# yanqinJiang/Animate3D

Measured on AMD Instinct MI355X. Metric: UNet denoise-steps/sec, 4view×16frame×512² MV-VDM @1/2/4/8 GPU, higher is better.
Workload: dtype bf16; 1 GPU; BASELINE config 2: 4 views x 16 frames x 512^2 px (64x64 latent), CFG-doubled batch V=8 videos, one MVUNetMotionModel.forward per step, SD1.5 MV-VDM UNet 1.53 B params, seeded synthetic weights; parallelism=single GPU

## Files before the change

### animate3d_amd/csrc/flash_attn.hip

```cpp
#include <type_traits>
#include <utility>

#include "common.h"
#include "flash_common.h"


namespace {

template <int D, int BKV, int QT, int OFS, bool ALIGNED, int VAR, int NM = 0, bool TWO = false>
__global__ __launch_bounds__(256, 2) void flash_attn_kernel(const AttnParams p) {
  constexpr int NU = BKV / 32;
  constexpr int VROW = BKV + 8;
  constexpr int DK = (D + 15) / 16 * 16;
  constexpr int KS = DK / 16;
  constexpr int MT = (D + 31) / 32;
  constexpr int KROW = DK + 8;
  constexpr int DCH = D / 8;
  constexpr int KCHUNKS = BKV * DCH;
  constexpr int KPT = (KCHUNKS + 255) / 256;
  constexpr int VITEMS = (BKV / 4) * DCH;
  constexpr int VPT = (VITEMS + 255) / 256;
  constexpr bool ONES = MT * 32 > D;
  constexpr int KS_ELEMS = BKV * KROW, VT_ELEMS = MT * 32 * VROW;
  constexpr int BQW = 32 * QT, BQ = 4 * BQW;
  constexpr int KS_PAD = D / 16, G_PAD = (D % 16) / 8;
  static_assert((KROW / 8) % 2 == 1 && (VROW / 8) % 2 == 1, "LDS row strides must be an odd number of 16-B slots");
  static_assert(OFS != OFS_PAD || (DK > D && D % 8 == 0), "OFS_PAD needs a spare contraction slot");

  __shared__ __attribute__((aligned(16))) uint16_t smem[2 * (KS_ELEMS + VT_ELEMS)];
  uint16_t* const Ks0 = smem;
  uint16_t* const Vt0 = smem + 2 * KS_ELEMS;

  const int tid = threadIdx.x, lane = tid & 63, wid = tid >> 6;
  const int l31 = lane & 31, g = lane >> 5;
  const int head = blockIdx.x % p.heads;
  const int qt = blockIdx.x / p.heads;
  const int64_t grp = blockIdx.y;
  const int64_t hoff = (int64_t)head * D;

  if constexpr (DK > D) {
    for (int i = tid; i < 2 * BKV * (DK - D); i += 256) {
      const int b = i / (BKV * (DK - D)), rem = i % (BKV * (DK - D));
      const int c = rem % (DK - D);
      Ks0[b * KS_ELEMS + (rem / (DK - D)) * KROW + D + c] = (OFS == OFS_PAD && c == 0) ? ONE16 : 0;
    }
  }
  if constexpr (ONES) {
    for (int i = tid; i < 2 * BKV; i += 256) Vt0[(i / BKV) * VT_ELEMS + D * VROW + (i % BKV)] = ONE16;
  }

  int q_idx[QT];
  bool q_ok[QT];
  u32x4_t qf[QT][KS];
#pragma unroll
  for (int qs = 0; qs < QT; ++qs) {
    q_idx[qs] = qt * BQ + wid * BQW + qs * 32 + l31;
    q_ok[qs] = q_idx[qs] < p.q_len;
    const int64_t q_row = map_row(p.qm, grp, q_ok[qs] ? q_idx[qs] : p.q_len - 1);
#pragma unroll
    for (int ks = 0; ks < KS; ++ks) {
      const int d0 = 16 * ks + 8 * g;
      if (d0 < D) {
        u32x4_t w = *reinterpret_cast<const u32x4_t*>(p.Q + q_row * p.qm.ld + hoff + d0);
        if constexpr (OFS != OFS_FMA) {
#pragma unroll
          for (int j = 0; j < 4; ++j) w[j] = pack16(lo16(w[j]) * p.scale_log2, hi16(w[j]) * p.scale_log2);
        }
        qf[qs][ks] = w;
      } else {
        qf[qs][ks] = u32x4_t{0u, 0u, 0u, 0u};
      }
    }
  }

#ifdef A3D_STORAGE_F16
  constexpr bool TRY_NOMAX = false;
#else
  constexpr bool TRY_NOMAX = NM != 0;
#endif
  static_assert(NM == 0 || (OFS != OFS_FMA && ALIGNED && ONES), "the max-free pass needs the offset inside the matrix pipe and MFMA row sums");
  f32x16_t osave[TWO ? QT : 1][TWO ? MT : 1];
  auto pass = [&](auto nm_c, auto set_c) __attribute__((always_inline)) -> bool {
  constexpr bool NOMAX = decltype(nm_c)::value;
  constexpr bool SET1 = decltype(set_c)::value;
  const uint16_t* const Kp = SET1 ? p.K2 : p.K;
  const uint16_t* const Vp = SET1 ? p.V2 : p.V;
  const a3d_rowmap& kmp = SET1 ? p.km2 : p.km;
  const int kvl = SET1 ? p.kv_len2 : p.kv_len;
  const float oscale = SET1 ? p.out_scale2 : p.out_scale;
  if constexpr (OFS == OFS_PAD) {
#pragma unroll
    for (int qs = 0; qs < QT; ++qs)
      if (g == G_PAD) qf[qs][KS_PAD][0] = 0u;
  }
  const int64_t ld = kmp.ld;
  const int64_t kgbase = map_group_base(kmp, grp);
  const uint16_t* const Kh = Kp + hoff;
  const uint16_t* const Vh = Vp + hoff;
  const uint32_t seg_len = (uint32_t)kmp.seg_len;
  const int64_t tile_step = (int64_t)BKV * ld;
  const int64_t wrap_step = (kmp.seg_stride - kmp.seg_len) * ld;
  int kr[KPT], kc[KPT], vq[VPT], vc[VPT];
  const uint16_t* kptr[KPT];
  const uint16_t* vptr[VPT];
#pragma unroll
  for (int i = 0; i < KPT; ++i) {
    const int c = tid + 256 * i;
    kr[i] = c / DCH; kc[i] = c % DCH;
    kptr[i] = Kh + (kgbase + kr[i]) * ld + kc[i] * 8;
  }
#pragma unroll
  for (int i = 0; i < VPT; ++i) {
    const int it = tid + 256 * i;
    vq[i] = it / DCH; vc[i] = it % DCH;
    vptr[i] = Vh + (kgbase + vq[i] * 4) * ld + vc[i] * 8;
  }
  uint32_t seg_off = 0;
  int next_kv0 = 0;

  auto row_generic = [&](int s) -> int64_t {
    if (s >= kvl) s = kvl - 1;
    const uint32_t seg = (uint32_t)s / seg_len;
    return kgbase + (int64_t)seg * kmp.seg_stride + ((uint32_t)s - seg * seg_len);
  };

  u32x4_t kreg[KPT];
  u32x4_t vreg[VPT][4];
  auto load_kv = [&](auto tail_c) {
    constexpr bool TAIL = decltype(tail_c)::value;
    if constexpr (ALIGNED && !TAIL) {
#pragma unroll
      for (int i = 0; i < KPT; ++i)
        if (tid + 256 * i < KCHUNKS) kreg[i] = *reinterpret_cast<const u32x4_t*>(kptr[i]);
#pragma unroll
      for (int i = 0; i < VPT; ++i)
        if (tid + 256 * i < VITEMS) {
#pragma unroll
          for (int r = 0; r < 4; ++r) vreg[i][r] = *reinterpret_cast<const u32x4_t*>(vptr[i] + r * ld);
        }
      seg_off += BKV;
      int64_t step = tile_step;
      if (seg_off >= seg_len) { step += wrap_step; seg_off = 0; }
#pragma unroll
      for (int i = 0; i < KPT; ++i) kptr[i] += step;
#pragma unroll
      for (int i = 0; i < VPT; ++i) vptr[i] += step;
    } else {
#pragma unroll
      for (int i = 0; i < KPT; ++i)
        if (tid + 256 * i < KCHUNKS)
          kreg[i] = *reinterpret_cast<const u32x4_t*>(Kh + row_generic(next_kv0 + kr[i]) * ld + kc[i] * 8);
#pragma unroll
      for (int i = 0; i < VPT; ++i)
        if (tid + 256 * i < VITEMS) {
#pragma unroll
          for (int r = 0; r < 4; ++r)
            vreg[i][r] = *reinterpret_cast<const u32x4_t*>(Vh + row_generic(next_kv0 + vq[i] * 4 + r) * ld + vc[i] * 8);
        }
    }
    next_kv0 += BKV;
  };
  auto store_kv = [&](int buf) {
    uint16_t* const Ks = Ks0 + buf * KS_ELEMS;
    uint16_t* const Vt = Vt0 + buf * VT_ELEMS;
#pragma unroll
    for (int i = 0; i < KPT; ++i)
      if (tid + 256 * i < KCHUNKS) *reinterpret_cast<u32x4_t*>(Ks + kr[i] * KROW + kc[i] * 8) = kreg[i];
#pragma unroll
    for (int i = 0; i < VPT; ++i)
      if (tid + 256 * i < VITEMS) {
#pragma unroll
        for (int j = 0; j < 4; ++j) {
          const uint32_t w0 = vreg[i][0][j], w1 = vreg[i][1][j], w2 = vreg[i][2][j], w3 = vreg[i][3][j];
          u32x2_t even, odd;
          even[0] = __builtin_amdgcn_perm(w1, w0, 0x05040100u);
          even[1] = __builtin_amdgcn_perm(w3, w2, 0x05040100u);
          odd[0] = __builtin_amdgcn_perm(w1, w0, 0x07060302u);
          odd[1] = __builtin_amdgcn_perm(w3, w2, 0x07060302u);
          *reinterpret_cast<u32x2_t*>(Vt + (vc[i] * 8 + 2 * j) * VROW + vq[i] * 4) = even;
          *reinterpret_cast<u32x2_t*>(Vt + (vc[i] * 8 + 2 * j + 1) * VROW + vq[i] * 4) = odd;
        }
      }
  };

  f32x16_t oacc[QT][MT];
#pragma unroll
  for (int qs = 0; qs < QT; ++qs)
#pragma unroll
    for (int mt = 0; mt < MT; ++mt)
#pragma unroll
      for (int r = 0; r < 16; ++r) oacc[qs][mt][r] = 0.f;
  float m_off[QT];
  float l_run = 0.f;
  f32x16_t minit[OFS == OFS_ACC ? QT : 1];
#pragma unroll
  for (int qs = 0; qs < QT; ++qs) m_off[qs] = (OFS == OFS_FMA) ? -INFINITY : 0.f;
  if constexpr (OFS == OFS_ACC) {
#pragma unroll
    for (int qs = 0; qs < QT; ++qs)
#pragma unroll
      for (int r = 0; r < 16; ++r) minit[qs][r] = 0.f;
  }
  bool first = true;
  const int krow_off = kperm(l31) * KROW + 8 * g;
  const int vrow_off = l31 * VROW + 8 * g;

  auto compute = [&](int buf, int kv0, auto tail_c, auto first_c) {
    constexpr bool TAIL = decltype(tail_c)::value;
    constexpr int FM = decltype(first_c)::value;
    const uint16_t* const Ks = Ks0 + buf * KS_ELEMS + krow_off;
    const uint16_t* const Vt = Vt0 + buf * VT_ELEMS + vrow_off;
    f32x16_t sacc[QT][NU];
#pragma unroll
    for (int u = 0; u < NU; ++u) {
#pragma unroll
      for (int qs = 0; qs < QT; ++qs) {
        if constexpr (OFS == OFS_ACC) sacc[qs][u] = minit[qs];
        else {
#pragma unroll
          for (int r = 0; r < 16; ++r) sacc[qs][u][r] = 0.f;
        }
      }
#pragma unroll
      for (int ks = 0; ks < KS; ++ks) {
        const u32x4_t kf = *reinterpret_cast<const u32x4_t*>(Ks + 32 * u * KROW + 16 * ks);
        if constexpr ((VAR & 1) != 0) __builtin_amdgcn_s_setprio(1);
#pragma unroll
        for (int qs = 0; qs < QT; ++qs) sacc[qs][u] = mfma32(kf, qf[qs][ks], sacc[qs][u]);
        if constexpr ((VAR & 1) != 0) __builtin_amdgcn_s_setprio(0);
      }
    }
    if constexpr (TAIL) {
#pragma unroll
      for (int u = 0; u < NU; ++u)
#pragma unroll
        for (int r = 0; r < 16; ++r)
          if (kv0 + 32 * u + 16 * (r >> 3) + 8 * g + (r & 7) >= kvl) {
#pragma unroll
            for (int qs = 0; qs < QT; ++qs) sacc[qs][u][r] = -INFINITY;
          }
    }
    if (p.causal) {
#pragma unroll
      for (int qs = 0; qs < QT; ++qs)
#pragma unroll
        for (int u = 0; u < NU; ++u)
#pragma unroll
          for (int r = 0; r < 16; ++r)
            if (kv0 + 32 * u + 16 * (r >> 3) + 8 * g + (r & 7) > q_idx[qs]) sacc[qs][u][r] = -INFINITY;
    }

    if constexpr (OFS == OFS_FMA && QT > 1) {
#pragma unroll
      for (int qs = 0; qs < QT; ++qs) {
        float mx = sacc[qs][0][0];
#pragma unroll
        for (int u = 0; u < NU; ++u)
#pragma unroll
          for (int r = 0; r < 16; ++r) mx = fmaxf(mx, sacc[qs][u][r]);
        if (__any(mx > m_off[qs] + LAZY_THR / p.scale_log2)) {
          mx = fmaxf(mx, __shfl_xor(mx, 32));
          const float m_new = fmaxf(m_off[qs], mx);
          const float alpha = __builtin_amdgcn_exp2f((m_off[qs] - m_new) * p.scale_log2);
          m_off[qs] = m_new;
          if constexpr (!ONES) l_run *= alpha;
#pragma unroll
          for (int mt = 0; mt < MT; ++mt)
#pragma unroll
            for (int r = 0; r < 16; ++r) oacc[qs][mt][r] *= alpha;
        }
        const float mneg = -m_off[qs] * p.scale_log2;
#pragma unroll
        for (int u = 0; u < NU; ++u)
#pragma unroll
          for (int r = 0; r < 16; ++r) sacc[qs][u][r] = fmaf(sacc[qs][u][r], p.scale_log2, mneg);
      }
    } else if constexpr (OFS == OFS_FMA) {
      float mx = sacc[0][0][0];
#pragma unroll
      for (int u = 0; u < NU; ++u)
#pragma unroll
        for (int r = 0; r < 16; ++r) mx = fmaxf(mx, sacc[0][u][r]);
      if (__any(mx > m_off[0] + LAZY_THR / p.scale_log2)) {
        mx = fmaxf(mx, __shfl_xor(mx, 32));
        const float m_new = fmaxf(m_off[0], mx);
        const float alpha = __builtin_amdgcn_exp2f((m_off[0] - m_new) * p.scale_log2);
        m_off[0] = m_new;
        l_run *= alpha;
#pragma unroll
        for (int mt = 0; mt < MT; ++mt)
#pragma unroll
          for (int r = 0; r < 16; ++r) oacc[0][mt][r] *= alpha;
      }
      const float mneg = -m_off[0] * p.scale_log2;
#pragma unroll
      for (int u = 0; u < NU; ++u)
#pragma unroll
        for (int r = 0; r < 16; ++r) sacc[0][u][r] = fmaf(sacc[0][u][r], p.scale_log2, mneg);
    } else {
      if constexpr (FM != 0) {
      const bool isfirst = (FM == 1) ? true : first;
#pragma unroll
      for (int qs = 0; qs < QT; ++qs) {
        float mx = sacc[qs][0][0];
#pragma unroll
        for (int u = 0; u < NU; ++u)
#pragma unroll
          for (int r = 0; r < 16; ++r) mx = fmaxf(mx, sacc[qs][u][r]);
        if (__any(isfirst || mx > LAZY_THR)) {
          const float mxp = fmaxf(mx, __shfl_xor(mx, 32));
          float delta = isfirst ? mxp + (NOMAX ? 40.f : 0.f) : fmaxf(mxp, 0.f);
          float new_off = m_off[qs] + delta;
          if constexpr (OFS == OFS_PAD) { new_off = round16(new_off); delta = new_off - m_off[qs]; }
          m_off[qs] = new_off;
#pragma unroll
          for (int u = 0; u < NU; ++u)
#pragma unroll
            for (int r = 0; r < 16; ++r) sacc[qs][u][r] -= delta;
          if (!isfirst) {
            const float alpha = __builtin_amdgcn_exp2f(-delta);
            if constexpr (!ONES) l_run *= alpha;
#pragma unroll
            for (int mt = 0; mt < MT; ++mt)
#pragma unroll
              for (int r = 0; r < 16; ++r) oacc[qs][mt][r] *= alpha;
          }
          if constexpr (OFS == OFS_PAD) {
            if (g == G_PAD) qf[qs][KS_PAD][0] = pack16(-new_off, 0.f);
          } else {
#pragma unroll
            for (int r = 0; r < 16; ++r) minit[qs][r] = -new_off;
          }
        }
      }
      }
      first = false;
    }

#pragma unroll
    for (int u = 0; u < NU; ++u) {
      u32x4_t vfr[(VAR & 2) ? MT : 1][2];
      if constexpr ((VAR & 2) != 0) {
#pragma unroll
        for (int mt = 0; mt < MT; ++mt)
#pragma unroll
          for (int h = 0; h < 2; ++h) vfr[mt][h] = *reinterpret_cast<const u32x4_t*>(Vt + 32 * mt * VROW + 32 * u + 16 * h);
      }
      u32x4_t pf[QT][2];
#pragma unroll
      for (int qs = 0; qs < QT; ++qs) {
        float pv[16];
#pragma unroll
        for (int r = 0; r < 16; ++r) {
          pv[r] = __builtin_amdgcn_exp2f(sacc[qs][u][r]);
          if constexpr (!ONES) l_run += pv[r];
        }
#pragma unroll
        for (int h = 0; h < 2; ++h)
#pragma unroll
          for (int j = 0; j < 4; ++j) pf[qs][h][j] = pack16(pv[8 * h + 2 * j], pv[8 * h + 2 * j + 1]);
      }
      if constexpr ((VAR & 1) != 0) __builtin_amdgcn_s_setprio(1);
#pragma unroll
      for (int mt = 0; mt < MT; ++mt)
#pragma unroll
        for (int h = 0; h < 2; ++h) {
          u32x4_t vf;
          if constexpr ((VAR & 2) != 0) vf = vfr[mt][h];
          else vf = *reinterpret_cast<const u32x4_t*>(Vt + 32 * mt * VROW + 32 * u + 16 * h);
#pragma unroll
          for (int qs = 0; qs < QT; ++qs) oacc[qs][mt] = mfma32(vf, pf[qs][h], oacc[qs][mt]);
        }
      if constexpr ((VAR & 1) != 0) __builtin_amdgcn_s_setprio(0);
    }
    if constexpr ((VAR & 4) != 0) {
#pragma unroll
      for (int i = 0; i < NU * MT * 2 * QT; ++i) {
        __builtin_amdgcn_sched_group_barrier(0x008, 1, 0);
        __builtin_amdgcn_sched_group_barrier(0x400, 4, 0);
        __builtin_amdgcn_sched_group_barrier(0x002, 2, 0);
      }
    }
  };

  const int ntiles = (kvl + BKV - 1) / BKV;
  const bool has_tail = (kvl % BKV) != 0;
  auto load_tile = [&](int t) {
    if (has_tail && t == ntiles - 1) load_kv(std::true_type{}); else load_kv(std::false_type{});
  };

  load_tile(0);
  store_kv(0);
  if (ntiles > 1) load_tile(1);
  __syncthreads();
  const int nfast = has_tail ? ntiles - 1 : ntiles;
  constexpr std::integral_constant<int, NOMAX ? 0 : 2> FM_LOOP{};
  int t = 0;
  if constexpr (ALIGNED) {
    if constexpr (NOMAX) {
      store_kv(1);
      load_kv(std::false_type{});
      compute(0, 0, std::false_type{}, std::integral_constant<int, 1>{});
      __syncthreads();
      t = 1;
    }
    for (; t + 2 < nfast; ++t) {
      store_kv((t + 1) & 1);
      load_kv(std::false_type{});
      compute(t & 1, t * BKV, std::false_type{}, FM_LOOP);
      __syncthreads();
    }
  }
  for (; t < ntiles - 1; ++t) {
    store_kv((t + 1) & 1);
    if (t + 2 < ntiles) load_tile(t + 2);
    compute(t & 1, t * BKV, std::false_type{}, FM_LOOP);
    __syncthreads();
  }
  if (has_tail) compute((ntiles - 1) & 1, (ntiles - 1) * BKV, std::true_type{}, FM_LOOP);
  else compute((ntiles - 1) & 1, (ntiles - 1) * BKV, std::false_type{}, FM_LOOP);

  float inv[QT], l_fin[QT];
  bool bad = false;
#pragma unroll
  for (int qs = 0; qs < QT; ++qs) {
    float l_tot;
    if constexpr (ONES) {
      constexpr int LM = D / 32, LR = ((D % 32) / 8) * 4;
      static_assert((D % 32) % 8 == 0, "row D must map to half 0");
      l_tot = __shfl(oacc[qs][LM][LR], l31);
    } else {
      l_tot = l_run + __shfl_xor(l_run, 32);
    }
    bad = bad || !(l_tot < 1.2676506e30f) || !(l_tot > 0.f);
    inv[qs] = oscale / l_tot;
    l_fin[qs] = l_tot;
  }
  if constexpr (NOMAX) {
    if (__syncthreads_or(bad ? 1 : 0)) return false;
  }
  if constexpr (!TWO) {
    if (p.lse != nullptr) {
#pragma unroll
      for (int qs = 0; qs < QT; ++qs)
        if (q_ok[qs] && g == 0)
          p.lse[((int64_t)grp * p.heads + head) * p.q_len + q_idx[qs]] =
              __builtin_amdgcn_logf(l_fin[qs]) + (OFS == OFS_FMA ? m_off[qs] * p.scale_log2 : m_off[qs]);
    }
  }
  if constexpr (TWO && !SET1) {
    if (p.K2 != nullptr) {
#pragma unroll
      for (int qs = 0; qs < QT; ++qs)
#pragma unroll
        for (int mt = 0; mt < MT; ++mt)
#pragma unroll
          for (int r = 0; r < 16; ++r) osave[qs][mt][r] = oacc[qs][mt][r] * inv[qs];
      return true;
    }
  }
#pragma unroll
  for (int qs = 0; qs < QT; ++qs) {
    if (q_ok[qs]) {
      uint16_t* orow = p.O + map_row(p.om, grp, q_idx[qs]) * p.om.ld + hoff;
#pragma unroll
      for (int mt = 0; mt < MT; ++mt)
#pragma unroll
        for (int qd = 0; qd < 4; ++qd) {
          const int d = 32 * mt + 8 * qd + 4 * g;
          if (d < D) {
            float v[4];
#pragma unroll
            for (int j = 0; j < 4; ++j) {
              v[j] = oacc[qs][mt][4 * qd + j] * inv[qs];
              if constexpr (TWO && SET1) v[j] += osave[qs][mt][4 * qd + j];
            }
            if (p.accumulate) {
              const u32x2_t prev = *reinterpret_cast<const u32x2_t*>(orow + d);
              v[0] += lo16(prev[0]); v[1] += hi16(prev[0]); v[2] += lo16(prev[1]); v[3] += hi16(prev[1]);
            }
            u32x2_t o;
            o[0] = pack16(v[0], v[1]);
            o[1] = pack16(v[2], v[3]);
            *reinterpret_cast<u32x2_t*>(orow + d) = o;
          }
        }
    }
  }
  return true;
  };

  if constexpr (TRY_NOMAX) {
    if (!pass(std::true_type{}, std::false_type{})) pass(std::false_type{}, std::false_type{});
  } else {
    pass(std::false_type{}, std::false_type{});
  }
  if constexpr (TWO) {
    if (p.K2 != nullptr) {
      __syncthreads();
      pass(std::false_type{}, std::true_type{});
    }
  }
}

bool map_ok(const a3d_rowmap* m, int head_dim) {
  return m && m->gdiv > 0 && m->seg_len > 0 && m->ld > 0 && m->ld % 8 == 0 && head_dim % 8 == 0;
}


template <int D, int BKV, int QT, int OFS, int VAR = 0, int NM = 0>
void launch(bool aligned, int groups, hipStream_t s, const AttnParams& p) {
  const int q_tiles = (p.q_len + 128 * QT - 1) / (128 * QT);
  const dim3 grid((unsigned)(p.heads * q_tiles), (unsigned)groups);
  if (aligned) flash_attn_kernel<D, BKV, QT, OFS, true, VAR, NM><<<grid, dim3(256), 0, s>>>(p);
  else flash_attn_kernel<D, BKV, QT, OFS, false, 0><<<grid, dim3(256), 0, s>>>(p);
}

template <int D, int BKV, int OFS>
void launch_two(bool aligned, int groups, hipStream_t s, const AttnParams& p) {
  const int q_tiles = (p.q_len + 127) / 128;
  const dim3 grid((unsigned)(p.heads * q_tiles), (unsigned)groups);
  if (aligned) flash_attn_kernel<D, BKV, 1, OFS, true, 0, 0, true><<<grid, dim3(256), 0, s>>>(p);
  else flash_attn_kernel<D, BKV, 1, OFS, false, 0, 0, true><<<grid, dim3(256), 0, s>>>(p);
}

}

static int flash_attn_impl(a3d_stream_t stream, const void* Q, const void* K, const void* V, void* O,
                           const a3d_rowmap* qmap, const a3d_rowmap* kmap, const a3d_rowmap* omap,
                           int groups, int heads, int head_dim, int64_t q_len, int64_t kv_len,
                           float scale, float out_scale, int accumulate, float* lse, unsigned int* counters = nullptr) {
  if (!Q || !K || !V || !O || groups <= 0 || heads <= 0 || q_len <= 0 || kv_len <= 0) return A3D_EINVAL;
  if (!map_ok(qmap, head_dim) || !map_ok(kmap, head_dim) || !map_ok(omap, head_dim)) return A3D_EINVAL;
  if ((reinterpret_cast<uintptr_t>(Q) | reinterpret_cast<uintptr_t>(K) | reinterpret_cast<uintptr_t>(V)) & 15u) return A3D_EINVAL;
  if (reinterpret_cast<uintptr_t>(O) & 7u) return A3D_EINVAL;
  if (groups > 65535 || q_len > 0x3fffffffLL || kv_len > 0x3fffffffLL || kmap->seg_len > 0x3fffffffLL) return A3D_EINVAL;
  AttnParams p{};
  p.Q = (const uint16_t*)Q; p.K = (const uint16_t*)K; p.V = (const uint16_t*)V; p.O = (uint16_t*)O;
  p.qm = *qmap; p.km = *kmap; p.om = *omap;
  p.heads = heads; p.q_len = (int)q_len; p.kv_len = (int)kv_len;
  if (accumulate & ~(A3D_ATTN_ACCUMULATE | A3D_ATTN_CAUSAL | A3D_ATTN_EXACT | A3D_ATTN_PLAIN)) return A3D_EINVAL;
  p.scale_log2 = scale * 1.4426950408889634f; p.out_scale = out_scale; p.accumulate = accumulate & 1; p.causal = (accumulate >> 1) & 1;
  const bool exact = (accumulate & A3D_ATTN_EXACT) != 0, plain = (accumulate & A3D_ATTN_PLAIN) != 0;
  p.lse = lse;
  p.counters = counters;
  if (p.causal && head_dim != 64 && head_dim != 160) return A3D_EUNSUPPORTED;
  const int bkv = head_dim == 160 ? 32 : 64;
  const bool aligned = (kmap->seg_len % bkv == 0) || (kv_len <= kmap->seg_len);
  hipStream_t s = (hipStream_t)stream;
  switch (head_dim) {
    case 40:
      if (q_len <= 128) { launch<40, 64, 1, OFS_PAD>(aligned, groups, s, p); break; }
      if (!plain && aligned && kv_len % 64 == 0 && kv_len >= 256 && q_len >= 256) {
        if (int rc = A3D_FN(a3d_launch_flash_dm)(exact ? 4 : 5, groups, s, p)) return rc;
        break;
      }
      launch<40, 64, 2, OFS_PAD, 0>(aligned, groups, s, p);
      break;
    case 80:
      if (!plain && aligned && kv_len % 64 == 0 && kv_len >= 512 && q_len >= 256) {
        if (int rc = A3D_FN(a3d_launch_flash_dm80)(exact ? 0 : 1, groups, s, p)) return rc;
        break;
      }
      if (q_len >= 2048 && kv_len >= 2048) { launch<80, 32, 2, OFS_FMA>(aligned, groups, s, p); break; }
      launch<80, 64, 1, OFS_ACC>(aligned, groups, s, p);
      break;
    case 64: launch<64, 64, 1, OFS_FMA>(aligned, groups, s, p); break;
    case 160:
#ifndef A3D_EXP_R5_PATHS
      if (!plain && !p.causal && kv_len % 64 == 0 && kv_len >= 256 && ((kmap->seg_len % 64 == 0) || (kv_len <= kmap->seg_len)) &&
          (reinterpret_cast<uintptr_t>(O) & 15u) == 0 && omap->ld % 8 == 0) {
        if (int rc = A3D_FN(a3d_launch_flash_dm160)(exact ? 0 : 1, groups, s, p)) return rc;
        break;
      }
#endif
      launch<160, 32, 1, OFS_FMA>(aligned, groups, s, p);
      break;
    default: return A3D_EUNSUPPORTED;
  }
  return a3d_launch_status();
}

extern "C" int A3D_FN(a3d_flash_attn)(a3d_stream_t stream, const void* Q, const void* K, const void* V, void* O,
                                   const a3d_rowmap* qmap, const a3d_rowmap* kmap, const a3d_rowmap* omap,
                                   int groups, int heads, int head_dim, int64_t q_len, int64_t kv_len,
                                   float scale, float out_scale, int accumulate) {
  return flash_attn_impl(stream, Q, K, V, O, qmap, kmap, omap, groups, heads, head_dim, q_len, kv_len, scale, out_scale, accumulate, nullptr);
}

extern "C" int A3D_FN(a3d_flash_attn_lse)(a3d_stream_t stream, const void* Q, const void* K, const void* V, void* O,
                                       const a3d_rowmap* qmap, const a3d_rowmap* kmap, const a3d_rowmap* omap,
                                       int groups, int heads, int head_dim, int64_t q_len, int64_t kv_len,
                                       float scale, float out_scale, int accumulate, float* lse2) {
  if (!lse2) return A3D_EINVAL;
  return flash_attn_impl(stream, Q, K, V, O, qmap, kmap, omap, groups, heads, head_dim, q_len, kv_len, scale, out_scale, accumulate, lse2);
}

extern "C" int A3D_FN(a3d_flash_attn_counted)(a3d_stream_t stream, const void* Q, const void* K, const void* V, void* O,
                                           const a3d_rowmap* qmap, const a3d_rowmap* kmap, const a3d_rowmap* omap,
                                           int groups, int heads, int head_dim, int64_t q_len, int64_t kv_len,
                                           float scale, float out_scale, int accumulate, unsigned int* counters) {
  if (!counters || (reinterpret_cast<uintptr_t>(counters) & 3u)) return A3D_EINVAL;
  return flash_attn_impl(stream, Q, K, V, O, qmap, kmap, omap, groups, heads, head_dim, q_len, kv_len, scale, out_scale, accumulate, nullptr, counters);
}

extern "C" int A3D_FN(a3d_flash_attn2)(a3d_stream_t stream, const void* Q, const void* K, const void* V, const void* K2, const void* V2, void* O,
                                    const a3d_rowmap* qmap, const a3d_rowmap* kmap, const a3d_rowmap* kmap2, const a3d_rowmap* omap,
                                    int groups, int heads, int head_dim, int64_t q_len, int64_t kv_len, int64_t kv_len2,
                                    float scale, float out_scale, float out_scale2, int accumulate) {
  if (!Q || !K || !V || !K2 || !V2 || !O || groups <= 0 || heads <= 0 || q_len <= 0 || kv_len <= 0 || kv_len2 <= 0) return A3D_EINVAL;
  if (!map_ok(qmap, head_dim) || !map_ok(kmap, head_dim) || !map_ok(kmap2, head_dim) || !map_ok(omap, head_dim)) return A3D_EINVAL;
  if ((reinterpret_cast<uintptr_t>(Q) | reinterpret_cast<uintptr_t>(K) | reinterpret_cast<uintptr_t>(V) | reinterpret_cast<uintptr_t>(K2) |
       reinterpret_cast<uintptr_t>(V2)) & 15u) return A3D_EINVAL;
  if (reinterpret_cast<uintptr_t>(O) & 7u) return A3D_EINVAL;
  if (groups > 65535 || q_len > 0x3fffffffLL || kv_len > 0x3fffffffLL || kv_len2 > 0x3fffffffLL || kmap->seg_len > 0x3fffffffLL ||
      kmap2->seg_len > 0x3fffffffLL) return A3D_EINVAL;
  if (head_dim != 40 && head_dim != 80) return A3D_EUNSUPPORTED;
  AttnParams p{};
  p.Q = (const uint16_t*)Q; p.K = (const uint16_t*)K; p.V = (const uint16_t*)V; p.O = (uint16_t*)O;
  p.K2 = (const uint16_t*)K2; p.V2 = (const uint16_t*)V2;
  p.qm = *qmap; p.km = *kmap; p.km2 = *kmap2; p.om = *omap;
  p.heads = heads; p.q_len = (int)q_len; p.kv_len = (int)kv_len; p.kv_len2 = (int)kv_len2;
  if (accumulate & ~(A3D_ATTN_ACCUMULATE | A3D_ATTN_PLAIN)) return A3D_EINVAL;
  p.scale_log2 = scale * 1.4426950408889634f; p.out_scale = out_scale; p.out_scale2 = out_scale2; p.accumulate = accumulate & 1; p.causal = 0;
  const bool aligned = ((kmap->seg_len % 64 == 0) || (kv_len <= kmap->seg_len)) && ((kmap2->seg_len % 64 == 0) || (kv_len2 <= kmap2->seg_len));
  hipStream_t s = (hipStream_t)stream;
  if (head_dim == 40 && !(accumulate & A3D_ATTN_PLAIN)) {
    const int rc = A3D_FN(a3d_launch_cross_attn40)(groups, s, p);
    if (rc != A3D_EUNSUPPORTED) return rc;
  }
  if (head_dim == 40) launch_two<40, 64, OFS_PAD>(aligned, groups, s, p);
  else launch_two<80, 64, OFS_ACC>(aligned, groups, s, p);
  return a3d_launch_status();
}
```

### animate3d_amd/csrc/flash_attn_dm80.hip

```cpp
#include "flash_common.h"

namespace {

constexpr int E_ROWB = 160;
constexpr int E_UNITB = 32 * E_ROWB;
constexpr int E_KB = 2 * E_UNITB;
constexpr int E_TILEB = 2 * E_KB;
constexpr int E_RING = 5;
constexpr int E_CV = E_RING * E_TILEB + 32;
constexpr int E_CV_BYTES = 2752;
constexpr int E_SAMPLE = E_CV + E_CV_BYTES;
constexpr int E_SMEM_BYTES = E_SAMPLE + E_UNITB;
constexpr float E_L_BAD = 1.2676506e30f;
#ifdef A3D_STORAGE_F16
constexpr float E_BIAS = F16_BIAS;
constexpr bool E_SAMPLED = true;
#else
constexpr float E_BIAS = 40.f;
constexpr bool E_SAMPLED = false;
#endif

#ifdef A3D_EXP_R5_PATHS
constexpr bool E_EARLY_DMA = false;
#else
constexpr bool E_EARLY_DMA = true;
#endif

extern __shared__ __attribute__((aligned(16))) uint8_t e_smem[];
A3D_DEV u32x4_t e_lds128(uint32_t off) { return *reinterpret_cast<const u32x4_t*>(e_smem + off); }
A3D_DEV u32x2_t e_ldstr(uint32_t off) { return lds_tr16_b64(reinterpret_cast<const uint16_t*>(e_smem + off)); }

template <int FLAGS>
__global__ __launch_bounds__(512, 2) void flash_attn_dm80_kernel(const AttnParams p) {
  constexpr int D = 80, KS = 5, MT = 3, NT = 512, BQ = 256;
  constexpr int NEXP = 16, NCVT = 8, NDMA = 3;
  constexpr bool TRY_NOMAX = (FLAGS & 1) != 0;

  const int tid = threadIdx.x, lane = tid & 63, wid = tid >> 6;
  const int w = __builtin_amdgcn_readfirstlane(wid);
  const int l31 = lane & 31, g = lane >> 5, i16 = lane & 15, q4 = lane >> 4;
  const int head = blockIdx.x % p.heads;
  const int qt = blockIdx.x / p.heads;
  const int64_t grp = blockIdx.y;
  const int64_t hoff = (int64_t)head * D;
  const uint32_t lds0 = fa_lds_addr(e_smem);

  for (int i = tid; i < E_CV_BYTES / 2; i += NT) {
    const int vb = 2 * i;
    reinterpret_cast<uint16_t*>(e_smem + E_CV)[i] = (vb == 0 || vb == 160 || vb == 2560 || vb == 2720) ? ONE16 : (uint16_t)0;
  }

  const int64_t ld = p.km.ld;
  const int64_t kgbase = map_group_base(p.km, grp);
  const uint32_t seg_len = (uint32_t)p.km.seg_len;
  const int64_t tile_step = (int64_t)64 * ld;
  const int64_t wrap_step = (p.km.seg_stride - p.km.seg_len) * ld;
  auto slot_src = [&](int slot) -> uint32_t {
    const bool isk = slot < 640;
    const int s2 = isk ? slot : slot - 640;
    const int prow = s2 / 10, cpos = s2 % 10;
    const int c = isk ? (cpos ^ ((prow >> 3) & 1)) : cpos;
    const int key = isk ? prow : ((prow & ~7) | (((prow & 7) >> 1) + 4 * (prow & 1)));
    return (uint32_t)(((int64_t)key * ld + c * 8) * 2);
  };
  const uint32_t voffA = slot_src(64 * w + lane);
  const uint32_t voffB = slot_src(512 + 64 * w + lane);
  const uint32_t voffC = slot_src(1024 + 32 * w + l31);
  uint32_t voffS = 0;
  if constexpr (E_SAMPLED) {
    const int ss = (64 * w + lane) % 320, prow = ss / 10;
    const int64_t key = (int64_t)prow * (p.kv_len / 32);
    voffS = (uint32_t)((map_seq(p.km, key) * ld + ((ss % 10) ^ ((prow >> 3) & 1)) * 8) * 2);
  }
  const uint64_t maskS = w < 5 ? ~0ull : 0ull;

  const int krow = kperm(l31);
  const uint32_t klane = (uint32_t)(krow * E_ROWB + 16 * (g ^ ((krow >> 3) & 1)));
  const int c4 = i16 & 3;
  const uint32_t vrow = (uint32_t)((8 * (q4 >> 1) + 2 * (i16 >> 2)) * E_ROWB);
  const uint32_t vlane01 = vrow + (uint32_t)(2 * (16 * (q4 & 1) + 4 * c4));
  const bool v2_data = (q4 & 1) == 0;
  const uint32_t vlane2 = v2_data ? vrow + (uint32_t)(2 * (64 + 4 * c4)) : (c4 == 0 ? (uint32_t)E_CV : (uint32_t)(E_CV + 8));
  uint32_t vmul = v2_data ? 1u : 0u;
  asm volatile("" : "+v"(vmul));

  const uint16_t* gA = nullptr;
  const uint16_t* gB = nullptr;
  const uint16_t* gC = nullptr;
  uint32_t seg_off = 0;
  auto dma_reset = [&]() __attribute__((always_inline)) {
    gA = dm_scalar(p.K + hoff + kgbase * ld);
    gB = dm_scalar((w < 2 ? p.K : p.V) + hoff + kgbase * ld);
    gC = dm_scalar(p.V + hoff + kgbase * ld);
    seg_off = 0;
  };
  auto tile_base = [&](int tile) __attribute__((always_inline)) -> uint32_t { return (uint32_t)((tile % E_RING) * E_TILEB); };
  auto dma_a = [&](int tile) __attribute__((always_inline)) { dm_glds16(voffA, gA, lds0 + tile_base(tile) + 1024 * w); };
  auto dma_b = [&](int tile) __attribute__((always_inline)) { dm_glds16(voffB, gB, lds0 + tile_base(tile) + 8192 + 1024 * w); };
  auto dma_c = [&](int tile) __attribute__((always_inline)) {
    dm_glds16_m(voffC, gC, lds0 + tile_base(tile) + 16384 + 512 * w, 0xffffffffull);
    seg_off += 64;
    int64_t stp = tile_step;
    if (seg_off >= seg_len) { stp += wrap_step; seg_off = 0; }
    gA += stp; gB += stp; gC += stp;
  };
  auto prologue_issue = [&]() __attribute__((always_inline)) {
    dma_reset();
    if constexpr (E_SAMPLED && TRY_NOMAX)
      dm_glds16_m(voffS, dm_scalar(p.K + hoff + kgbase * ld), lds0 + (uint32_t)(E_SAMPLE + 1024 * (w < 5 ? w : 0)), maskS);
    dma_a(0); dma_b(0); dma_c(0);
    dma_a(1); dma_b(1); dma_c(1);
    dma_a(2); dma_b(2); dma_c(2);
  };
  auto prologue_wait = [&]() __attribute__((always_inline)) { asm volatile("s_waitcnt vmcnt(%0)\n\ts_barrier" :: "i"(NDMA) : "memory"); };
  if constexpr (E_EARLY_DMA) prologue_issue();

  const int q_idx = qt * BQ + wid * 32 + l31;
  u32x4_t qf[KS];
  {
    const int64_t q_row = map_row(p.qm, grp, q_idx < p.q_len ? q_idx : p.q_len - 1);
#pragma unroll
    for (int ks = 0; ks < KS; ++ks) {
      u32x4_t wq = *reinterpret_cast<const u32x4_t*>(p.Q + q_row * p.qm.ld + hoff + 16 * ks + 8 * g);
#pragma unroll
      for (int j = 0; j < 4; ++j) wq[j] = pack16(lo16(wq[j]) * p.scale_log2, hi16(wq[j]) * p.scale_log2);
      qf[ks] = wq;
    }
  }


  f32x16_t oacc[MT];
  f32x16_t minit;
  u32x4_t kf[KS];
  u32x4_t vf[MT][2];
  auto read_k = [&](uint32_t koff) __attribute__((always_inline)) {
    const uint32_t a = klane + koff;
#pragma unroll
    for (int ks = 0; ks < KS; ++ks) kf[ks] = e_lds128(a + 32 * ks);
  };
  auto read_vhalf = [&](auto i_c, uint32_t a01, uint32_t a2) __attribute__((always_inline)) {
    constexpr int i = decltype(i_c)::value, h = i / 6, mt = (i / 2) % 3, rr = i % 2;
    const u32x2_t t = e_ldstr((mt == 2 ? a2 : a01 + 64 * mt) + (16 * h + rr) * E_ROWB);
    vf[mt][h][2 * rr] = t[0];
    vf[mt][h][2 * rr + 1] = t[1];
  };
  auto read_v = [&](uint32_t voff) __attribute__((always_inline)) {
    const uint32_t a01 = vlane01 + voff, a2 = __umul24(vmul, voff) + vlane2;
    static_for<12>([&](auto i_c) __attribute__((always_inline)) { read_vhalf(i_c, a01, a2); });
  };
  auto pv_mfma = [&](auto i_c, u32x4_t (&P)[2]) __attribute__((always_inline)) {
    constexpr int i = decltype(i_c)::value, h = i / 3, mt = i % 3;
    oacc[mt] = mfma32(vf[mt][h], P[h], oacc[mt]);
  };
  auto clear_o = [&]() __attribute__((always_inline)) {
#pragma unroll
    for (int mt = 0; mt < MT; ++mt)
#pragma unroll
      for (int r = 0; r < 16; ++r) oacc[mt][r] = 0.f;
#pragma unroll
    for (int r = 0; r < 16; ++r) minit[r] = 0.f;
  };
  const int nt = p.kv_len / 64;
  auto first_scores = [&](f32x16_t& s, float& m_off, float bias, uint32_t koff = 0u) __attribute__((always_inline)) -> bool {
    read_k(koff);
#pragma unroll
    for (int r = 0; r < 16; ++r) s[r] = 0.f;
#pragma unroll
    for (int ks = 0; ks < KS; ++ks) s = mfma32(kf[ks], qf[ks], s);
    float mx = s[0];
#pragma unroll
    for (int r = 1; r < 16; ++r) mx = fmaxf(mx, s[r]);
    mx = fmaxf(mx, __shfl_xor(mx, 32));
    bool wide = false;
    if constexpr (E_SAMPLED) {
      if (bias != 0.f) {
        float sm = 0.f, sq = 0.f;
#pragma unroll
        for (int r = 0; r < 16; ++r) { sm += s[r]; sq = fmaf(s[r], s[r], sq); }
        sm += __shfl_xor(sm, 32); sq += __shfl_xor(sq, 32);
        const float mean = sm * (1.f / 32.f);
        bias = f16_sampled_bias(mx, mean, sq * (1.f / 32.f) - mean * mean, f16_expected_max_sds(p.kv_len), wide);
      }
    }
    m_off = mx + bias;
#pragma unroll
    for (int r = 0; r < 16; ++r) { s[r] -= m_off; minit[r] = -m_off; }
    return wide;
  };
  auto finish = [&](bool check) __attribute__((always_inline)) -> bool {
    const float l_tot = __shfl(oacc[2][8], l31);
    const bool bad = !(l_tot < E_L_BAD) || !(l_tot > 0.f);
    if (check) {
      if (__syncthreads_or(bad ? 1 : 0)) { dm_count(p, 1); return false; }
    }
    const float inv = p.out_scale / l_tot;
    if (p.lse != nullptr && q_idx < p.q_len && g == 0)
      p.lse[((int64_t)grp * p.heads + head) * p.q_len + q_idx] = __builtin_amdgcn_logf(l_tot) - minit[0];
    if (q_idx < p.q_len) {
      uint16_t* orow = p.O + map_row(p.om, grp, q_idx) * p.om.ld + hoff;
      const bool wide_rows = E_EARLY_DMA && !p.accumulate && ((reinterpret_cast<uintptr_t>(p.O) | (uintptr_t)(p.om.ld * 2)) & 15u) == 0;
      if (wide_rows) {
#pragma unroll
        for (int mt = 0; mt < MT; ++mt)
#pragma unroll
          for (int pr = 0; pr < 2; ++pr) {
            if (32 * mt + 16 * pr >= D) continue;
            u32x4_t v;
#pragma unroll
            for (int c = 0; c < 2; ++c) {
              const uint32_t w0 = pack16(oacc[mt][8 * pr + 2 * c] * inv, oacc[mt][8 * pr + 2 * c + 1] * inv);
              const uint32_t w1 = pack16(oacc[mt][8 * pr + 4 + 2 * c] * inv, oacc[mt][8 * pr + 4 + 2 * c + 1] * inv);
              const auto r = __builtin_amdgcn_permlane32_swap(w0, w1, false, false);
              v[c] = r[0];
              v[2 + c] = r[1];
            }
            *reinterpret_cast<u32x4_t*>(orow + 32 * mt + 16 * pr + 8 * g) = v;
          }
      } else {
#pragma unroll
        for (int mt = 0; mt < MT; ++mt)
#pragma unroll
          for (int qd = 0; qd < 4; ++qd) {
            const int d = 32 * mt + 8 * qd + 4 * g;
            if (d < D) {
              float v[4];
#pragma unroll
              for (int j = 0; j < 4; ++j) v[j] = oacc[mt][4 * qd + j] * inv;
              if (p.accumulate) {
                const u32x2_t prev = *reinterpret_cast<const u32x2_t*>(orow + d);
                v[0] += lo16(prev[0]); v[1] += hi16(prev[0]); v[2] += lo16(prev[1]); v[3] += hi16(prev[1]);
              }
              u32x2_t o;
              o[0] = pack16(v[0], v[1]);
              o[1] = pack16(v[2], v[3]);
              *reinterpret_cast<u32x2_t*>(orow + d) = o;
            }
          }
      }
    }
    return true;
  };

  auto run_fast = [&]() __attribute__((always_inline)) -> bool {
    clear_o();
    f32x16_t sA, sB;
    u32x4_t pA[2], pB[2];
#pragma unroll
    for (int h = 0; h < 2; ++h) { pA[h] = u32x4_t{0u, 0u, 0u, 0u}; pB[h] = u32x4_t{0u, 0u, 0u, 0u}; }

    auto step = [&](auto do_qk_c, auto do_pv_c, f32x16_t& sCur, f32x16_t& sNext, u32x4_t (&pCur)[2], u32x4_t (&pPrev)[2],
                    uint32_t kOff, uint32_t vOff, auto&& hook) __attribute__((always_inline)) {
      constexpr bool DO_QK = decltype(do_qk_c)::value, DO_PV = decltype(do_pv_c)::value;
      constexpr int NPV = DO_PV ? 2 * MT : 0, NQK = DO_QK ? KS : 0, NS = NPV + NQK;
      constexpr int KSLOT = 2, VS0 = NPV + 1, VPS = 3;
      const uint32_t va01 = vlane01 + vOff, va2 = __umul24(vmul, vOff) + vlane2;
      float e[NEXP];
      auto do_cvt = [&](auto c_c) __attribute__((always_inline)) {
        constexpr int c = decltype(c_c)::value, h = c / 4, jj = c % 4;
        pCur[h][jj] = pack16(e[2 * c], e[2 * c + 1]);
      };
      auto cdone = [](int s) constexpr { return s < 0 ? 0 : (NEXP * s / NS) / 2; };
      __builtin_amdgcn_sched_barrier(0);
      static_for<NS>([&](auto s_c) __attribute__((always_inline)) {
        constexpr int s = decltype(s_c)::value;
        if constexpr (s < NPV) {
          pv_mfma(s_c, pPrev);
        } else {
          constexpr int ks = s - NPV;
          if constexpr (ks == 0) sNext = mfma32(kf[0], qf[0], minit);
          else sNext = mfma32(kf[ks], qf[ks], sNext);
        }
        if constexpr (DO_QK && DO_PV && s == KSLOT) read_k(kOff);
        if constexpr (DO_QK && s >= VS0 && VPS * (s - VS0) < 12) {
          static_for<VPS>([&](auto i_c) __attribute__((always_inline)) {
            constexpr int i = VPS * (s - VS0) + decltype(i_c)::value;
            if constexpr (i < 12) read_vhalf(std::integral_constant<int, i>{}, va01, va2);
          });
        }
        hook(s_c);
        constexpr int E0 = NEXP * s / NS, E1 = NEXP * (s + 1) / NS;
        static_for<E1 - E0>([&](auto x_c) __attribute__((always_inline)) {
          constexpr int x = E0 + decltype(x_c)::value;
          e[x] = __builtin_amdgcn_exp2f(sCur[x]);
        });
        constexpr int C0 = cdone(s - 1), C1 = cdone(s);
        static_for<C1 - C0>([&](auto c_c) __attribute__((always_inline)) { do_cvt(std::integral_constant<int, C0 + decltype(c_c)::value>{}); });
        __builtin_amdgcn_sched_barrier(0);
      });
      {
        constexpr int C0 = cdone(NS - 1);
        static_for<NCVT - C0>([&](auto c_c) __attribute__((always_inline)) { do_cvt(std::integral_constant<int, C0 + decltype(c_c)::value>{}); });
      }
    };

    if constexpr (!E_EARLY_DMA) prologue_issue();
    prologue_wait();
    {
      float m_off;
      if constexpr (E_SAMPLED) {
        const bool wide = first_scores(sA, m_off, E_BIAS, (uint32_t)E_SAMPLE);
        if (__syncthreads_count(wide ? 1 : 0) * 4 > NT) { dm_count(p, 0); return false; }
        read_k(0u);
        sA = minit;
#pragma unroll
        for (int ks = 0; ks < KS; ++ks) sA = mfma32(kf[ks], qf[ks], sA);
      } else {
        first_scores(sA, m_off, E_BIAS);
      }
      read_k((uint32_t)E_UNITB);
    }

    auto iteration = [&](int t, auto first_c, auto last_c, auto dma_c_) __attribute__((always_inline)) {
      constexpr bool FIRST = decltype(first_c)::value, LAST = decltype(last_c)::value, DMA = decltype(dma_c_)::value;
      auto even_hook = [&](auto s_c) __attribute__((always_inline)) {
        if constexpr (DMA && decltype(s_c)::value == 1) dma_a(t + 3);
      };
      auto odd_hook = [&](auto s_c) __attribute__((always_inline)) {
        if constexpr (DMA && decltype(s_c)::value == 1) dma_b(t + 3);
        if constexpr (DMA && decltype(s_c)::value == 4) dma_c(t + 3);
      };
      const uint32_t tb = tile_base(t), tn = tile_base(t + 1);
      step(std::true_type{}, std::integral_constant<bool, !FIRST>{}, sA, sB, pA, pB, tb + E_UNITB, tb + E_KB, even_hook);
      step(std::integral_constant<bool, !LAST>{}, std::true_type{}, sB, sA, pB, pA, tn, tb + E_KB + E_UNITB, odd_hook);
      if constexpr (!LAST) {
        if constexpr (DMA) asm volatile("s_waitcnt vmcnt(%0)\n\ts_barrier" :: "i"(NDMA) : "memory");
        else asm volatile("s_waitcnt vmcnt(0)\n\ts_barrier" ::: "memory");
      }
    };
    constexpr std::true_type Y{};
    constexpr std::false_type N{};
    iteration(0, Y, N, Y);
    for (int t = 1; t < nt - 3; ++t) iteration(t, N, N, Y);
    iteration(nt - 3, N, N, N);
    iteration(nt - 2, N, N, N);
    iteration(nt - 1, N, Y, N);
    {
      read_v(tile_base(nt - 1) + E_KB + E_UNITB);
      static_for<2 * MT>([&](auto i_c) __attribute__((always_inline)) { pv_mfma(i_c, pB); });
    }
    return finish(true);
  };

  auto run_exact = [&](auto rerun_c) __attribute__((always_inline)) {
    clear_o();
    float m_off;
    f32x16_t sc;
    if constexpr (decltype(rerun_c)::value || !E_EARLY_DMA) prologue_issue();
    prologue_wait();
    first_scores(sc, m_off, 0.f);
    for (int t = 0; t < nt; ++t) {
      const bool more = t + 3 < nt;
      if (more) { dma_a(t + 3); dma_b(t + 3); dma_c(t + 3); }
      const uint32_t tb = tile_base(t);
#pragma unroll
      for (int sub = 0; sub < 2; ++sub) {
        if (t > 0 || sub > 0) {
          read_k(tb + sub * E_UNITB);
          sc = minit;
#pragma unroll
          for (int ks = 0; ks < KS; ++ks) sc = mfma32(kf[ks], qf[ks], sc);
          float mx = sc[0];
#pragma unroll
          for (int r = 1; r < 16; ++r) mx = fmaxf(mx, sc[r]);
          if (__any(mx > LAZY_THR)) {
            const float delta = fmaxf(fmaxf(mx, __shfl_xor(mx, 32)), 0.f);
            m_off += delta;
            const float alpha = __builtin_amdgcn_exp2f(-delta);
#pragma unroll
            for (int r = 0; r < 16; ++r) { sc[r] -= delta; minit[r] = -m_off; }
#pragma unroll
            for (int mt = 0; mt < MT; ++mt)
#pragma unroll
              for (int r = 0; r < 16; ++r) oacc[mt][r] *= alpha;
          }
        }
        u32x4_t pf[2];
#pragma unroll
        for (int h = 0; h < 2; ++h)
#pragma unroll
          for (int jj = 0; jj < 4; ++jj)
            pf[h][jj] = pack16(__builtin_amdgcn_exp2f(sc[8 * h + 2 * jj]), __builtin_amdgcn_exp2f(sc[8 * h + 2 * jj + 1]));
        read_v(tb + E_KB + sub * E_UNITB);
        static_for<2 * MT>([&](auto i_c) __attribute__((always_inline)) { pv_mfma(i_c, pf); });
      }
      if (t + 1 < nt) {
        if (more) asm volatile("s_waitcnt vmcnt(%0)\n\ts_barrier" :: "i"(NDMA) : "memory");
        else asm volatile("s_waitcnt vmcnt(0)\n\ts_barrier" ::: "memory");
      }
    }
    finish(false);
  };

  __syncthreads();
  dm_count(p, 2);
  if constexpr (TRY_NOMAX) {
    if (!run_fast()) run_exact(std::true_type{});
  } else {
    run_exact(std::false_type{});
  }
}

template <int FLAGS>
int launch_dm80(int groups, hipStream_t s, const AttnParams& p) {
  static uint64_t attr_done = 0;
  if (int rc = a3d_once_per_device(attr_done, [] {
        return (int)hipFuncSetAttribute(reinterpret_cast<const void*>(&flash_attn_dm80_kernel<FLAGS>),
                                        hipFuncAttributeMaxDynamicSharedMemorySize, E_SMEM_BYTES); })) return rc;
  const int q_tiles = (p.q_len + 255) / 256;
  flash_attn_dm80_kernel<FLAGS><<<dim3((unsigned)(p.heads * q_tiles), (unsigned)groups), dim3(512), E_SMEM_BYTES, s>>>(p);
  return a3d_launch_status();
}

}

int A3D_FN(a3d_launch_flash_dm80)(int flags, int groups, hipStream_t s, const AttnParams& p) {
  switch (flags) {
    case 0: return launch_dm80<0>(groups, s, p);
    case 1: return launch_dm80<1>(groups, s, p);
    default: return A3D_EINVAL;
  }
}
```

### animate3d_amd/csrc/flash_common.h

```cpp
#pragma once
#include <type_traits>
#include <utility>

#include "common.h"

struct AttnParams {
  const uint16_t* Q; const uint16_t* K; const uint16_t* V; uint16_t* O;
  a3d_rowmap qm, km, om;
  int heads; int q_len, kv_len;
  float scale_log2, out_scale; int accumulate;
  int causal;
  const uint16_t* K2; const uint16_t* V2; a3d_rowmap km2; int kv_len2; float out_scale2;
  float* lse;
  unsigned int* counters;
};

namespace {

constexpr int OFS_FMA = 0, OFS_PAD = 1, OFS_ACC = 2;
constexpr float LAZY_THR = 6.0f;


A3D_DEV uint32_t map_clamp32(int64_t d) { return d > 0x7fffffffLL ? 0x7fffffffu : (uint32_t)d; }
A3D_DEV int64_t map_group_base(const a3d_rowmap& m, int64_t g) {
  const uint32_t g32 = (uint32_t)g, gd = map_clamp32(m.gdiv), gq = g32 / gd, gr = g32 - gq * gd;
  return (int64_t)gq * m.ga + (int64_t)gr * m.gb;
}
A3D_DEV int64_t map_seq(const a3d_rowmap& m, int64_t s) {
  const uint32_t s32 = (uint32_t)s, sl = map_clamp32(m.seg_len), sq = s32 / sl, sr = s32 - sq * sl;
  return (int64_t)sq * m.seg_stride + (int64_t)sr;
}
A3D_DEV int64_t map_row(const a3d_rowmap& m, int64_t g, int64_t s) { return map_group_base(m, g) + map_seq(m, s); }

A3D_DEV int kperm(int i) {
  const int j = i & 3, g = (i >> 2) & 1, b = i >> 3;
  return 16 * (b >> 1) + 8 * g + 4 * (b & 1) + j;
}

A3D_DEV float round16(float x) { return lo16(pack16(x, 0.f)); }

constexpr float F16_BIAS = 4.f, F16_LIFT_MAX = 8.f, F16_TOP = 16.f;
A3D_DEV float f16_expected_max_sds(int kv_len) {
  return 2.85f + 0.175f * (float)(31 - __builtin_clz((unsigned)(kv_len < 256 ? 256 : kv_len)) - 8);
}
A3D_DEV float f16_sampled_bias(float mx, float mean, float var, float cmax, bool& wide) {
  const float sd = __builtin_amdgcn_sqrtf(fmaxf(var, 0.f));
  const float lift = fminf(fmaxf(fmaf(cmax, sd, mean) - mx, 0.f), F16_LIFT_MAX);
  wide = !(fmaf(cmax + 2.2f, sd, mean) <= mx + F16_BIAS + lift + F16_TOP);
  return F16_BIAS + lift;
}


A3D_DEV void dm_glds16(uint32_t voff, const void* sbase, uint32_t lds_dst) {
  unsigned keep;
  asm volatile("s_mov_b32 %0, m0\n\ts_mov_b32 m0, %3\n\ts_nop 0\n\tglobal_load_lds_dwordx4 %1, %2\n\ts_mov_b32 m0, %0"
               : "=&s"(keep) : "v"(voff), "s"(sbase), "s"(__builtin_amdgcn_readfirstlane(lds_dst)) : "memory");
}
A3D_DEV void dm_glds16_q(uint32_t voff, const void* sbase, uint32_t lds_dst) {
  unsigned keep;
  uint64_t ex;
  asm volatile("s_mov_b32 %0, m0\n\ts_mov_b32 m0, %4\n\ts_mov_b64 %1, exec\n\ts_mov_b64 exec, 0xffff\n\ts_nop 0\n\t"
               "global_load_lds_dwordx4 %2, %3\n\ts_mov_b64 exec, %1\n\ts_mov_b32 m0, %0"
               : "=&s"(keep), "=&s"(ex) : "v"(voff), "s"(sbase), "s"(__builtin_amdgcn_readfirstlane(lds_dst)) : "memory");
}
A3D_DEV void dm_glds16_m(uint32_t voff, const void* sbase, uint32_t lds_dst, uint64_t mask) {
  unsigned keep;
  uint64_t ex;
  mask = ((uint64_t)(uint32_t)__builtin_amdgcn_readfirstlane((int)(mask >> 32)) << 32) | (uint32_t)__builtin_amdgcn_readfirstlane((int)(uint32_t)mask);
  asm volatile("s_mov_b32 %0, m0\n\ts_mov_b32 m0, %4\n\ts_mov_b64 %1, exec\n\ts_mov_b64 exec, %5\n\ts_nop 0\n\t"
               "global_load_lds_dwordx4 %2, %3\n\ts_mov_b64 exec, %1\n\ts_mov_b32 m0, %0"
               : "=&s"(keep), "=&s"(ex) : "v"(voff), "s"(sbase), "s"(__builtin_amdgcn_readfirstlane(lds_dst)), "s"(mask) : "memory");
}
A3D_DEV const uint16_t* dm_scalar(const uint16_t* ptr) {
  const uint64_t a = (uint64_t)(uintptr_t)ptr;
  return (const uint16_t*)(uintptr_t)(((uint64_t)(uint32_t)__builtin_amdgcn_readfirstlane((int)(a >> 32)) << 32) |
                                      (uint32_t)__builtin_amdgcn_readfirstlane((int)(uint32_t)a));
}

A3D_DEV void dm_count(const AttnParams& p, int which) {
#ifndef A3D_EXP_R5_PATHS
  if (p.counters != nullptr && threadIdx.x == 0) atomicAdd(p.counters + which, 1u);
#endif
}

A3D_DEV uint32_t fa_lds_addr(const void* p) {
  return (uint32_t)(uintptr_t)(__attribute__((address_space(3))) const void*)p;
}

}

__attribute__((visibility("hidden"))) int A3D_FN(a3d_launch_flash_dm)(int flags, int groups, hipStream_t s, const AttnParams& p);
__attribute__((visibility("hidden"))) int A3D_FN(a3d_launch_flash_dm80)(int flags, int groups, hipStream_t s, const AttnParams& p);
__attribute__((visibility("hidden"))) int A3D_FN(a3d_launch_flash_dm160)(int flags, int groups, hipStream_t s, const AttnParams& p);
__attribute__((visibility("hidden"))) int A3D_FN(a3d_launch_cross_attn40)(int groups, hipStream_t s, const AttnParams& p);
```

### animate3d_amd/hip_ops.py

```python
from __future__ import annotations

import ctypes
import os
from dataclasses import dataclass
from typing import Optional

import torch

_LIB_PATH = os.path.join(os.path.dirname(os.path.abspath(__file__)), "lib", "libanimate3d_hip.so")
_lib = None

c_i64, c_int, c_f32, c_vp = ctypes.c_int64, ctypes.c_int, ctypes.c_float, ctypes.c_void_p


class _RowMapC(ctypes.Structure):
    _fields_ = [("gdiv", c_i64), ("ga", c_i64), ("gb", c_i64), ("seg_len", c_i64), ("seg_stride", c_i64), ("ld", c_i64)]


@dataclass(frozen=True)
class RowMap:
    gdiv: int
    ga: int
    gb: int
    seg_len: int
    seg_stride: int

    def c(self, ld: int) -> _RowMapC:
        return _RowMapC(self.gdiv, self.ga, self.gb, self.seg_len, self.seg_stride, ld)


def rowmap_rows(m: RowMap, groups: int, step: int, length: int, device="cpu") -> torch.Tensor:
    g = torch.arange(0, groups, step, device=device).view(-1, 1)
    s = torch.arange(length, device=device).view(1, -1)
    return ((g // m.gdiv) * m.ga + (g % m.gdiv) * m.gb + (s // m.seg_len) * m.seg_stride + s % m.seg_len).reshape(-1)


def rowmap_covers(m: RowMap, groups: int, step: int, length: int, rows: int, device="cpu") -> bool:
    if (groups + step - 1) // step * length != rows:
        return False
    idx = rowmap_rows(m, groups, step, length, device)
    return bool(int(idx.min()) >= 0 and int(idx.max()) < rows and torch.unique(idx).numel() == rows)


_SIGNATURES = {
    "a3d_version": (ctypes.c_char_p, []),
    "a3d_gemm_bf16": (c_int, [c_vp, c_vp, c_i64, c_vp, c_i64, c_vp, c_vp, c_i64, c_vp, c_i64, c_vp, c_i64, c_i64, c_i64, c_i64, c_f32, c_f32, c_int]),
    "a3d_gemm_ws_bf16": (c_int, [c_vp, c_vp, c_i64, c_vp, c_i64, c_vp, c_vp, c_i64, c_vp, c_i64, c_vp, c_i64, c_i64, c_i64, c_i64, c_f32, c_f32, c_int,
                                 c_vp, c_i64, ctypes.POINTER(c_i64)]),
    "a3d_gemm2_bf16": (c_int, [c_vp, c_vp, c_i64, c_vp, c_i64, c_i64, c_vp, c_i64, c_vp, c_vp, c_i64, c_i64, c_i64, c_i64, c_int]),
    "a3d_gemm_geglu_bf16": (c_int, [c_vp, c_vp, c_i64, c_vp, c_i64, c_vp, c_vp, c_i64, c_i64, c_i64, c_i64, c_int]),
    "a3d_conv3x3_bf16": (c_int, [c_vp, c_vp, c_vp, c_vp, c_vp, c_i64, c_vp, c_vp, c_int, c_int, c_int, c_int, c_int, c_int, c_int, c_int]),
    "a3d_conv3x3_ws_bf16": (c_int, [c_vp, c_vp, c_vp, c_vp, c_vp, c_i64, c_vp, c_vp, c_int, c_int, c_int, c_int, c_int, c_int, c_int, c_int,
                                    c_vp, c_i64, ctypes.POINTER(c_i64)]),
    "a3d_flash_attn_bf16": (c_int, [c_vp, c_vp, c_vp, c_vp, c_vp, ctypes.POINTER(_RowMapC), ctypes.POINTER(_RowMapC), ctypes.POINTER(_RowMapC),
                                    c_int, c_int, c_int, c_i64, c_i64, c_f32, c_f32, c_int]),
    "a3d_flash_attn_counted_bf16": (c_int, [c_vp, c_vp, c_vp, c_vp, c_vp, ctypes.POINTER(_RowMapC), ctypes.POINTER(_RowMapC), ctypes.POINTER(_RowMapC),
                                            c_int, c_int, c_int, c_i64, c_i64, c_f32, c_f32, c_int, c_vp]),
    "a3d_flash_attn2_bf16": (c_int, [c_vp, c_vp, c_vp, c_vp, c_vp, c_vp, c_vp, ctypes.POINTER(_RowMapC), ctypes.POINTER(_RowMapC), ctypes.POINTER(_RowMapC),
                                     ctypes.POINTER(_RowMapC), c_int, c_int, c_int, c_i64, c_i64, c_i64, c_f32, c_f32, c_f32, c_int]),
    "a3d_temporal_attn_bf16": (c_int, [c_vp, c_vp, c_vp, c_vp, c_i64, c_vp, c_i64, c_int, c_int, c_i64, c_int, c_int, c_f32]),
    "a3d_temporal_attn_sharded_bf16": (c_int, [c_vp, c_vp, c_i64, c_vp, c_vp, c_i64, c_vp, c_i64, c_int, c_int, c_i64, c_int, c_int, c_f32,
                                               c_int, c_int, c_int, c_i64]),
    "a3d_group_norm_ws_floats": (c_i64, [c_int, c_i64, c_int]),
    "a3d_group_norm_bf16": (c_int, [c_vp, c_vp, c_vp, c_vp, c_vp, c_vp, c_int, c_i64, c_int, c_int, c_f32, c_int]),
    "a3d_group_norm2_bf16": (c_int, [c_vp, c_vp, c_int, c_vp, c_int, c_vp, c_vp, c_vp, c_vp, c_int, c_i64, c_int, c_f32, c_int]),
    "a3d_group_norm_sums_bf16": (c_int, [c_vp, c_vp, c_vp, c_vp, c_int, c_i64, c_int, c_int]),
    "a3d_group_norm_apply_bf16": (c_int, [c_vp, c_vp, c_vp, c_vp, c_vp, c_vp, c_int, c_i64, c_int, c_int, c_int]),
    "a3d_layer_norm_bf16": (c_int, [c_vp, c_vp, c_vp, c_vp, c_vp, c_vp, c_i64, c_int, c_f32, c_vp, c_i64, c_i64, c_vp, c_i64, c_i64]),
    "a3d_geglu_bf16": (c_int, [c_vp, c_vp, c_i64, c_vp, c_i64, c_i64, c_i64]),
    "a3d_silu_bf16": (c_int, [c_vp, c_vp, c_vp, c_i64]),
    "a3d_activation_bf16": (c_int, [c_vp, c_vp, c_vp, c_i64, c_int]),
    "a3d_concat_bf16": (c_int, [c_vp, c_vp, c_i64, c_vp, c_i64, c_vp, c_i64]),
    "a3d_timestep_embed_bf16": (c_int, [c_vp, c_vp, c_vp, c_int, c_int]),
    "a3d_im2col_in": (c_int, [c_vp, c_vp, c_int, c_vp, c_int, c_int, c_int, c_int, c_int]),
    "a3d_unpack_out": (c_int, [c_vp, c_vp, c_vp, c_int, c_int, c_int, c_int, c_int, c_int]),
    "a3d_gemm_f32out_bf16": (c_int, [c_vp, c_vp, c_i64, c_vp, c_i64, c_vp, c_vp, c_i64, c_i64, c_i64, c_i64, c_f32]),
    "a3d_softmax_rows_f32_bf16": (c_int, [c_vp, c_vp, c_i64, c_vp, c_i64, c_i64, c_i64]),
    "a3d_softmax_rows_bwd_bf16": (c_int, [c_vp, c_vp, c_i64, c_vp, c_i64, c_vp, c_i64, c_i64, c_i64, c_f32]),
    "a3d_im2col_in_bwd": (c_int, [c_vp, c_vp, c_vp, c_int, c_int, c_int, c_int, c_int, c_f32]),
    "a3d_channel_mix_f32": (c_int, [c_vp, c_vp, c_vp, c_vp, c_vp, c_int, c_int, c_int, c_i64, c_f32]),
    "a3d_cfg_ddim_step_f32": (c_int, [c_vp, c_vp, c_vp, c_vp, c_vp, c_i64, c_int, c_int, c_i64, c_f32, c_f32, c_f32]),
    "a3d_flash_attn_bwd_bf16": (c_int, [c_vp, c_vp, c_vp, c_vp, c_vp, c_vp, c_vp, c_vp, c_vp, c_vp,
                                        ctypes.POINTER(_RowMapC), ctypes.POINTER(_RowMapC), ctypes.POINTER(_RowMapC), ctypes.POINTER(_RowMapC),
                                        ctypes.POINTER(_RowMapC), c_int, c_int, c_int, c_i64, c_i64, c_int, c_f32, c_f32, c_int]),
    "a3d_flash_attn_lse_bf16": (c_int, [c_vp, c_vp, c_vp, c_vp, c_vp, ctypes.POINTER(_RowMapC), ctypes.POINTER(_RowMapC), ctypes.POINTER(_RowMapC),
                                        c_int, c_int, c_int, c_i64, c_i64, c_f32, c_f32, c_int, c_vp]),
    "a3d_attn_delta_bf16": (c_int, [c_vp, c_vp, c_vp, ctypes.POINTER(_RowMapC), ctypes.POINTER(_RowMapC), c_vp, c_int, c_int, c_int, c_i64]),
    "a3d_temporal_attn_bwd_bf16": (c_int, [c_vp, c_vp, c_vp, c_vp, c_i64, c_vp, c_i64, c_vp, c_vp, c_vp, c_i64, c_int, c_int, c_i64, c_int, c_int, c_f32]),
    "a3d_layer_norm_bwd_bf16": (c_int, [c_vp, c_vp, c_vp, c_vp, c_vp, c_vp, c_vp, c_i64, c_int, c_f32, c_int]),
    "a3d_group_norm_bwd_bf16": (c_int, [c_vp, c_vp, c_vp, c_vp, c_vp, c_vp, c_vp, c_vp, c_vp, c_vp, c_int, c_i64, c_int, c_int, c_int]),
    "a3d_geglu_bwd_bf16": (c_int, [c_vp, c_vp, c_i64, c_vp, c_i64, c_vp, c_i64, c_i64, c_i64]),
    "a3d_transpose_bf16": (c_int, [c_vp, c_vp, c_i64, c_vp, c_i64, c_i64, c_i64, c_i64]),
    "a3d_wgrad_ws_floats": (c_i64, [c_i64, c_i64, c_i64]),
    "a3d_wgrad_bf16": (c_int, [c_vp, c_vp, c_i64, c_vp, c_i64, c_vp, c_i64, c_vp, c_i64, c_i64, c_i64, c_f32, c_int]),
    "a3d_colsum_bf16": (c_int, [c_vp, c_vp, c_i64, c_i64, c_i64, c_vp, c_f32, c_int]),
    "a3d_axpby_bf16": (c_int, [c_vp, c_vp, c_vp, c_i64, c_f32, c_f32]),
    "a3d_zero_insert2x_bf16": (c_int, [c_vp, c_vp, c_vp, c_int, c_int, c_int, c_int]),
    "a3d_upsample2x_bwd_bf16": (c_int, [c_vp, c_vp, c_vp, c_int, c_int, c_int, c_int, c_int, c_int]),
    "a3d_sqnorm_f32": (c_int, [c_vp, c_vp, c_i64, c_vp, c_int]),
    "a3d_clip_ctrl_f32": (c_int, [c_vp, c_vp, c_f32, c_f32, c_vp]),
    "a3d_adamw_f32": (c_int, [c_vp, c_vp, c_vp, c_vp, c_vp, c_i64, c_f32, c_f32, c_f32, c_f32, c_f32, c_f32, c_f32, c_vp]),
    "a3d_gs_preprocess_f32": (c_int, [c_vp, c_int, c_int, c_vp, c_i64, c_vp, c_i64, c_vp, c_i64, c_vp, c_i64, c_vp, c_i64, c_int, c_int, c_vp, c_i64, c_vp, c_vp, c_vp, c_vp, c_vp, c_int, c_int, c_f32, c_vp, c_vp, c_vp, c_vp, c_vp, c_vp, c_vp]),
    "a3d_gs_duplicate_f32": (c_int, [c_vp, c_int, c_int, c_int, c_int, c_vp, c_vp, c_vp, c_vp, c_vp, c_vp]),
    "a3d_gs_tile_ranges_f32": (c_int, [c_vp, c_vp, c_i64, c_vp, c_i64]),
    "a3d_gs_render_f32": (c_int, [c_vp, c_int, c_int, c_int, c_int, c_vp, c_vp, c_vp, c_vp, c_vp, c_vp, c_vp, c_vp, c_vp, c_vp, c_vp, c_vp, c_vp]),
    "a3d_gs_render_bwd_f32": (c_int, [c_vp, c_int, c_int, c_int, c_int, c_vp, c_vp, c_vp, c_vp, c_vp, c_vp, c_vp, c_vp, c_vp, c_vp, c_vp,
                                      c_vp, c_vp, c_vp]),
    "a3d_gs_preprocess_bwd_f32": (c_int, [c_vp, c_int, c_int, c_vp, c_i64, c_vp, c_i64, c_vp, c_i64, c_vp, c_i64, c_vp, c_i64, c_int, c_int, c_vp, c_i64, c_vp, c_vp, c_vp, c_vp, c_vp, c_int, c_int, c_f32, c_vp, c_vp, c_vp, c_vp, c_vp, c_vp, c_vp, c_vp, c_vp, c_vp, c_vp, c_vp]),
    "a3d_gs_sum_batch_f32": (c_int, [c_vp, c_vp, c_vp, c_int, c_i64]),
    "a3d_dg_cells_f32": (c_int, [c_vp, c_int, c_vp, c_vp, c_vp]),
    "a3d_dg_mean_partials": (c_i64, [c_int]),
    "a3d_dg_forward_f32": (c_int, [c_vp, c_int, c_int, c_int, c_vp, c_vp, c_vp, c_vp, c_vp, c_vp, c_vp, c_int, c_vp, c_vp, c_vp, c_vp, c_vp, c_vp,
                                   c_vp, c_vp, c_vp]),
    "a3d_dg_backward_ws_floats": (c_i64, [c_int, c_int, c_vp]),
    "a3d_dg_backward_f32": (c_int, [c_vp, c_int, c_int, c_int, c_vp, c_vp, c_vp, c_vp, c_vp, c_vp, c_vp, c_int, c_vp, c_vp, c_vp, c_vp, c_vp,
                                    c_vp, c_vp, c_vp, c_vp, c_vp, c_vp, c_vp, c_vp, c_vp, c_vp]),
    "a3d_knn_f32": (c_int, [c_vp, c_int, c_vp, c_int, c_int, c_f32, c_vp, c_vp]),
    "a3d_arap_energy_f32": (c_int, [c_vp, c_int, c_int, c_int, c_int, c_vp, c_vp, c_i64, c_vp, c_vp, c_vp, c_vp, c_vp, c_vp, c_vp]),
    "a3d_arap_backward_f32": (c_int, [c_vp, c_int, c_int, c_int, c_int, c_vp, c_vp, c_i64, c_vp, c_vp, c_vp, c_vp, c_vp, c_vp, c_vp, c_vp, c_vp]),
}
_UNSUFFIXED_TWINS = ("a3d_im2col_in", "a3d_unpack_out", "a3d_im2col_in_bwd")
for _name in list(_SIGNATURES):
    if _name.endswith("_bf16"):
        _SIGNATURES[_name[:-5] + "_f16"] = _SIGNATURES[_name]
    elif _name in _UNSUFFIXED_TWINS:
        _SIGNATURES[_name + "_f16"] = _SIGNATURES[_name]
EXPORTED_SYMBOLS = tuple(_SIGNATURES)

_DTYPE_CODE = {torch.float32: 0, torch.bfloat16: 1, torch.float16: 2}
A3D_EUNSUPPORTED = -2


def lib_path() -> str:
    return _LIB_PATH


def load_library():
    global _lib
    if _lib is None:
        if not os.path.exists(_LIB_PATH):
            raise RuntimeError(f"{_LIB_PATH} is missing: run `python -m animate3d_amd.build` (or __graft_entry__.build()). "
                               "There is no CPU fallback for the MI355X kernels.")
        lib = ctypes.CDLL(_LIB_PATH)
        for name, (res, args) in _SIGNATURES.items():
            fn = getattr(lib, name)
            fn.restype, fn.argtypes = res, args
        _lib = lib
    return _lib


def _check(rc: int, what: str):
    if rc != 0:
        kind = {-1: "A3D_EINVAL (shape/alignment precondition)", -2: "A3D_EUNSUPPORTED"}.get(rc, f"hipError {rc}")
        raise RuntimeError(f"{what} failed: {kind}")


def _p(t: Optional[torch.Tensor]):
    return None if t is None else t.data_ptr()


def on_model_device(method):
    import functools

    @functools.wraps(method)
    def wrapper(self, *args, **kwargs):
        dev = self.device
        if dev.type == "cuda" and torch.cuda.current_device() != (dev.index if dev.index is not None else torch.cuda.current_device()):
            with torch.cuda.device(dev):
                return method(self, *args, **kwargs)
        return method(self, *args, **kwargs)
    return wrapper


class _Entry:

    def __init__(self, lib, f16: bool):
        self._lib, self._f16 = lib, f16

    def __getattr__(self, name):
        if self._f16:
            if name.endswith("_bf16"):
                name = name[:-5] + "_f16"
            elif name in _UNSUFFIXED_TWINS:
                name = name + "_f16"
        return getattr(self._lib, name)


class HipOps:

    has_attn_lse = True

    def __init__(self, device: Optional[torch.device] = None, act_dtype: torch.dtype = torch.bfloat16, split_k: bool = True):
        if not torch.cuda.is_available():
            raise RuntimeError("HipOps needs a visible MI355X (torch.cuda.is_available() is False); no CPU fallback exists")
        if act_dtype not in (torch.bfloat16, torch.float16):
            raise ValueError(f"storage type {act_dtype} is not supported (bfloat16 or float16)")
        self.raw_lib = load_library()
        self._kv_row_cache = {}
        self._kv_cover_cache = {}
        self.act_dtype = act_dtype
        self.lib = _Entry(self.raw_lib, act_dtype == torch.float16)
        self.device = torch.device(device) if device is not None else torch.device("cuda", torch.cuda.current_device())
        self.reserved_cus = 0
        self.split_k = bool(split_k)
        self.split_k_gemm = False
        self.attn_counters = None
        self._ws_plan = {}
        self._ws_bufs = {}

    def _workspace(self, need: int) -> torch.Tensor:
        if torch.cuda.is_current_stream_capturing():
            return torch.empty(max(need, 1 << 20), dtype=torch.uint8, device=self.device)
        stream = self._stream()
        buf = self._ws_bufs.get(stream)
        if buf is None or buf.numel() < need:
            buf = self._ws_bufs[stream] = torch.empty(max(need, 1 << 20), dtype=torch.uint8, device=self.device)
        return buf

    def _gemm_flags(self, tile128: bool, ring: bool = False, direct: bool = False) -> int:
        r = int(self.reserved_cus)
        if not 0 <= r <= 0xFF:
            raise ValueError(f"reserved_cus = {self.reserved_cus}: the flags word of a3d_gemm / a3d_conv3x3 carries 0..255 reserved compute units")
        return r | (0x100 if tile128 else (0x200 if ring else (0x300 if direct else 0)))

    def _stream(self):
        return torch.cuda.current_stream(self.device).cuda_stream

    def _act(self, t: torch.Tensor, name: str):
        if t.dtype != self.act_dtype or not t.is_cuda or t.dim() != 2 or t.stride(1) != 1:
            raise RuntimeError(f"{name}: expected a 2-D {self.act_dtype} CUDA tensor with contiguous rows, got {t.dtype} {tuple(t.shape)} {t.device} strides {t.stride()}")
        return t

    def split_cols(self, x, *bounds):
        return tuple(x[:, a:b] for a, b in zip(bounds[:-1], bounds[1:]))

    def empty(self, rows: int, cols: int) -> torch.Tensor:
        return torch.empty((rows, cols), dtype=self.act_dtype, device=self.device)

    def gemm(self, x, w, bias=None, *, residual=None, alpha: float = 1.0, beta: float = 1.0, rowbias=None, rb_div: int = 1, out=None,
             tile128: bool = False, ring: bool = False, direct: bool = False):
        x, w = self._act(x, "gemm.x"), self._act(w, "gemm.w")
        M, K = x.shape
        N = w.shape[0]
        assert w.shape[1] == K, (x.shape, w.shape)
        y = out if out is not None else self.empty(M, N)
        self._act(y, "gemm.out")
        if residual is not None:
            self._act(residual, "gemm.residual")
            assert residual.shape == (M, N)
        if rowbias is not None:
            self._act(rowbias, "gemm.rowbias")
            assert rowbias.is_contiguous() and rowbias.shape[1] == N
        if bias is not None:
            assert bias.dtype == torch.float32 and bias.numel() == N
        flags = self._gemm_flags(tile128, ring, direct)
        args = (self._stream(), _p(x), x.stride(0), _p(w), w.stride(0), _p(bias), _p(rowbias), rb_div,
                _p(residual), residual.stride(0) if residual is not None else 0, _p(y), y.stride(0), M, N, K, alpha, beta, flags)
        if self.split_k and self.split_k_gemm and not tile128 and M <= 32768 and K >= 1152:
            key = ("gemm", M, N, K, x.stride(0), w.stride(0), y.stride(0), rb_div if rowbias is not None else 0, flags)
            need = self._ws_plan.get(key)
            if need is None:
                q = c_i64(0)
                _check(self.lib.a3d_gemm_ws_bf16(*args, None, 0, ctypes.byref(q)), f"a3d_gemm_ws_bf16 (query) M={M} N={N} K={K}")
                need = self._ws_plan[key] = int(q.value)
            if need > 0:
                ws = self._workspace(need)
                _check(self.lib.a3d_gemm_ws_bf16(*args, _p(ws), need, None), f"a3d_gemm_ws_bf16 M={M} N={N} K={K}")
                return y
        rc = self.lib.a3d_gemm_bf16(*args)
        _check(rc, f"a3d_gemm_bf16 M={M} N={N} K={K}")
        return y

    def gemm2(self, xa, xb, w, bias=None):
        xa, xb, w = self._act(xa, "gemm2.xa"), self._act(xb, "gemm2.xb"), self._act(w, "gemm2.w")
        M, K1 = xa.shape
        K = K1 + xb.shape[1]
        N = w.shape[0]
        assert xb.shape[0] == M and w.shape[1] == K
        if K1 % 64 or K % 64 or N % 8:
            return None
        y = self.empty(M, N)
        rc = self.lib.a3d_gemm2_bf16(self._stream(), _p(xa), xa.stride(0), _p(xb), xb.stride(0), K1, _p(w), w.stride(0), _p(bias), _p(y), y.stride(0),
                                     M, N, K, self._gemm_flags(False))
        if rc == A3D_EUNSUPPORTED:
            return None
        _check(rc, f"a3d_gemm2_bf16 M={M} N={N} K={K1}+{K - K1}")
        return y

    @staticmethod
    def interleave_geglu(w: torch.Tensor) -> torch.Tensor:
        n = w.shape[0] // 2
        assert n % 32 == 0
        h, g = w[:n].reshape(n // 32, 32, *w.shape[1:]), w[n:].reshape(n // 32, 32, *w.shape[1:])
        return torch.stack([h, g], dim=1).reshape(w.shape).contiguous()

    def gemm_geglu(self, x, w_il, bias_il, *, tile128: bool = False):
        x, w_il = self._act(x, "geglu.x"), self._act(w_il, "geglu.w")
        M, K = x.shape
        N2 = w_il.shape[0]
        y = self.empty(M, N2 // 2)
        rc = self.lib.a3d_gemm_geglu_bf16(self._stream(), _p(x), x.stride(0), _p(w_il), w_il.stride(0), _p(bias_il), _p(y), y.stride(0), M, N2, K,
                                          self._gemm_flags(tile128))
        _check(rc, f"a3d_gemm_geglu_bf16 M={M} N2={N2} K={K}")
        return y

    def conv3x3(self, x, B: int, H: int, W: int, w, bias, *, stride: int = 1, up2x: bool = False, rowbias=None, rb_div: int = 1, residual=None,
                up_size=None, tile128: bool = False):
        x, w = self._act(x, "conv.x"), self._act(w, "conv.w")
        Cin = x.shape[1]
        Cout = w.shape[0]
        assert x.is_contiguous() and w.is_contiguous() and x.shape[0] == B * H * W and w.shape[1] == 9 * Cin
        He, We = (2 * H, 2 * W) if up2x else (H, W)
        up_code = 1 if up2x else 0
        if up_size is not None:
            if not up2x or up_size[0] not in (2 * H, 2 * H - 1) or up_size[1] not in (2 * W, 2 * W - 1):
                raise ValueError(f"forced upsample size {tuple(up_size)} is not reachable from {(H, W)} (2x or 2x - 1 per axis)")
            He, We = int(up_size[0]), int(up_size[1])
            up_code |= (2 if He == 2 * H - 1 else 0) | (4 if We == 2 * W - 1 else 0)
        Ho, Wo = (He - 1) // stride + 1, (We - 1) // stride + 1
        y = self.empty(B * Ho * Wo, Cout)
        if residual is not None:
            assert residual.is_contiguous() and residual.shape == y.shape
        if rowbias is not None:
            assert rowbias.is_contiguous() and rowbias.shape[1] == Cout
        flags = self._gemm_flags(tile128)
        args = (self._stream(), _p(x), _p(w), _p(bias), _p(rowbias), rb_div, _p(residual), _p(y), B, H, W, Cin, Cout, stride, up_code, flags)
        if self.split_k and not tile128 and B * Ho * Wo <= 32768:
            key = ("conv", B, H, W, Cin, Cout, stride, up_code, rb_div if rowbias is not None else 0, flags)
            need = self._ws_plan.get(key)
            if need is None:
                q = c_i64(0)
                _check(self.lib.a3d_conv3x3_ws_bf16(*args, None, 0, ctypes.byref(q)), f"a3d_conv3x3_ws_bf16 (query) B={B} H={H} W={W} Cin={Cin} Cout={Cout}")
                need = self._ws_plan[key] = int(q.value)
            if need > 0:
                ws = self._workspace(need)
                _check(self.lib.a3d_conv3x3_ws_bf16(*args, _p(ws), need, None), f"a3d_conv3x3_ws_bf16 B={B} H={H} W={W} Cin={Cin} Cout={Cout}")
                return y, Ho, Wo
        rc = self.lib.a3d_conv3x3_bf16(*args)
        _check(rc, f"a3d_conv3x3_bf16 B={B} H={H} W={W} Cin={Cin} Cout={Cout} stride={stride} up={up2x}")
        return y, Ho, Wo

    def flash_attn(self, q, k, v, qmap: RowMap, kmap: RowMap, groups: int, heads: int, q_len: int, kv_len: int, *,
                   out=None, out_scale: float = 1.0, accumulate: bool = False, causal: bool = False, with_lse: bool = False,
                   accumulation_target: bool = False, exact: bool = False, plain: bool = False):
        q, k, v = self._act(q, "attn.q"), self._act(k, "attn.k"), self._act(v, "attn.v")
        C = q.shape[1]
        D = C // heads
        assert k.stride(0) == v.stride(0)
        o = out if out is not None else self.empty(q.shape[0], C)
        qm, km, om = qmap.c(q.stride(0)), kmap.c(k.stride(0)), qmap.c(o.stride(0))
        flags = (1 if accumulate else 0) | (2 if causal else 0) | (4 if exact else 0) | (8 if plain else 0)
        if with_lse:
            lse = torch.empty((groups, heads, q_len), dtype=torch.float32, device=self.device)
            rc = self.lib.a3d_flash_attn_lse_bf16(self._stream(), _p(q), _p(k), _p(v), _p(o), ctypes.byref(qm), ctypes.byref(km), ctypes.byref(om),
                                                  groups, heads, D, q_len, kv_len, float(D) ** -0.5, out_scale,
                                                  flags, _p(lse))
            _check(rc, f"a3d_flash_attn_lse_bf16 groups={groups} heads={heads} D={D} q_len={q_len} kv_len={kv_len}")
            return o, lse
        if self.attn_counters is not None:
            cnt = self.attn_counters
            assert cnt.dtype == torch.int32 and cnt.is_cuda and cnt.numel() >= 3 and cnt.is_contiguous()
            rc = self.lib.a3d_flash_attn_counted_bf16(self._stream(), _p(q), _p(k), _p(v), _p(o), ctypes.byref(qm), ctypes.byref(km), ctypes.byref(om),
                                                      groups, heads, D, q_len, kv_len, float(D) ** -0.5, out_scale, flags, _p(cnt))
            _check(rc, f"a3d_flash_attn_counted_bf16 groups={groups} heads={heads} D={D} q_len={q_len} kv_len={kv_len}")
            return o
        rc = self.lib.a3d_flash_attn_bf16(self._stream(), _p(q), _p(k), _p(v), _p(o), ctypes.byref(qm), ctypes.byref(km), ctypes.byref(om),
                                          groups, heads, D, q_len, kv_len, float(D) ** -0.5, out_scale, flags)
        _check(rc, f"a3d_flash_attn_bf16 groups={groups} heads={heads} D={D} q_len={q_len} kv_len={kv_len}")
        return o

    def flash_attn2(self, q, k, v, k2, v2, qmap: RowMap, kmap: RowMap, kmap2: RowMap, groups: int, heads: int, q_len: int, kv_len: int,
                    kv_len2: int, *, out_scale2: float = 1.0):
        D = q.shape[1] // heads
        if D not in (40, 80):
            return None
        q, k, v, k2, v2 = self._act(q, "attn.q"), self._act(k, "attn.k"), self._act(v, "attn.v"), self._act(k2, "attn.k2"), self._act(v2, "attn.v2")
        assert k.stride(0) == v.stride(0) and k2.stride(0) == v2.stride(0)
        o = self.empty(q.shape[0], q.shape[1])
        qm, km, km2, om = qmap.c(q.stride(0)), kmap.c(k.stride(0)), kmap2.c(k2.stride(0)), qmap.c(o.stride(0))
        rc = self.lib.a3d_flash_attn2_bf16(self._stream(), _p(q), _p(k), _p(v), _p(k2), _p(v2), _p(o), ctypes.byref(qm), ctypes.byref(km),
                                           ctypes.byref(km2), ctypes.byref(om), groups, heads, D, q_len, kv_len, kv_len2, float(D) ** -0.5,
                                           1.0, out_scale2, 0)
        _check(rc, f"a3d_flash_attn2_bf16 groups={groups} heads={heads} D={D} q_len={q_len} kv_len={kv_len} kv_len2={kv_len2}")
        return o

    def temporal_attn(self, q, k, v, videos: int, frames: int, L: int, heads: int, *, q_f0: int = 0, q_frames: Optional[int] = None,
                      out=None):
        q, k, v = self._act(q, "tattn.q"), self._act(k, "tattn.k"), self._act(v, "tattn.v")
        C = q.shape[1]
        D = C // heads
        assert k.stride(0) == v.stride(0)
        o = self._act(out, "tattn.out") if out is not None else self.empty(q.shape[0], C)
        assert o.shape == (q.shape[0], C)
        if q_frames is None or q_frames == frames:
            assert q.stride(0) == k.stride(0)
            rc = self.lib.a3d_temporal_attn_bf16(self._stream(), _p(q), _p(k), _p(v), q.stride(0), _p(o), o.stride(0),
                                                 videos, frames, L, heads, D, float(D) ** -0.5)
        else:
            assert q.shape[0] == videos * q_frames * L and k.shape[0] == videos * frames * L
            rc = self.lib.a3d_temporal_attn_sharded_bf16(self._stream(), _p(q), q.stride(0), _p(k), _p(v), k.stride(0), _p(o), o.stride(0),
                                                         videos, frames, L, heads, D, float(D) ** -0.5, q_f0, q_frames, q_frames,
                                                         videos * q_frames * L)
        _check(rc, f"a3d_temporal_attn_bf16 videos={videos} frames={frames} L={L} D={D} q_f0={q_f0} q_frames={q_frames}")
        return o

    def group_norm(self, x, B: int, rows: int, gamma, beta, groups: int, eps: float, silu: bool):
        x = self._act(x, "gn.x")
        assert x.is_contiguous() and x.shape[0] == B * rows
        C = x.shape[1]
        y = self.empty(x.shape[0], C)
        ws = torch.empty(int(self.lib.a3d_group_norm_ws_floats(B, rows, groups)), dtype=torch.float32, device=self.device)
        rc = self.lib.a3d_group_norm_bf16(self._stream(), _p(x), _p(y), _p(gamma), _p(beta), _p(ws), B, rows, C, groups, eps, 1 if silu else 0)
        _check(rc, f"a3d_group_norm_bf16 B={B} rows={rows} C={C}")
        return y

    def group_norm2(self, xa, xb, B: int, rows: int, gamma, beta, groups: int, eps: float, silu: bool):
        xa, xb = self._act(xa, "gn2.xa"), self._act(xb, "gn2.xb")
        assert xa.is_contiguous() and xb.is_contiguous() and xa.shape[0] == B * rows == xb.shape[0]
        Ca, Cb = xa.shape[1], xb.shape[1]
        y = self.empty(xa.shape[0], Ca + Cb)
        ws = torch.empty(int(self.lib.a3d_group_norm_ws_floats(B, rows, groups)), dtype=torch.float32, device=self.device)
        rc = self.lib.a3d_group_norm2_bf16(self._stream(), _p(xa), Ca, _p(xb), Cb, _p(y), _p(gamma), _p(beta), _p(ws), B, rows, groups, eps, 1 if silu else 0)
        _check(rc, f"a3d_group_norm2_bf16 B={B} rows={rows} C={Ca}+{Cb}")
        return y

    def group_norm_sums(self, x, B: int, rows: int, groups: int) -> torch.Tensor:
        x = self._act(x, "gn.x")
        assert x.is_contiguous() and x.shape[0] == B * rows
        ws = torch.empty(int(self.lib.a3d_group_norm_ws_floats(B, rows, groups)), dtype=torch.float32, device=self.device)
        sums = torch.empty((B, groups, 2), dtype=torch.float64, device=self.device)
        _check(self.lib.a3d_group_norm_sums_bf16(self._stream(), _p(x), _p(ws), _p(sums), B, rows, x.shape[1], groups),
               f"a3d_group_norm_sums_bf16 B={B} rows={rows} C={x.shape[1]}")
        return sums

    def group_norm_apply(self, x, B: int, rows: int, gamma, beta, groups: int, stats: torch.Tensor, silu: bool):
        x = self._act(x, "gn.x")
        assert x.is_contiguous() and x.shape[0] == B * rows
        assert stats.dtype == torch.float32 and stats.is_contiguous() and stats.shape == (B, groups, 2)
        y = self.empty(x.shape[0], x.shape[1])
        _check(self.lib.a3d_group_norm_apply_bf16(self._stream(), _p(x), _p(y), _p(gamma), _p(beta), _p(stats), B, rows, x.shape[1], groups,
                                                  1 if silu else 0), f"a3d_group_norm_apply_bf16 B={B} rows={rows} C={x.shape[1]}")
        return y

    def layer_norm(self, x, gamma, beta, eps: float, pe1=None, pe1_div: int = 1, pe2=None, pe2_div: int = 1, two: bool = False):
        x = self._act(x, "ln.x")
        assert x.is_contiguous()
        M, C = x.shape
        y1 = self.empty(M, C)
        y2 = self.empty(M, C) if two else None
        for pe in (pe1, pe2):
            if pe is not None:
                self._act(pe, "ln.pe")
                assert pe.is_contiguous() and pe.shape[1] == C
        rc = self.lib.a3d_layer_norm_bf16(self._stream(), _p(x), _p(y1), _p(y2), _p(gamma), _p(beta), M, C, eps,
                                          _p(pe1), pe1_div, pe1.shape[0] if pe1 is not None else 1,
                                          _p(pe2), pe2_div, pe2.shape[0] if pe2 is not None else 1)
        _check(rc, f"a3d_layer_norm_bf16 M={M} C={C}")
        return (y1, y2) if two else y1

    def geglu(self, x):
        x = self._act(x, "geglu.x")
        M, N2 = x.shape
        y = self.empty(M, N2 // 2)
        _check(self.lib.a3d_geglu_bf16(self._stream(), _p(x), x.stride(0), _p(y), y.stride(0), M, N2 // 2), "a3d_geglu_bf16")
        return y

    def silu(self, x):
        x = self._act(x, "silu.x")
        assert x.is_contiguous()
        y = torch.empty_like(x)
        _check(self.lib.a3d_silu_bf16(self._stream(), _p(x), _p(y), x.numel()), "a3d_silu_bf16")
        return y

    def activation(self, x, kind: str):
        x = self._act(x, "act.x")
        assert x.is_contiguous()
        y = torch.empty_like(x)
        _check(self.lib.a3d_activation_bf16(self._stream(), _p(x), _p(y), x.numel(), {"silu": 0, "quick_gelu": 1, "gelu": 2}[kind]), f"a3d_activation {kind}")
        return y

    def concat(self, a, b):
        a, b = self._act(a, "concat.a"), self._act(b, "concat.b")
        assert a.is_contiguous() and b.is_contiguous() and a.shape[0] == b.shape[0]
        y = self.empty(a.shape[0], a.shape[1] + b.shape[1])
        _check(self.lib.a3d_concat_bf16(self._stream(), _p(a), a.shape[1], _p(b), b.shape[1], _p(y), a.shape[0]), "a3d_concat_bf16")
        return y

    def timestep_embed(self, t: torch.Tensor, dim: int):
        assert t.dtype == torch.float32 and t.is_cuda and t.dim() == 1
        y = self.empty(t.shape[0], dim)
        _check(self.lib.a3d_timestep_embed_bf16(self._stream(), _p(t), _p(y), t.shape[0], dim), "a3d_timestep_embed_bf16")
        return y

    def im2col_in(self, sample: torch.Tensor):
        assert sample.is_cuda and sample.dim() == 5 and sample.dtype in _DTYPE_CODE
        sample = sample.contiguous()
        V, C, F, H, W = sample.shape
        y = self.empty(V * F * H * W, 64)
        _check(self.lib.a3d_im2col_in(self._stream(), _p(sample), _DTYPE_CODE[sample.dtype], _p(y), V, C, F, H, W), "a3d_im2col_in")
        return y

    def unpack_out(self, x, V: int, C: int, F: int, H: int, W: int, dtype: torch.dtype):
        x = self._act(x, "unpack.x")
        assert x.is_contiguous() and x.shape == (V * F * H * W, C)
        y = torch.empty((V, C, F, H, W), dtype=dtype, device=self.device)
        _check(self.lib.a3d_unpack_out(self._stream(), _p(x), _p(y), _DTYPE_CODE[dtype], V, C, F, H, W), "a3d_unpack_out")
        return y

    def gemm_f32out(self, x, w, bias=None, alpha: float = 1.0):
        x, w = self._act(x, "gemm_f32out.x"), self._act(w, "gemm_f32out.w")
        M, K = x.shape
        N = w.shape[0]
        assert x.stride(1) == 1 and w.stride(1) == 1 and w.shape[1] == K
        y = torch.empty((M, N), dtype=torch.float32, device=x.device)
        _check(self.lib.a3d_gemm_f32out_bf16(self._stream(), _p(x), x.stride(0), _p(w), w.stride(0), _p(bias), _p(y), N, M, N, K, alpha),
               f"a3d_gemm_f32out M={M} N={N} K={K}")
        return y

    def softmax_rows(self, x, out=None):
        assert x.dtype == torch.float32 and x.is_contiguous() and x.is_cuda
        M, N = x.shape
        y = self._act(out, "softmax_rows.out") if out is not None else self.empty(M, N)
        assert y.shape == (M, N)
        _check(self.lib.a3d_softmax_rows_f32_bf16(self._stream(), _p(x), N, _p(y), y.stride(0), M, N), f"a3d_softmax_rows_f32_bf16 M={M} N={N}")
        return y

    def channel_mix(self, x, w, bias, scale: float = 1.0):
        assert x.dtype == torch.float32 and x.is_contiguous() and x.is_cuda
        B, Cin, H, W = x.shape
        Cout = w.shape[0]
        w = w.to(device=x.device, dtype=torch.float32).contiguous()
        b = None if bias is None else bias.to(device=x.device, dtype=torch.float32).contiguous()
        y = torch.empty((B, Cout, H, W), dtype=torch.float32, device=x.device)
        _check(self.lib.a3d_channel_mix_f32(self._stream(), _p(x), _p(w), _p(b), _p(y), B, Cin, Cout, H * W, scale), "a3d_channel_mix_f32")
        return y

    def im2col_in_bwd(self, dcol, V: int, C: int, F: int, H: int, W: int, scale: float = 1.0):
        dcol = self._act(dcol, "im2col_in_bwd.dcol")
        assert dcol.is_contiguous() and dcol.shape == (V * F * H * W, 64)
        dx = torch.empty((V, C, F, H, W), dtype=torch.float32, device=self.device)
        _check(self.lib.a3d_im2col_in_bwd(self._stream(), _p(dcol), _p(dx), V, C, F, H, W, scale), f"a3d_im2col_in_bwd V={V} C={C} F={F} H={H} W={W}")
        return dx

    def softmax_rows_bwd(self, p, dp, alpha: float = 1.0, out=None):
        p = self._act(p, "softmax_rows_bwd.p")
        assert dp.dtype == torch.float32 and dp.is_cuda and dp.stride(1) == 1 and dp.shape == p.shape
        M, N = p.shape
        y = self._act(out, "softmax_rows_bwd.out") if out is not None else self.empty(M, N)
        assert y.shape == (M, N)
        _check(self.lib.a3d_softmax_rows_bwd_bf16(self._stream(), _p(p), p.stride(0), _p(dp), dp.stride(0), _p(y), y.stride(0), M, N, alpha),
               f"a3d_softmax_rows_bwd M={M} N={N}")
        return y

    def flash_attn_bwd(self, q, k, v, do, qmap: RowMap, kmap: RowMap, groups: int, heads: int, q_len: int, kv_len: int, *,
                       q_per_kv: int = 1, do_scale: float = 1.0, need_dq: bool = True, need_dkv: bool = True, o=None, lse=None,
                       dq_out=None, dk_out=None, dv_out=None, accumulate: bool = False):
        q, k, v, do = self._act(q, "attn_bwd.q"), self._act(k, "attn_bwd.k"), self._act(v, "attn_bwd.v"), self._act(do, "attn_bwd.do")
        C = q.shape[1]
        D = C // heads
        assert k.stride(0) == v.stride(0) and do.shape == q.shape
        def grad_buf(out, rows, covered):
            if out is not None:
                assert out.shape == (rows, C) and out.stride(1) == 1 and out.dtype == self.act_dtype and out.stride(0) % 8 == 0 and out.data_ptr() % 16 == 0
                if not covered and not accumulate:
                    out.zero_()
                return out
            return self.empty(rows, C) if covered else torch.zeros((rows, C), dtype=self.act_dtype, device=self.device)
        assert (dk_out is None) == (dv_out is None)
        if accumulate:
            assert (dq_out is not None or not need_dq) and (dk_out is not None or not need_dkv), "accumulate adds into dq_out / dk_out / dv_out"
        flags = 1 if accumulate else 0
        dq = grad_buf(dq_out, q.shape[0], q.shape[0] == groups * q_len) if need_dq else None
        kv_covered = need_dkv and self._kv_map_covers(kmap, groups, q_per_kv, kv_len, k.shape[0])
        dk = grad_buf(dk_out, k.shape[0], kv_covered) if need_dkv else None
        dv = grad_buf(dv_out, k.shape[0], kv_covered) if need_dkv else None
        assert dk is None or dk.stride(0) == dv.stride(0)
        qm, km, dom = qmap.c(q.stride(0)), kmap.c(k.stride(0)), qmap.c(do.stride(0))
        dqm, dkm = qmap.c(dq.stride(0) if dq is not None else C), kmap.c(dk.stride(0) if dk is not None else C)
        if lse is not None:
            assert o is not None and lse.dtype == torch.float32 and lse.is_contiguous() and lse.numel() == groups * heads * q_len
            o = self._act(o, "attn_bwd.o")
            lse2, delta = lse, torch.empty(groups * heads * q_len, dtype=torch.float32, device=self.device)
            om = qmap.c(o.stride(0))
            rc = self.lib.a3d_attn_delta_bf16(self._stream(), _p(do), _p(o), ctypes.byref(dom), ctypes.byref(om), _p(delta), groups, heads, D, q_len)
            _check(rc, f"a3d_attn_delta_bf16 groups={groups} heads={heads} D={D} q_len={q_len}")
            flags |= 2
        else:
            stats = torch.empty((2, groups * heads * q_len), dtype=torch.float32, device=self.device)
            lse2, delta = stats[0], stats[1]
        def run(dq_, dk_, dv_, dkm_, share, fl):
            rc = self.lib.a3d_flash_attn_bwd_bf16(self._stream(), _p(q), _p(k), _p(v), _p(do), _p(dq_), _p(dk_), _p(dv_), _p(lse2), _p(delta),
                                                  ctypes.byref(qm), ctypes.byref(km), ctypes.byref(dom), ctypes.byref(dqm), ctypes.byref(dkm_),
                                                  groups, heads, D, q_len, kv_len, share, float(D) ** -0.5, do_scale, fl)
            _check(rc, f"a3d_flash_attn_bwd_bf16 groups={groups} heads={heads} D={D} q_len={q_len} kv_len={kv_len} q_per_kv={share}")

        wgs_shared = (groups // q_per_kv) * heads * ((kv_len + 127) // 128)
        if need_dkv and q_per_kv > 1 and wgs_shared < 512:
            if need_dq:
                run(dq, None, None, dkm, q_per_kv, flags)
            pk = self.empty(groups * kv_len, C)
            pv = self.empty(groups * kv_len, C)
            run(None, pk, pv, RowMap(1, kv_len, 0, kv_len, 0).c(C), 1, (flags & 2) | (2 if need_dq else 0))
            idx = self._shared_kv_rows(kmap, groups, q_per_kv, kv_len)
            put = dk.index_add_ if accumulate else dk.index_copy_
            put(0, idx, pk.view(groups // q_per_kv, q_per_kv, kv_len, C).sum(dim=1).view(-1, C))
            put = dv.index_add_ if accumulate else dv.index_copy_
            put(0, idx, pv.view(groups // q_per_kv, q_per_kv, kv_len, C).sum(dim=1).view(-1, C))
            return dq, dk, dv
        run(dq, dk, dv, dkm, q_per_kv, flags)
        return dq, dk, dv

    def _kv_map_covers(self, kmap: RowMap, groups: int, q_per_kv: int, kv_len: int, rows: int) -> bool:
        key = (kmap.gdiv, kmap.ga, kmap.gb, kmap.seg_len, kmap.seg_stride, groups, q_per_kv, kv_len, rows)
        hit = self._kv_cover_cache.get(key)
        if hit is None:
            hit = self._kv_cover_cache[key] = rowmap_covers(kmap, groups, q_per_kv, kv_len, rows, "cpu")
        return hit

    def _shared_kv_rows(self, kmap: RowMap, groups: int, q_per_kv: int, kv_len: int) -> torch.Tensor:
        key = (kmap.gdiv, kmap.ga, kmap.gb, kmap.seg_len, kmap.seg_stride, groups, q_per_kv, kv_len)
        cache = self._kv_row_cache
        if key not in cache:
            cache[key] = rowmap_rows(kmap, groups, q_per_kv, kv_len, self.device)
        return cache[key]

    def temporal_attn_bwd(self, q, k, v, do, videos: int, frames: int, L: int, heads: int):
        q, k, v, do = self._act(q, "tattn_bwd.q"), self._act(k, "tattn_bwd.k"), self._act(v, "tattn_bwd.v"), self._act(do, "tattn_bwd.do")
        C = q.shape[1]
        assert q.stride(0) == k.stride(0) == v.stride(0)
        d = self.empty(q.shape[0], 3 * C)
        rc = self.lib.a3d_temporal_attn_bwd_bf16(self._stream(), _p(q), _p(k), _p(v), q.stride(0), _p(do), do.stride(0),
                                                 _p(d), d.data_ptr() + 2 * C, d.data_ptr() + 4 * C, 3 * C,
                                                 videos, frames, L, heads, C // heads, float(C // heads) ** -0.5)
        _check(rc, f"a3d_temporal_attn_bwd_bf16 videos={videos} frames={frames} L={L} C={C}")
        return d

    def layer_norm_bwd(self, x, dy, gamma, eps: float, need_param: bool = True):
        x, dy = self._act(x, "ln_bwd.x"), self._act(dy, "ln_bwd.dy")
        assert x.is_contiguous() and dy.is_contiguous() and x.shape == dy.shape
        M, C = x.shape
        dx = self.empty(M, C)
        dg = torch.empty(C, dtype=torch.float32, device=self.device) if need_param else None
        db = torch.empty(C, dtype=torch.float32, device=self.device) if need_param else None
        _check(self.lib.a3d_layer_norm_bwd_bf16(self._stream(), _p(x), _p(dy), _p(gamma), _p(dx), _p(dg), _p(db), M, C, eps, 0),
               f"a3d_layer_norm_bwd_bf16 M={M} C={C}")
        return dx, dg, db

    def group_norm_stats(self, x, B: int, rows: int, groups: int, eps: float) -> torch.Tensor:
        sums = self.group_norm_sums(x, B, rows, groups)
        m = sums / float(rows * (x.shape[1] // groups))
        mean = m[..., 0]
        rstd = torch.addcmul(m[..., 1], mean, mean, value=-1.0).clamp_min_(0.0).add_(eps).rsqrt_()
        return torch.stack([mean, rstd], dim=-1).to(torch.float32)

    def group_norm_bwd(self, x, dy, B: int, rows: int, gamma, beta, groups: int, stats, silu: bool, need_param: bool = False):
        x, dy = self._act(x, "gn_bwd.x"), self._act(dy, "gn_bwd.dy")
        assert x.is_contiguous() and dy.is_contiguous() and x.shape == dy.shape and x.shape[0] == B * rows
        C = x.shape[1]
        dx = self.empty(x.shape[0], C)
        ws = torch.empty(B * C * 2, dtype=torch.float32, device=self.device)
        dg = torch.zeros(C, dtype=torch.float32, device=self.device) if need_param else None
        db = torch.zeros(C, dtype=torch.float32, device=self.device) if need_param else None
        _check(self.lib.a3d_group_norm_bwd_bf16(self._stream(), _p(x), _p(dy), _p(gamma), _p(beta), _p(stats), _p(dx), _p(ws), _p(dg), _p(db),
                                                B, rows, C, groups, 1 if silu else 0), f"a3d_group_norm_bwd_bf16 B={B} rows={rows} C={C}")
        return dx, dg, db

    def geglu_bwd(self, proj_il, dy):
        proj_il, dy = self._act(proj_il, "geglu_bwd.p"), self._act(dy, "geglu_bwd.dy")
        M, N2 = proj_il.shape
        dp = self.empty(M, N2)
        _check(self.lib.a3d_geglu_bwd_bf16(self._stream(), _p(proj_il), proj_il.stride(0), _p(dy), dy.stride(0), _p(dp), N2, M, N2 // 2),
               f"a3d_geglu_bwd_bf16 M={M} N={N2 // 2}")
        return dp

    def transpose(self, x, pad: int = 64):
        x = self._act(x, "transpose.x")
        rows, cols = x.shape
        rp = (rows + pad - 1) // pad * pad
        y = self.empty(cols, rp)
        _check(self.lib.a3d_transpose_bf16(self._stream(), _p(x), x.stride(0), _p(y), rp, rows, cols, rp), f"a3d_transpose_bf16 {rows}x{cols}")
        return y

    def wgrad(self, dy, x, alpha: float = 1.0):
        dy, x = self._act(dy, "wgrad.dy"), self._act(x, "wgrad.x")
        assert dy.shape[0] == x.shape[0]
        M, N, K = dy.shape[0], dy.shape[1], x.shape[1]
        dw = torch.empty((N, K), dtype=torch.float32, device=self.device)
        ws = torch.empty(int(self.raw_lib.a3d_wgrad_ws_floats(M, N, K)), dtype=torch.float32, device=self.device)
        _check(self.lib.a3d_wgrad_bf16(self._stream(), _p(dy), dy.stride(0), _p(x), x.stride(0), _p(dw), K, _p(ws), M, N, K, alpha, 0),
               f"a3d_wgrad_bf16 M={M} N={N} K={K}")
        return dw

    def colsum(self, x, alpha: float = 1.0):
        x = self._act(x, "colsum.x")
        out = torch.empty(x.shape[1], dtype=torch.float32, device=self.device)
        _check(self.lib.a3d_colsum_bf16(self._stream(), _p(x), x.stride(0), x.shape[0], x.shape[1], _p(out), alpha, 0), "a3d_colsum_bf16")
        return out

    def axpby_(self, x, y, a: float = 1.0, b: float = 1.0):
        x, y = self._act(x, "axpby.x"), self._act(y, "axpby.y")
        assert x.is_contiguous() and y.is_contiguous() and x.shape == y.shape
        _check(self.lib.a3d_axpby_bf16(self._stream(), _p(x), _p(y), x.numel(), a, b), "a3d_axpby_bf16")
        return y

    def scaled(self, x, a: float):
        return self.axpby_(x, torch.empty_like(x), a, 0.0)

    def zero_insert2x(self, dy, B: int, H: int, W: int):
        dy = self._act(dy, "zero_insert.dy")
        assert dy.is_contiguous() and dy.shape[0] == B * ((H - 1) // 2 + 1) * ((W - 1) // 2 + 1)
        z = self.empty(B * H * W, dy.shape[1])
        _check(self.lib.a3d_zero_insert2x_bf16(self._stream(), _p(dy), _p(z), B, H, W, dy.shape[1]), "a3d_zero_insert2x_bf16")
        return z

    def upsample2x_bwd(self, du, B: int, H: int, W: int, He: int, We: int):
        du = self._act(du, "upsample_bwd.du")
        assert du.is_contiguous() and du.shape[0] == B * He * We
        dx = self.empty(B * H * W, du.shape[1])
        _check(self.lib.a3d_upsample2x_bwd_bf16(self._stream(), _p(du), _p(dx), B, H, W, He, We, du.shape[1]), "a3d_upsample2x_bwd_bf16")
        return dx

    def sqnorm(self, g: torch.Tensor, out: Optional[torch.Tensor] = None, accumulate: bool = False):
        assert g.dtype == torch.float32 and g.is_contiguous()
        out = out if out is not None else torch.empty(1, dtype=torch.float32, device=self.device)
        _check(self.raw_lib.a3d_sqnorm_f32(self._stream(), _p(g), g.numel(), _p(out), 1 if accumulate else 0), "a3d_sqnorm_f32")
        return out

    def clip_ctrl(self, sq: torch.Tensor, max_norm: float, inv_loss_scale: float = 1.0):
        ctrl = torch.empty(3, dtype=torch.float32, device=self.device)
        _check(self.raw_lib.a3d_clip_ctrl_f32(self._stream(), _p(sq), max_norm, inv_loss_scale, _p(ctrl)), "a3d_clip_ctrl_f32")
        return ctrl

    def adamw_(self, p, g, m, v, *, lr: float, betas=(0.9, 0.999), eps: float = 1e-8, weight_decay: float = 1e-2, step: int = 1, ctrl=None):
        for t in (p, g, m, v):
            assert t.dtype == torch.float32 and t.is_contiguous() and t.numel() == p.numel()
        b1, b2 = betas
        _check(self.raw_lib.a3d_adamw_f32(self._stream(), _p(p), _p(g), _p(m), _p(v), p.numel(), lr, b1, b2, eps, weight_decay,
                                          1.0 - b1 ** step, 1.0 - b2 ** step, _p(ctrl)), "a3d_adamw_f32")
        return p

    def cfg_ddim_step(self, eps_pair, x, first_frame, guidance: float, alpha_t: float, alpha_prev: float):
        for t in (eps_pair, x, first_frame):
            assert t.is_cuda and t.dtype == torch.float32 and t.is_contiguous()
        n, C, F, H, W = x.shape
        assert eps_pair.shape == (2 * n, C, F, H, W) and first_frame.numel() == n * C * H * W
        y = torch.empty_like(x)
        _check(self.lib.a3d_cfg_ddim_step_f32(self._stream(), _p(eps_pair), _p(x), _p(first_frame), _p(y), n, C, F, H * W,
                                              guidance, alpha_t, alpha_prev), "a3d_cfg_ddim_step_f32")
        return y
```

### include/animate3d_hip.h

```cpp
#ifndef ANIMATE3D_HIP_H
#define ANIMATE3D_HIP_H

#include <stdint.h>

#ifdef __cplusplus
extern "C" {
#endif

typedef void* a3d_stream_t;

enum {
  A3D_OK = 0,
  A3D_EINVAL = -1,
  A3D_EUNSUPPORTED = -2
};

enum { A3D_F32 = 0, A3D_BF16 = 1, A3D_F16 = 2 };

const char* a3d_version(void);

typedef struct a3d_rowmap {
  int64_t gdiv, ga, gb;
  int64_t seg_len, seg_stride;
  int64_t ld;
} a3d_rowmap;

#define A3D_GEMM_RESERVED_CUS_MASK 0xff
#define A3D_GEMM_KERNEL_MASK 0x300
#define A3D_GEMM_TILE128 0x100
#define A3D_GEMM_RING 0x200
#define A3D_GEMM_DIRECT 0x300
int a3d_gemm_bf16(a3d_stream_t stream, const void* X, int64_t ldx, const void* W, int64_t ldw,
                  const float* bias, const void* rowbias, int64_t rb_div, const void* R, int64_t ldr,
                  void* Y, int64_t ldy, int64_t M, int64_t N, int64_t K, float alpha, float beta, int flags);

int a3d_gemm_ws_bf16(a3d_stream_t stream, const void* X, int64_t ldx, const void* W, int64_t ldw,
                     const float* bias, const void* rowbias, int64_t rb_div, const void* R, int64_t ldr,
                     void* Y, int64_t ldy, int64_t M, int64_t N, int64_t K, float alpha, float beta, int flags,
                     void* ws, int64_t ws_bytes, int64_t* ws_needed);

int a3d_gemm2_bf16(a3d_stream_t stream, const void* X, int64_t ldx, const void* X2, int64_t ldx2, int64_t K1,
                   const void* W, int64_t ldw, const float* bias, void* Y, int64_t ldy, int64_t M, int64_t N, int64_t K, int flags);

int a3d_gemm_f32out_bf16(a3d_stream_t stream, const void* X, int64_t ldx, const void* W, int64_t ldw,
                         const float* bias, float* Y, int64_t ldy, int64_t M, int64_t N, int64_t K, float alpha);

int a3d_gemm_geglu_bf16(a3d_stream_t stream, const void* X, int64_t ldx, const void* W, int64_t ldw,
                        const float* bias, void* Y, int64_t ldy, int64_t M, int64_t N2, int64_t K, int flags);

int a3d_conv3x3_bf16(a3d_stream_t stream, const void* X, const void* Wp, const float* bias,
                     const void* rowbias, int64_t rb_div, const void* R, void* Y,
                     int B, int H, int W, int Cin, int Cout, int stride, int up2x, int flags);

int a3d_conv3x3_ws_bf16(a3d_stream_t stream, const void* X, const void* Wp, const float* bias,
                        const void* rowbias, int64_t rb_div, const void* R, void* Y,
                        int B, int H, int W, int Cin, int Cout, int stride, int up2x, int flags,
                        void* ws, int64_t ws_bytes, int64_t* ws_needed);

#define A3D_ATTN_ACCUMULATE 1
#define A3D_ATTN_CAUSAL 2
#define A3D_ATTN_EXACT 4
#define A3D_ATTN_PLAIN 8
int a3d_flash_attn_bf16(a3d_stream_t stream, const void* Q, const void* K, const void* V, void* O,
                        const a3d_rowmap* qmap, const a3d_rowmap* kmap, const a3d_rowmap* omap,
                        int groups, int heads, int head_dim, int64_t q_len, int64_t kv_len,
                        float scale, float out_scale, int accumulate);

int a3d_flash_attn_counted_bf16(a3d_stream_t stream, const void* Q, const void* K, const void* V, void* O,
                                const a3d_rowmap* qmap, const a3d_rowmap* kmap, const a3d_rowmap* omap,
                                int groups, int heads, int head_dim, int64_t q_len, int64_t kv_len,
                                float scale, float out_scale, int accumulate, unsigned int* counters);

int a3d_flash_attn2_bf16(a3d_stream_t stream, const void* Q, const void* K, const void* V, const void* K2, const void* V2, void* O,
                         const a3d_rowmap* qmap, const a3d_rowmap* kmap, const a3d_rowmap* kmap2, const a3d_rowmap* omap,
                         int groups, int heads, int head_dim, int64_t q_len, int64_t kv_len, int64_t kv_len2,
                         float scale, float out_scale, float out_scale2, int accumulate);

int a3d_temporal_attn_bf16(a3d_stream_t stream, const void* Q, const void* K, const void* V, int64_t ldqkv,
                           void* O, int64_t ldo, int videos, int frames, int64_t L, int heads,
                           int head_dim, float scale);

int a3d_temporal_attn_sharded_bf16(a3d_stream_t stream, const void* Q, int64_t ldq, const void* K, const void* V, int64_t ldkv,
                                   void* O, int64_t ldo, int videos, int frames, int64_t L, int heads,
                                   int head_dim, float scale, int q_f0, int q_frames, int kv_frames_per_block,
                                   int64_t kv_block_stride);

int64_t a3d_group_norm_ws_floats(int B, int64_t rows, int groups);
int a3d_group_norm_bf16(a3d_stream_t stream, const void* X, void* Y, const float* gamma, const float* beta,
                        float* ws, int B, int64_t rows, int C, int groups, float eps, int silu);

int a3d_group_norm2_bf16(a3d_stream_t stream, const void* Xa, int Ca, const void* Xb, int Cb, void* Y, const float* gamma,
                         const float* beta, float* ws, int B, int64_t rows, int groups, float eps, int silu);

int a3d_group_norm_sums_bf16(a3d_stream_t stream, const void* X, float* ws, double* sums, int B, int64_t rows, int C, int groups);
int a3d_group_norm_apply_bf16(a3d_stream_t stream, const void* X, void* Y, const float* gamma, const float* beta,
                              const float* stats, int B, int64_t rows, int C, int groups, int silu);

int a3d_layer_norm_bf16(a3d_stream_t stream, const void* X, void* Y1, void* Y2, const float* gamma,
                        const float* beta, int64_t M, int C, float eps,
                        const void* pe1, int64_t pe1_div, int64_t pe1_mod,
                        const void* pe2, int64_t pe2_div, int64_t pe2_mod);

int a3d_geglu_bf16(a3d_stream_t stream, const void* X, int64_t ldx, void* Y, int64_t ldy, int64_t M, int64_t N);

int a3d_silu_bf16(a3d_stream_t stream, const void* X, void* Y, int64_t n);

int a3d_activation_bf16(a3d_stream_t stream, const void* X, void* Y, int64_t n, int mode);

int a3d_concat_bf16(a3d_stream_t stream, const void* A, int64_t Ca, const void* Bsrc, int64_t Cb, void* Y, int64_t M);

int a3d_timestep_embed_bf16(a3d_stream_t stream, const float* t, void* Y, int V, int dim);

int a3d_im2col_in(a3d_stream_t stream, const void* sample, int dtype, void* Y, int V, int C, int F, int H, int W);

int a3d_im2col_in_bwd(a3d_stream_t stream, const void* dCol, float* dX, int V, int C, int F, int H, int W, float scale);

int a3d_unpack_out(a3d_stream_t stream, const void* X, void* Y, int dtype, int V, int C, int F, int H, int W);

int a3d_softmax_rows_f32_bf16(a3d_stream_t stream, const float* X, int64_t ldx, void* Y, int64_t ldy, int64_t M, int64_t N);

int a3d_softmax_rows_bwd_bf16(a3d_stream_t stream, const void* P, int64_t ldp, const float* dP, int64_t lddp, void* dS, int64_t ldds,
                              int64_t M, int64_t N, float alpha);

int a3d_channel_mix_f32(a3d_stream_t stream, const float* X, const float* W, const float* bias, float* Y,
                        int B, int Cin, int Cout, int64_t HW, float scale);

int a3d_cfg_ddim_step_f32(a3d_stream_t stream, const float* eps_pair, const float* x, const float* first_frame,
                          float* x_prev, int64_t n, int C, int F, int64_t HW, float guidance,
                          float alpha_t, float alpha_prev);



int a3d_flash_attn_bwd_bf16(a3d_stream_t stream, const void* Q, const void* K, const void* V, const void* dO,
                            void* dQ, void* dK, void* dV, float* lse2, float* delta,
                            const a3d_rowmap* qmap, const a3d_rowmap* kmap, const a3d_rowmap* domap,
                            const a3d_rowmap* dqmap, const a3d_rowmap* dkmap,
                            int groups, int heads, int head_dim, int64_t q_len, int64_t kv_len, int q_per_kv,
                            float scale, float do_scale, int accumulate);

int a3d_flash_attn_lse_bf16(a3d_stream_t stream, const void* Q, const void* K, const void* V, void* O,
                            const a3d_rowmap* qmap, const a3d_rowmap* kmap, const a3d_rowmap* omap,
                            int groups, int heads, int head_dim, int64_t q_len, int64_t kv_len,
                            float scale, float out_scale, int accumulate, float* lse2);
int a3d_attn_delta_bf16(a3d_stream_t stream, const void* dO, const void* O, const a3d_rowmap* domap, const a3d_rowmap* omap,
                        float* delta, int groups, int heads, int head_dim, int64_t q_len);

int a3d_temporal_attn_bwd_bf16(a3d_stream_t stream, const void* Q, const void* K, const void* V, int64_t ldqkv,
                               const void* dO, int64_t lddo, void* dQ, void* dK, void* dV, int64_t ldd,
                               int videos, int frames, int64_t L, int heads, int head_dim, float scale);

int a3d_layer_norm_bwd_bf16(a3d_stream_t stream, const void* X, const void* dY, const float* gamma, void* dX,
                            float* dgamma, float* dbeta, int64_t M, int C, float eps, int accumulate);

int a3d_group_norm_bwd_bf16(a3d_stream_t stream, const void* X, const void* dY, const float* gamma, const float* beta,
                            const float* stats, void* dX, float* ws, float* dgamma, float* dbeta,
                            int B, int64_t rows, int C, int groups, int silu);

int a3d_geglu_bwd_bf16(a3d_stream_t stream, const void* P, int64_t ldp, const void* dY, int64_t lddy, void* dP, int64_t lddp,
                       int64_t M, int64_t N);

int a3d_transpose_bf16(a3d_stream_t stream, const void* X, int64_t ldx, void* Y, int64_t ldy, int64_t rows, int64_t cols,
                       int64_t rows_pad);

int64_t a3d_wgrad_ws_floats(int64_t M, int64_t N, int64_t K);
int a3d_wgrad_bf16(a3d_stream_t stream, const void* dY, int64_t lddy, const void* X, int64_t ldx, float* dW, int64_t lddw,
                   float* ws, int64_t M, int64_t N, int64_t K, float alpha, int accumulate);

int a3d_colsum_bf16(a3d_stream_t stream, const void* X, int64_t ldx, int64_t rows, int64_t cols, float* out, float alpha, int accumulate);

int a3d_axpby_bf16(a3d_stream_t stream, const void* X, void* Y, int64_t n, float a, float b);

int a3d_zero_insert2x_bf16(a3d_stream_t stream, const void* dY, void* Z, int B, int H, int W, int C);

int a3d_upsample2x_bwd_bf16(a3d_stream_t stream, const void* dU, void* dX, int B, int H, int W, int He, int We, int C);

int a3d_sqnorm_f32(a3d_stream_t stream, const float* g, int64_t n, float* out, int accumulate);
int a3d_clip_ctrl_f32(a3d_stream_t stream, const float* sqnorm, float max_norm, float inv_loss_scale, float* ctrl);
int a3d_adamw_f32(a3d_stream_t stream, float* p, const float* g, float* m, float* v, int64_t n, float lr, float beta1, float beta2,
                  float eps, float weight_decay, float bias_corr1, float bias_corr2, const float* ctrl);

int a3d_gs_preprocess_f32(a3d_stream_t stream, int B, int N, const float* means, int64_t means_bs, const float* scales, int64_t scales_bs,
                          const float* rots, int64_t rots_bs, const float* opac, int64_t opac_bs, const float* shs, int64_t shs_bs, int M,
                          int deg, const float* colors, int64_t colors_bs, const float* view, const float* proj, const float* campos,
                          const float* tanfovx, const float* tanfovy, int H, int W, float scale_mod, int* radii, float* xy, float* depth,
                          float* conic_o, float* rgb, int* clamped, int* tiles_touched);
int a3d_gs_duplicate_f32(a3d_stream_t stream, int B, int N, int H, int W, const float* xy, const float* depth, const int* radii,
                         const int64_t* offsets, int64_t* keys, int* vals);
int a3d_gs_tile_ranges_f32(a3d_stream_t stream, const int64_t* keys, int64_t L, int* ranges, int64_t n_tiles);
int a3d_gs_render_f32(a3d_stream_t stream, int B, int N, int H, int W, const int* ranges, const int64_t* perm, const int* vals,
                      const float* xy, const float* conic_o, const float* rgb, const float* depth, const float* bg,
                      float* out_img, float* out_depth, float* out_alpha, float* T_final, int* n_contrib);
int a3d_gs_render_bwd_f32(a3d_stream_t stream, int B, int N, int H, int W, const int* ranges, const int64_t* perm, const int* vals,
                          const float* xy, const float* conic_o, const float* rgb, const float* depth, const float* bg,
                          const float* T_final, const int* n_contrib, const float* d_img, const float* d_depth,
                          const float* d_alpha, float* rows);
int a3d_gs_preprocess_bwd_f32(a3d_stream_t stream, int B, int N, const float* means, int64_t means_bs, const float* scales, int64_t scales_bs,
                              const float* rots, int64_t rots_bs, const float* opac, int64_t opac_bs, const float* shs, int64_t shs_bs, int M,
                              int deg, const float* colors, int64_t colors_bs, const float* view, const float* proj, const float* campos,
                              const float* tanfovx, const float* tanfovy, int H, int W, float scale_mod, const int* radii,
                              const int* clamped, const int64_t* offsets, const int* tiles_touched, const float* rows,
                              float* d_means2d, float* d_means, float* d_scales, float* d_rots, float* d_opac, float* d_shs,
                              float* d_colors);
int a3d_gs_sum_batch_f32(a3d_stream_t stream, const float* src, float* dst, int B, int64_t M);

int a3d_dg_cells_f32(a3d_stream_t stream, int N, const float* xyz, const int64_t* plane_desc, int* cells);
int64_t a3d_dg_mean_partials(int N);
int a3d_dg_forward_f32(a3d_stream_t stream, int T, int N, int B, const float* xyz, const float* scaling, const float* rotation,
                       const float* timestamps, const float* grid, const int64_t* plane_desc, const float* weights, int flags,
                       const int* img_start, const int* img_list, float* sp, float* mpart, float* gmean, float* glob, float* means,
                       float* scales, float* rots);
int64_t a3d_dg_backward_ws_floats(int T, int N, const int64_t* plane_desc);
int a3d_dg_backward_f32(a3d_stream_t stream, int T, int N, int B, const float* xyz, const float* scaling, const float* rotation,
                        const float* timestamps, const float* grid, const int64_t* plane_desc, const float* weights, int flags,
                        const int* img_start, const int* img_list, const float* sp, const float* gmean, const float* glob,
                        const int* order, const int* starts, const float* d_means, const float* d_scales, const float* d_rots,
                        float* ws, float* d_grid, float* d_weights, float* d_scaling, float* d_rotation);

int a3d_knn_f32(a3d_stream_t stream, int N, const float* points, int K, int least_edge_num, float radius2, int* nn_idx, float* nn_dist);
int a3d_arap_energy_f32(a3d_stream_t stream, int F, int Nv, int K, int S, const float* source, const float* targets, int64_t targets_bs,
                        const int* nn_idx, const float* weight, const int* sample_idx, double* rot, float* rot_f32, double* energy,
                        float* loss);
int a3d_arap_backward_f32(a3d_stream_t stream, int F, int Nv, int K, int S, const float* source, const float* targets, int64_t targets_bs,
                          const int* nn_idx, const float* weight, const int* sample_idx, const double* rot, const int* order,
                          const int* starts, const float* grad_out, float* d_targets, float* d_source);

int a3d_gemm_f16(a3d_stream_t stream, const void* X, int64_t ldx, const void* W, int64_t ldw,
                  const float* bias, const void* rowbias, int64_t rb_div, const void* R, int64_t ldr,
                  void* Y, int64_t ldy, int64_t M, int64_t N, int64_t K, float alpha, float beta, int flags);
int a3d_gemm_ws_f16(a3d_stream_t stream, const void* X, int64_t ldx, const void* W, int64_t ldw,
                    const float* bias, const void* rowbias, int64_t rb_div, const void* R, int64_t ldr,
                    void* Y, int64_t ldy, int64_t M, int64_t N, int64_t K, float alpha, float beta, int flags,
                    void* ws, int64_t ws_bytes, int64_t* ws_needed);
int a3d_gemm2_f16(a3d_stream_t stream, const void* X, int64_t ldx, const void* X2, int64_t ldx2, int64_t K1,
                  const void* W, int64_t ldw, const float* bias, void* Y, int64_t ldy, int64_t M, int64_t N, int64_t K, int flags);
int a3d_gemm_f32out_f16(a3d_stream_t stream, const void* X, int64_t ldx, const void* W, int64_t ldw,
                         const float* bias, float* Y, int64_t ldy, int64_t M, int64_t N, int64_t K, float alpha);
int a3d_gemm_geglu_f16(a3d_stream_t stream, const void* X, int64_t ldx, const void* W, int64_t ldw,
                        const float* bias, void* Y, int64_t ldy, int64_t M, int64_t N2, int64_t K, int flags);
int a3d_conv3x3_f16(a3d_stream_t stream, const void* X, const void* Wp, const float* bias,
                     const void* rowbias, int64_t rb_div, const void* R, void* Y,
                     int B, int H, int W, int Cin, int Cout, int stride, int up2x, int flags);
int a3d_conv3x3_ws_f16(a3d_stream_t stream, const void* X, const void* Wp, const float* bias,
                       const void* rowbias, int64_t rb_div, const void* R, void* Y,
                       int B, int H, int W, int Cin, int Cout, int stride, int up2x, int flags,
                       void* ws, int64_t ws_bytes, int64_t* ws_needed);
int a3d_flash_attn_f16(a3d_stream_t stream, const void* Q, const void* K, const void* V, void* O,
                        const a3d_rowmap* qmap, const a3d_rowmap* kmap, const a3d_rowmap* omap,
                        int groups, int heads, int head_dim, int64_t q_len, int64_t kv_len,
                        float scale, float out_scale, int accumulate);
int a3d_flash_attn_counted_f16(a3d_stream_t stream, const void* Q, const void* K, const void* V, void* O,
                               const a3d_rowmap* qmap, const a3d_rowmap* kmap, const a3d_rowmap* omap,
                               int groups, int heads, int head_dim, int64_t q_len, int64_t kv_len,
                               float scale, float out_scale, int accumulate, unsigned int* counters);
int a3d_flash_attn2_f16(a3d_stream_t stream, const void* Q, const void* K, const void* V, const void* K2, const void* V2, void* O,
                        const a3d_rowmap* qmap, const a3d_rowmap* kmap, const a3d_rowmap* kmap2, const a3d_rowmap* omap,
                        int groups, int heads, int head_dim, int64_t q_len, int64_t kv_len, int64_t kv_len2,
                        float scale, float out_scale, float out_scale2, int accumulate);
int a3d_temporal_attn_f16(a3d_stream_t stream, const void* Q, const void* K, const void* V, int64_t ldqkv,
                           void* O, int64_t ldo, int videos, int frames, int64_t L, int heads,
                           int head_dim, float scale);
int a3d_temporal_attn_sharded_f16(a3d_stream_t stream, const void* Q, int64_t ldq, const void* K, const void* V, int64_t ldkv,
                                   void* O, int64_t ldo, int videos, int frames, int64_t L, int heads,
                                   int head_dim, float scale, int q_f0, int q_frames, int kv_frames_per_block,
                                   int64_t kv_block_stride);
int a3d_group_norm_f16(a3d_stream_t stream, const void* X, void* Y, const float* gamma, const float* beta,
                        float* ws, int B, int64_t rows, int C, int groups, float eps, int silu);
int a3d_group_norm2_f16(a3d_stream_t stream, const void* Xa, int Ca, const void* Xb, int Cb, void* Y, const float* gamma,
                        const float* beta, float* ws, int B, int64_t rows, int groups, float eps, int silu);
int a3d_group_norm_sums_f16(a3d_stream_t stream, const void* X, float* ws, double* sums, int B, int64_t rows, int C, int groups);
int a3d_group_norm_apply_f16(a3d_stream_t stream, const void* X, void* Y, const float* gamma, const float* beta,
                              const float* stats, int B, int64_t rows, int C, int groups, int silu);
int a3d_layer_norm_f16(a3d_stream_t stream, const void* X, void* Y1, void* Y2, const float* gamma,
                        const float* beta, int64_t M, int C, float eps,
                        const void* pe1, int64_t pe1_div, int64_t pe1_mod,
                        const void* pe2, int64_t pe2_div, int64_t pe2_mod);
int a3d_geglu_f16(a3d_stream_t stream, const void* X, int64_t ldx, void* Y, int64_t ldy, int64_t M, int64_t N);
int a3d_silu_f16(a3d_stream_t stream, const void* X, void* Y, int64_t n);
int a3d_activation_f16(a3d_stream_t stream, const void* X, void* Y, int64_t n, int mode);
int a3d_concat_f16(a3d_stream_t stream, const void* A, int64_t Ca, const void* Bsrc, int64_t Cb, void* Y, int64_t M);
int a3d_timestep_embed_f16(a3d_stream_t stream, const float* t, void* Y, int V, int dim);
int a3d_im2col_in_f16(a3d_stream_t stream, const void* sample, int dtype, void* Y, int V, int C, int F, int H, int W);
int a3d_unpack_out_f16(a3d_stream_t stream, const void* X, void* Y, int dtype, int V, int C, int F, int H, int W);
int a3d_softmax_rows_f32_f16(a3d_stream_t stream, const float* X, int64_t ldx, void* Y, int64_t ldy, int64_t M, int64_t N);
int a3d_softmax_rows_bwd_f16(a3d_stream_t stream, const void* P, int64_t ldp, const float* dP, int64_t lddp, void* dS, int64_t ldds,
                             int64_t M, int64_t N, float alpha);
int a3d_im2col_in_bwd_f16(a3d_stream_t stream, const void* dCol, float* dX, int V, int C, int F, int H, int W, float scale);
int a3d_flash_attn_bwd_f16(a3d_stream_t stream, const void* Q, const void* K, const void* V, const void* dO,
                            void* dQ, void* dK, void* dV, float* lse2, float* delta,
                            const a3d_rowmap* qmap, const a3d_rowmap* kmap, const a3d_rowmap* domap,
                            const a3d_rowmap* dqmap, const a3d_rowmap* dkmap,
                            int groups, int heads, int head_dim, int64_t q_len, int64_t kv_len, int q_per_kv,
                            float scale, float do_scale, int accumulate);
int a3d_flash_attn_lse_f16(a3d_stream_t stream, const void* Q, const void* K, const void* V, void* O,
                           const a3d_rowmap* qmap, const a3d_rowmap* kmap, const a3d_rowmap* omap,
                           int groups, int heads, int head_dim, int64_t q_len, int64_t kv_len,
                           float scale, float out_scale, int accumulate, float* lse2);
int a3d_attn_delta_f16(a3d_stream_t stream, const void* dO, const void* O, const a3d_rowmap* domap, const a3d_rowmap* omap,
                       float* delta, int groups, int heads, int head_dim, int64_t q_len);
int a3d_temporal_attn_bwd_f16(a3d_stream_t stream, const void* Q, const void* K, const void* V, int64_t ldqkv,
                               const void* dO, int64_t lddo, void* dQ, void* dK, void* dV, int64_t ldd,
                               int videos, int frames, int64_t L, int heads, int head_dim, float scale);
int a3d_layer_norm_bwd_f16(a3d_stream_t stream, const void* X, const void* dY, const float* gamma, void* dX,
                            float* dgamma, float* dbeta, int64_t M, int C, float eps, int accumulate);
int a3d_group_norm_bwd_f16(a3d_stream_t stream, const void* X, const void* dY, const float* gamma, const float* beta,
                            const float* stats, void* dX, float* ws, float* dgamma, float* dbeta,
                            int B, int64_t rows, int C, int groups, int silu);
int a3d_geglu_bwd_f16(a3d_stream_t stream, const void* P, int64_t ldp, const void* dY, int64_t lddy, void* dP, int64_t lddp,
                       int64_t M, int64_t N);
int a3d_transpose_f16(a3d_stream_t stream, const void* X, int64_t ldx, void* Y, int64_t ldy, int64_t rows, int64_t cols,
                       int64_t rows_pad);
int a3d_colsum_f16(a3d_stream_t stream, const void* X, int64_t ldx, int64_t rows, int64_t cols, float* out, float alpha, int accumulate);
int a3d_axpby_f16(a3d_stream_t stream, const void* X, void* Y, int64_t n, float a, float b);
int a3d_zero_insert2x_f16(a3d_stream_t stream, const void* dY, void* Z, int B, int H, int W, int C);
int a3d_upsample2x_bwd_f16(a3d_stream_t stream, const void* dU, void* dX, int B, int H, int W, int He, int We, int C);
int a3d_wgrad_f16(a3d_stream_t stream, const void* dY, int64_t lddy, const void* X, int64_t ldx, float* dW, int64_t lddw,
                   float* ws, int64_t M, int64_t N, int64_t K, float alpha, int accumulate);

#ifdef __cplusplus
}
#endif
#endif
```

Measured before the change: 2.379 denoise-steps/s.

## Restructure head-dim-80 flash attention kernel with 16x16 MFMA and configurable wavefronts

Replaces the default head-dim-80 direct-to-LDS flash attention kernel with a template over wavefront count. Each wave now processes 64 query rows as two 32-row subtiles, and the PV product uses 16x16 MFMA with permlane16 swaps. The LDS ring shrinks from 5 to 3 tiles, and per-lane DMA source offsets move into an LDS table to cut register use. The previous kernel stays available behind a new 'narrow' flag, and a WG512 flag picks the wider variant. The aim is better occupancy and data reuse for the 4096-token self-attention, at the cost of shallower prefetch and a risk of new scheduling stalls.

```diff
diff --git a/animate3d_amd/csrc/flash_attn.hip b/animate3d_amd/csrc/flash_attn.hip
--- a/animate3d_amd/csrc/flash_attn.hip
+++ b/animate3d_amd/csrc/flash_attn.hip
@@ -539,7 +539,7 @@
   p.Q = (const uint16_t*)Q; p.K = (const uint16_t*)K; p.V = (const uint16_t*)V; p.O = (uint16_t*)O;
   p.qm = *qmap; p.km = *kmap; p.om = *omap;
   p.heads = heads; p.q_len = (int)q_len; p.kv_len = (int)kv_len;
-  if (accumulate & ~(A3D_ATTN_ACCUMULATE | A3D_ATTN_CAUSAL | A3D_ATTN_EXACT | A3D_ATTN_PLAIN)) return A3D_EINVAL;
+  if (accumulate & ~(A3D_ATTN_ACCUMULATE | A3D_ATTN_CAUSAL | A3D_ATTN_EXACT | A3D_ATTN_PLAIN | A3D_ATTN_DM80_NARROW | A3D_ATTN_DM80_WG512)) return A3D_EINVAL;
   p.scale_log2 = scale * 1.4426950408889634f; p.out_scale = out_scale; p.accumulate = accumulate & 1; p.causal = (accumulate >> 1) & 1;
   const bool exact = (accumulate & A3D_ATTN_EXACT) != 0, plain = (accumulate & A3D_ATTN_PLAIN) != 0;
   p.lse = lse;
@@ -559,7 +559,8 @@
       break;
     case 80:
       if (!plain && aligned && kv_len % 64 == 0 && kv_len >= 512 && q_len >= 256) {
-        if (int rc = A3D_FN(a3d_launch_flash_dm80)(exact ? 0 : 1, groups, s, p)) return rc;
+        if (int rc = (accumulate & A3D_ATTN_DM80_NARROW) ? A3D_FN(a3d_launch_flash_dm80_narrow)(exact ? 0 : 1, groups, s, p)
+                                                         : A3D_FN(a3d_launch_flash_dm80)((exact ? 0 : 1) | ((accumulate & A3D_ATTN_DM80_WG512) ? 2 : 0), groups, s, p)) return rc;
         break;
       }
       if (q_len >= 2048 && kv_len >= 2048) { launch<80, 32, 2, OFS_FMA>(aligned, groups, s, p); break; }
diff --git a/animate3d_amd/csrc/flash_attn_dm80.hip b/animate3d_amd/csrc/flash_attn_dm80.hip
--- a/animate3d_amd/csrc/flash_attn_dm80.hip
+++ b/animate3d_amd/csrc/flash_attn_dm80.hip
@@ -2,38 +2,41 @@
 
 namespace {
 
-constexpr int E_ROWB = 160;
-constexpr int E_UNITB = 32 * E_ROWB;
-constexpr int E_KB = 2 * E_UNITB;
-constexpr int E_TILEB = 2 * E_KB;
-constexpr int E_RING = 5;
-constexpr int E_CV = E_RING * E_TILEB + 32;
-constexpr int E_CV_BYTES = 2752;
-constexpr int E_SAMPLE = E_CV + E_CV_BYTES;
-constexpr int E_SMEM_BYTES = E_SAMPLE + E_UNITB;
-constexpr float E_L_BAD = 1.2676506e30f;
+constexpr int W_D = 80, W_KS = 5, W_MB = 5;
+constexpr int W_ROWB = 2 * W_D;
+constexpr int W_CPR = W_D / 8;
+constexpr int W_UNITB = 32 * W_ROWB;
+constexpr int W_KB = 2 * W_UNITB;
+constexpr int W_TILEB = 2 * W_KB;
+constexpr int W_RING = 3;
+constexpr int W_BLOCKS = 2 * W_CPR;
+constexpr int W_SAMPLE = W_RING * W_TILEB;
+constexpr int W_SBLOCKS = W_CPR / 2;
+constexpr float W_L_HI = 1.2676506e30f;
 #ifdef A3D_STORAGE_F16
-constexpr float E_BIAS = F16_BIAS;
-constexpr bool E_SAMPLED = true;
+constexpr float W_BIAS = F16_BIAS;
+constexpr bool W_SAMPLED = true;
+constexpr float W_L_LO = 1.220703125e-4f;
+constexpr int W_TAB = W_SAMPLE + W_UNITB;
 #else
-constexpr float E_BIAS = 40.f;
-constexpr bool E_SAMPLED = false;
+constexpr float W_BIAS = 40.f;
+constexpr bool W_SAMPLED = false;
+constexpr float W_L_LO = 7.8886091e-31f;
+constexpr int W_TAB = W_SAMPLE;
 #endif
-
-#ifdef A3D_EXP_R5_PATHS
-constexpr bool E_EARLY_DMA = false;
-#else
-constexpr bool E_EARLY_DMA = true;
-#endif
-
-extern __shared__ __attribute__((aligned(16))) uint8_t e_smem[];
-A3D_DEV u32x4_t e_lds128(uint32_t off) { return *reinterpret_cast<const u32x4_t*>(e_smem + off); }
-A3D_DEV u32x2_t e_ldstr(uint32_t off) { return lds_tr16_b64(reinterpret_cast<const uint16_t*>(e_smem + off)); }
-
-template <int FLAGS>
-__global__ __launch_bounds__(512, 2) void flash_attn_dm80_kernel(const AttnParams p) {
-  constexpr int D = 80, KS = 5, MT = 3, NT = 512, BQ = 256;
-  constexpr int NEXP = 16, NCVT = 8, NDMA = 3;
+A3D_DEV int w_kswz(int row) { return (row >> 3) & 1; }
+A3D_DEV int w_vkey(int r) { return 16 * ((r >> 2) & 1) + 8 * (r >> 4) + 4 * ((r >> 3) & 1) + (r & 3); }
+
+extern __shared__ __attribute__((aligned(16))) uint8_t w_smem[];
+A3D_DEV u32x4_t w_lds128(uint32_t off) { return *reinterpret_cast<const u32x4_t*>(w_smem + off); }
+A3D_DEV u32x2_t w_ldstr(uint32_t off) { return lds_tr16_b64(reinterpret_cast<const uint16_t*>(w_smem + off)); }
+
+template <int FLAGS, int NW>
+__global__ __launch_bounds__(64 * NW, 2) void flash_attn_dm80_kernel(const AttnParams p) {
+  constexpr int D = W_D, KS = W_KS, MB = W_MB, NT = 64 * NW, BQ = 64 * NW;
+  constexpr int NDMA = (W_BLOCKS + NW - 1) / NW;
+  constexpr int NSMP = (W_SBLOCKS + NW - 1) / NW;
+  constexpr int NEXP = 32, NCVT = 16;
   constexpr bool TRY_NOMAX = (FLAGS & 1) != 0;
 
   const int tid = threadIdx.x, lane = tid & 63, wid = tid >> 6;
@@ -43,12 +46,7 @@
   const int qt = blockIdx.x / p.heads;
   const int64_t grp = blockIdx.y;
   const int64_t hoff = (int64_t)head * D;
-  const uint32_t lds0 = fa_lds_addr(e_smem);
-
-  for (int i = tid; i < E_CV_BYTES / 2; i += NT) {
-    const int vb = 2 * i;
-    reinterpret_cast<uint16_t*>(e_smem + E_CV)[i] = (vb == 0 || vb == 160 || vb == 2560 || vb == 2720) ? ONE16 : (uint16_t)0;
-  }
+  const uint32_t lds0 = fa_lds_addr(w_smem);
 
   const int64_t ld = p.km.ld;
   const int64_t kgbase = map_group_base(p.km, grp);
@@ -56,186 +54,243 @@
   const int64_t tile_step = (int64_t)64 * ld;
   const int64_t wrap_step = (p.km.seg_stride - p.km.seg_len) * ld;
   auto slot_src = [&](int slot) -> uint32_t {
-    const bool isk = slot < 640;
-    const int s2 = isk ? slot : slot - 640;
-    const int prow = s2 / 10, cpos = s2 % 10;
-    const int c = isk ? (cpos ^ ((prow >> 3) & 1)) : cpos;
-    const int key = isk ? prow : ((prow & ~7) | (((prow & 7) >> 1) + 4 * (prow & 1)));
+    if (slot >= 64 * W_BLOCKS) slot = lane;
+    const bool isk = slot < 64 * W_CPR;
+    const int s2 = isk ? slot : slot - 64 * W_CPR;
+    const int prow = s2 / W_CPR, cpos = s2 % W_CPR;
+    const int c = isk ? (cpos ^ w_kswz(prow)) : cpos;
+    const int key = isk ? prow : ((prow & ~31) | w_vkey(prow & 31));
     return (uint32_t)(((int64_t)key * ld + c * 8) * 2);
   };
-  const uint32_t voffA = slot_src(64 * w + lane);
-  const uint32_t voffB = slot_src(512 + 64 * w + lane);
-  const uint32_t voffC = slot_src(1024 + 32 * w + l31);
-  uint32_t voffS = 0;
-  if constexpr (E_SAMPLED) {
-    const int ss = (64 * w + lane) % 320, prow = ss / 10;
-    const int64_t key = (int64_t)prow * (p.kv_len / 32);
-    voffS = (uint32_t)((map_seq(p.km, key) * ld + ((ss % 10) ^ ((prow >> 3) & 1)) * 8) * 2);
+#pragma unroll
+  for (int i = 0; i < NDMA; ++i) *reinterpret_cast<uint32_t*>(w_smem + W_TAB + (i * NT + tid) * 4) = slot_src(64 * (NW * i + w) + lane);
+  auto tab = [&](int I) __attribute__((always_inline)) -> uint32_t {
+    const uint32_t ln = __builtin_amdgcn_mbcnt_hi(~0u, __builtin_amdgcn_mbcnt_lo(~0u, 0u));
+    return *reinterpret_cast<const uint32_t*>(w_smem + (ln * 4u + (uint32_t)(W_TAB + I * NT * 4 + w * 256)));
+  };
+  uint32_t voffS[NSMP];
+#pragma unroll
+  for (int i = 0; i < NSMP; ++i) {
+    voffS[i] = 0u;
+    if constexpr (W_SAMPLED) {
+      const int ss = (64 * (NW * i + w) + lane) % (32 * W_CPR), prow = ss / W_CPR;
+      const int64_t key = (int64_t)prow * (p.kv_len / 32);
+      voffS[i] = (uint32_t)((map_seq(p.km, key) * ld + ((ss % W_CPR) ^ w_kswz(prow)) * 8) * 2);
+    }
   }
-  const uint64_t maskS = w < 5 ? ~0ull : 0ull;
 
   const int krow = kperm(l31);
-  const uint32_t klane = (uint32_t)(krow * E_ROWB + 16 * (g ^ ((krow >> 3) & 1)));
-  const int c4 = i16 & 3;
-  const uint32_t vrow = (uint32_t)((8 * (q4 >> 1) + 2 * (i16 >> 2)) * E_ROWB);
-  const uint32_t vlane01 = vrow + (uint32_t)(2 * (16 * (q4 & 1) + 4 * c4));
-  const bool v2_data = (q4 & 1) == 0;
-  const uint32_t vlane2 = v2_data ? vrow + (uint32_t)(2 * (64 + 4 * c4)) : (c4 == 0 ? (uint32_t)E_CV : (uint32_t)(E_CV + 8));
-  uint32_t vmul = v2_data ? 1u : 0u;
-  asm volatile("" : "+v"(vmul));
-
-  const uint16_t* gA = nullptr;
-  const uint16_t* gB = nullptr;
-  const uint16_t* gC = nullptr;
+  const uint32_t klane = (uint32_t)(krow * W_ROWB + 16 * (g ^ w_kswz(krow)));
+  const uint32_t vlane = (uint32_t)((16 * (q4 >> 1) + 4 * (q4 & 1) + (i16 >> 2)) * W_ROWB + 8 * (i16 & 3));
+
+  const uint16_t* gK = nullptr;
+  const uint16_t* gV = nullptr;
   uint32_t seg_off = 0;
   auto dma_reset = [&]() __attribute__((always_inline)) {
-    gA = dm_scalar(p.K + hoff + kgbase * ld);
-    gB = dm_scalar((w < 2 ? p.K : p.V) + hoff + kgbase * ld);
-    gC = dm_scalar(p.V + hoff + kgbase * ld);
+    gK = dm_scalar(p.K + hoff + kgbase * ld);
+    gV = dm_scalar(p.V + hoff + kgbase * ld);
     seg_off = 0;
   };
-  auto tile_base = [&](int tile) __attribute__((always_inline)) -> uint32_t { return (uint32_t)((tile % E_RING) * E_TILEB); };
-  auto dma_a = [&](int tile) __attribute__((always_inline)) { dm_glds16(voffA, gA, lds0 + tile_base(tile) + 1024 * w); };
-  auto dma_b = [&](int tile) __attribute__((always_inline)) { dm_glds16(voffB, gB, lds0 + tile_base(tile) + 8192 + 1024 * w); };
-  auto dma_c = [&](int tile) __attribute__((always_inline)) {
-    dm_glds16_m(voffC, gC, lds0 + tile_base(tile) + 16384 + 512 * w, 0xffffffffull);
-    seg_off += 64;
-    int64_t stp = tile_step;
-    if (seg_off >= seg_len) { stp += wrap_step; seg_off = 0; }
-    gA += stp; gB += stp; gC += stp;
+  auto tile_base = [&](int tile) __attribute__((always_inline)) -> uint32_t { return (uint32_t)((tile % W_RING) * W_TILEB); };
+  auto dma_i = [&](int tile, auto i_c, uint32_t vo) __attribute__((always_inline)) {
+    constexpr int I = decltype(i_c)::value;
+    const int b = NW * I + w;
+    const uint16_t* src = b < W_CPR ? gK : gV;
+    if constexpr (NW * I + NW - 1 < W_BLOCKS) {
+      dm_glds16(vo, src, lds0 + tile_base(tile) + 1024u * (uint32_t)b);
+    } else {
+      const bool on = b < W_BLOCKS;
+      dm_glds16_m(vo, src, lds0 + tile_base(tile) + 1024u * (uint32_t)(on ? b : 0), on ? ~0ull : 0ull);
+    }
+    if constexpr (I == NDMA - 1) {
+      seg_off += 64;
+      int64_t stp = tile_step;
+      if (seg_off >= seg_len) { stp += wrap_step; seg_off = 0; }
+      gK += stp; gV += stp;
+    }
+  };
+  auto dma_tile = [&](int tile) __attribute__((always_inline)) {
+    static_for<NDMA>([&](auto i_c) __attribute__((always_inline)) { dma_i(tile, i_c, tab(decltype(i_c)::value)); });
   };
   auto prologue_issue = [&]() __attribute__((always_inline)) {
     dma_reset();
-    if constexpr (E_SAMPLED && TRY_NOMAX)
-      dm_glds16_m(voffS, dm_scalar(p.K + hoff + kgbase * ld), lds0 + (uint32_t)(E_SAMPLE + 1024 * (w < 5 ? w : 0)), maskS);
-    dma_a(0); dma_b(0); dma_c(0);
-    dma_a(1); dma_b(1); dma_c(1);
-    dma_a(2); dma_b(2); dma_c(2);
-  };
-  auto prologue_wait = [&]() __attribute__((always_inline)) { asm volatile("s_waitcnt vmcnt(%0)\n\ts_barrier" :: "i"(NDMA) : "memory"); };
-  if constexpr (E_EARLY_DMA) prologue_issue();
-
-  const int q_idx = qt * BQ + wid * 32 + l31;
-  u32x4_t qf[KS];
-  {
+    if constexpr (W_SAMPLED && TRY_NOMAX) {
+#pragma unroll
+      for (int i = 0; i < NSMP; ++i) {
+        const int b = NW * i + w;
+        const bool on = b < W_SBLOCKS;
+        dm_glds16_m(voffS[i], dm_scalar(p.K + hoff + kgbase * ld), lds0 + (uint32_t)(W_SAMPLE + 1024 * (on ? b : 0)), on ? ~0ull : 0ull);
+      }
+    }
+    dma_tile(0);
+    dma_tile(1);
+  };
+  auto prologue_wait = [&]() __attribute__((always_inline)) { asm volatile("s_waitcnt vmcnt(0)\n\ts_barrier" ::: "memory"); };
+  prologue_issue();
+
+  const int q_base = qt * BQ + wid * 64;
+  u32x4_t qf[2][KS];
+#pragma unroll
+  for (int qs = 0; qs < 2; ++qs) {
+    const int q_idx = q_base + 32 * qs + l31;
     const int64_t q_row = map_row(p.qm, grp, q_idx < p.q_len ? q_idx : p.q_len - 1);
 #pragma unroll
     for (int ks = 0; ks < KS; ++ks) {
       u32x4_t wq = *reinterpret_cast<const u32x4_t*>(p.Q + q_row * p.qm.ld + hoff + 16 * ks + 8 * g);
 #pragma unroll
       for (int j = 0; j < 4; ++j) wq[j] = pack16(lo16(wq[j]) * p.scale_log2, hi16(wq[j]) * p.scale_log2);
-      qf[ks] = wq;
+      qf[qs][ks] = wq;
     }
   }
 
-
-  f32x16_t oacc[MT];
-  f32x16_t minit;
+  f32x4_t oacc[MB][4];
   u32x4_t kf[KS];
-  u32x4_t vf[MT][2];
+  u32x4_t vf[MB];
+  float off[2] = {0.f, 0.f};
+  float lsum[2] = {0.f, 0.f};
+  auto read_k1 = [&](auto ks_c, uint32_t ka) __attribute__((always_inline)) {
+    constexpr int ks = decltype(ks_c)::value;
+    kf[ks] = w_lds128(ka + 32 * ks);
+  };
   auto read_k = [&](uint32_t koff) __attribute__((always_inline)) {
-    const uint32_t a = klane + koff;
-#pragma unroll
-    for (int ks = 0; ks < KS; ++ks) kf[ks] = e_lds128(a + 32 * ks);
-  };
-  auto read_vhalf = [&](auto i_c, uint32_t a01, uint32_t a2) __attribute__((always_inline)) {
-    constexpr int i = decltype(i_c)::value, h = i / 6, mt = (i / 2) % 3, rr = i % 2;
-    const u32x2_t t = e_ldstr((mt == 2 ? a2 : a01 + 64 * mt) + (16 * h + rr) * E_ROWB);
-    vf[mt][h][2 * rr] = t[0];
-    vf[mt][h][2 * rr + 1] = t[1];
-  };
-  auto read_v = [&](uint32_t voff) __attribute__((always_inline)) {
-    const uint32_t a01 = vlane01 + voff, a2 = __umul24(vmul, voff) + vlane2;
-    static_for<12>([&](auto i_c) __attribute__((always_inline)) { read_vhalf(i_c, a01, a2); });
-  };
-  auto pv_mfma = [&](auto i_c, u32x4_t (&P)[2]) __attribute__((always_inline)) {
-    constexpr int i = decltype(i_c)::value, h = i / 3, mt = i % 3;
-    oacc[mt] = mfma32(vf[mt][h], P[h], oacc[mt]);
+    uint32_t ka = klane + koff;
+    asm volatile("" : "+v"(ka));
+    static_for<KS>([&](auto ks_c) __attribute__((always_inline)) { read_k1(ks_c, ka); });
+  };
+  auto read_v1 = [&](auto i_c, uint32_t va) __attribute__((always_inline)) {
+    constexpr int i = decltype(i_c)::value, mb = i / 2, rr = i % 2;
+    const u32x2_t t = w_ldstr(va + 32 * mb + rr * 8 * W_ROWB);
+    vf[mb][2 * rr] = t[0];
+    vf[mb][2 * rr + 1] = t[1];
+  };
+  auto read_v = [&](uint32_t voff_) __attribute__((always_inline)) {
+    uint32_t va = vlane + voff_;
+    asm volatile("" : "+v"(va));
+    static_for<2 * MB>([&](auto i_c) __attribute__((always_inline)) { read_v1(i_c, va); });
+  };
+  auto pv_mfma = [&](auto i_c, u32x4_t (&P)[2][2]) __attribute__((always_inline)) {
+    constexpr int i = decltype(i_c)::value, mb = i / 4, nb = i % 4;
+    oacc[mb][nb] = mfma16(vf[mb], P[nb / 2][nb % 2], oacc[mb][nb]);
+  };
+  auto swap_p = [&](auto k_c, u32x4_t (&P)[2][2]) __attribute__((always_inline)) {
+    constexpr int k = decltype(k_c)::value, qs = k / 4, jj = k % 4;
+    const auto r = __builtin_amdgcn_permlane16_swap(P[qs][0][jj], P[qs][1][jj], false, false);
+    P[qs][0][jj] = r[0];
+    P[qs][1][jj] = r[1];
   };
   auto clear_o = [&]() __attribute__((always_inline)) {
 #pragma unroll
-    for (int mt = 0; mt < MT; ++mt)
-#pragma unroll
-      for (int r = 0; r < 16; ++r) oacc[mt][r] = 0.f;
-#pragma unroll
-    for (int r = 0; r < 16; ++r) minit[r] = 0.f;
+    for (int mb = 0; mb < MB; ++mb)
+#pragma unroll
+      for (int nb = 0; nb < 4; ++nb) oacc[mb][nb] = f32x4_t{0.f, 0.f, 0.f, 0.f};
+    lsum[0] = 0.f; lsum[1] = 0.f;
+  };
+  auto qk_scores = [&](f32x16_t (&s)[2]) __attribute__((always_inline)) {
+#pragma unroll
+    for (int qs = 0; qs < 2; ++qs) {
+#pragma unroll
+      for (int r = 0; r < 16; ++r) s[qs][r] = 0.f;
+#pragma unroll
+      for (int ks = 0; ks < KS; ++ks) s[qs] = mfma32(kf[ks], qf[qs][ks], s[qs]);
+    }
   };
   const int nt = p.kv_len / 64;
-  auto first_scores = [&](f32x16_t& s, float& m_off, float bias, uint32_t koff = 0u) __attribute__((always_inline)) -> bool {
+  [[maybe_unused]] const float cmax_sds = f16_expected_max_sds(p.kv_len);
+  auto first_scores = [&](f32x16_t (&s)[2], float bias, uint32_t koff) __attribute__((always_inline)) -> bool {
     read_k(koff);
-#pragma unroll
-    for (int r = 0; r < 16; ++r) s[r] = 0.f;
-#pragma unroll
-    for (int ks = 0; ks < KS; ++ks) s = mfma32(kf[ks], qf[ks], s);
-    float mx = s[0];
-#pragma unroll
-    for (int r = 1; r < 16; ++r) mx = fmaxf(mx, s[r]);
-    mx = fmaxf(mx, __shfl_xor(mx, 32));
+    qk_scores(s);
     bool wide = false;
-    if constexpr (E_SAMPLED) {
-      if (bias != 0.f) {
-        float sm = 0.f, sq = 0.f;
-#pragma unroll
-        for (int r = 0; r < 16; ++r) { sm += s[r]; sq = fmaf(s[r], s[r], sq); }
-        sm += __shfl_xor(sm, 32); sq += __shfl_xor(sq, 32);
-        const float mean = sm * (1.f / 32.f);
-        bias = f16_sampled_bias(mx, mean, sq * (1.f / 32.f) - mean * mean, f16_expected_max_sds(p.kv_len), wide);
-      }
-    }
-    m_off = mx + bias;
-#pragma unroll
-    for (int r = 0; r < 16; ++r) { s[r] -= m_off; minit[r] = -m_off; }
+#pragma unroll
+    for (int qs = 0; qs < 2; ++qs) {
+      float mx = s[qs][0];
+#pragma unroll
+      for (int r = 1; r < 16; ++r) mx = fmaxf(mx, s[qs][r]);
+      mx = fmaxf(mx, __shfl_xor(mx, 32));
+      float b = bias;
+      if constexpr (W_SAMPLED) {
+        if (bias != 0.f) {
+          float sm = 0.f, sq = 0.f;
+#pragma unroll
+          for (int r = 0; r < 16; ++r) { sm += s[qs][r]; sq = fmaf(s[qs][r], s[qs][r], sq); }
+          sm += __shfl_xor(sm, 32); sq += __shfl_xor(sq, 32);
+          const float mean = sm * (1.f / 32.f);
+          bool wq;
+          b = f16_sampled_bias(mx, mean, sq * (1.f / 32.f) - mean * mean, cmax_sds, wq);
+          wide = wide || wq;
+        }
+      }
+      off[qs] = mx + b;
+    }
     return wide;
   };
+  auto store4 = [&](uint16_t* dst, const f32x4_t& a, float inv) __attribute__((always_inline)) {
+    float v0 = a[0] * inv, v1 = a[1] * inv, v2 = a[2] * inv, v3 = a[3] * inv;
+    if (p.accumulate) {
+      const u32x2_t prev = *reinterpret_cast<const u32x2_t*>(dst);
+      v0 += lo16(prev[0]); v1 += hi16(prev[0]); v2 += lo16(prev[1]); v3 += hi16(prev[1]);
+    }
+    u32x2_t o;
+    o[0] = pack16(v0, v1);
+    o[1] = pack16(v2, v3);
+    *reinterpret_cast<u32x2_t*>(dst) = o;
+  };
   auto finish = [&](bool check) __attribute__((always_inline)) -> bool {
-    const float l_tot = __shfl(oacc[2][8], l31);
-    const bool bad = !(l_tot < E_L_BAD) || !(l_tot > 0.f);
+    float l_tot[2];
+#pragma unroll
+    for (int qs = 0; qs < 2; ++qs) l_tot[qs] = lsum[qs] + __shfl_xor(lsum[qs], 32);
     if (check) {
+      bool bad = false;
+#pragma unroll
+      for (int qs = 0; qs < 2; ++qs) bad = bad || !(l_tot[qs] < W_L_HI) || !(l_tot[qs] > W_L_LO);
+#ifdef A3D_STORAGE_F16
+      float chk = 0.f;
+#pragma unroll
+      for (int mb = 0; mb < MB; ++mb)
+#pragma unroll
+        for (int nb = 0; nb < 4; ++nb)
+#pragma unroll
+          for (int r = 0; r < 4; ++r) chk += fabsf(oacc[mb][nb][r]);
+      bad = bad || !(chk < 3.0e38f);
+#endif
       if (__syncthreads_or(bad ? 1 : 0)) { dm_count(p, 1); return false; }
     }
-    const float inv = p.out_scale / l_tot;
-    if (p.lse != nullptr && q_idx < p.q_len && g == 0)
-      p.lse[((int64_t)grp * p.heads + head) * p.q_len + q_idx] = __builtin_amdgcn_logf(l_tot) - minit[0];
-    if (q_idx < p.q_len) {
-      uint16_t* orow = p.O + map_row(p.om, grp, q_idx) * p.om.ld + hoff;
-      const bool wide_rows = E_EARLY_DMA && !p.accumulate && ((reinterpret_cast<uintptr_t>(p.O) | (uintptr_t)(p.om.ld * 2)) & 15u) == 0;
-      if (wide_rows) {
-#pragma unroll
-        for (int mt = 0; mt < MT; ++mt)
-#pragma unroll
-          for (int pr = 0; pr < 2; ++pr) {
-            if (32 * mt + 16 * pr >= D) continue;
-            u32x4_t v;
-#pragma unroll
-            for (int c = 0; c < 2; ++c) {
-              const uint32_t w0 = pack16(oacc[mt][8 * pr + 2 * c] * inv, oacc[mt][8 * pr + 2 * c + 1] * inv);
-              const uint32_t w1 = pack16(oacc[mt][8 * pr + 4 + 2 * c] * inv, oacc[mt][8 * pr + 4 + 2 * c + 1] * inv);
-              const auto r = __builtin_amdgcn_permlane32_swap(w0, w1, false, false);
-              v[c] = r[0];
-              v[2 + c] = r[1];
-            }
-            *reinterpret_cast<u32x4_t*>(orow + 32 * mt + 16 * pr + 8 * g) = v;
-          }
-      } else {
-#pragma unroll
-        for (int mt = 0; mt < MT; ++mt)
-#pragma unroll
-          for (int qd = 0; qd < 4; ++qd) {
-            const int d = 32 * mt + 8 * qd + 4 * g;
-            if (d < D) {
-              float v[4];
-#pragma unroll
-              for (int j = 0; j < 4; ++j) v[j] = oacc[mt][4 * qd + j] * inv;
-              if (p.accumulate) {
-                const u32x2_t prev = *reinterpret_cast<const u32x2_t*>(orow + d);
-                v[0] += lo16(prev[0]); v[1] += hi16(prev[0]); v[2] += lo16(prev[1]); v[3] += hi16(prev[1]);
-              }
-              u32x2_t o;
-              o[0] = pack16(v[0], v[1]);
-              o[1] = pack16(v[2], v[3]);
-              *reinterpret_cast<u32x2_t*>(orow + d) = o;
-            }
-          }
+    if (p.lse != nullptr && g == 0) {
+#pragma unroll
+      for (int qs = 0; qs < 2; ++qs) {
+        const int q_idx = q_base + 32 * qs + l31;
+        if (q_idx < p.q_len) p.lse[((int64_t)grp * p.heads + head) * p.q_len + q_idx] = __builtin_amdgcn_logf(l_tot[qs]) + off[qs];
+      }
+    }
+    float inv[4];
+#pragma unroll
+    for (int nb = 0; nb < 4; ++nb) inv[nb] = p.out_scale / __shfl(l_tot[nb / 2], 16 * (nb & 1) + i16);
+    const bool wide_rows = !p.accumulate && ((reinterpret_cast<uintptr_t>(p.O) | (uintptr_t)(p.om.ld * 2)) & 15u) == 0;
+    if (wide_rows) {
+#pragma unroll
+      for (int np = 0; np < 2; ++np) {
+        const int q_idx = q_base + 16 * (2 * np + (q4 & 1)) + i16;
+        uint16_t* orow = p.O + map_row(p.om, grp, q_idx < p.q_len ? q_idx : p.q_len - 1) * p.om.ld + hoff + 8 * (q4 >> 1);
+#pragma unroll
+        for (int mb = 0; mb < MB; ++mb) {
+          const f32x4_t& a = oacc[mb][2 * np];
+          const f32x4_t& b = oacc[mb][2 * np + 1];
+          const auto r0 = __builtin_amdgcn_permlane16_swap(pack16(a[0] * inv[2 * np], a[1] * inv[2 * np]),
+                                                           pack16(b[0] * inv[2 * np + 1], b[1] * inv[2 * np + 1]), false, false);
+          const auto r1 = __builtin_amdgcn_permlane16_swap(pack16(a[2] * inv[2 * np], a[3] * inv[2 * np]),
+                                                           pack16(b[2] * inv[2 * np + 1], b[3] * inv[2 * np + 1]), false, false);
+          const u32x4_t v{r0[0], r1[0], r0[1], r1[1]};
+          if (q_idx < p.q_len) *reinterpret_cast<u32x4_t*>(orow + 16 * mb) = v;
+        }
+      }
+    } else {
+#pragma unroll
+      for (int nb = 0; nb < 4; ++nb) {
+        const int q_idx = q_base + 16 * nb + i16;
+        if (q_idx < p.q_len) {
+          uint16_t* orow = p.O + map_row(p.om, grp, q_idx) * p.om.ld + hoff + 4 * q4;
+#pragma unroll
+          for (int mb = 0; mb < MB; ++mb) store4(orow + 16 * mb, oacc[mb][nb], inv[nb]);
+        }
       }
     }
     return true;
@@ -243,155 +298,176 @@
 
   auto run_fast = [&]() __attribute__((always_inline)) -> bool {
     clear_o();
-    f32x16_t sA, sB;
-    u32x4_t pA[2], pB[2];
-#pragma unroll
-    for (int h = 0; h < 2; ++h) { pA[h] = u32x4_t{0u, 0u, 0u, 0u}; pB[h] = u32x4_t{0u, 0u, 0u, 0u}; }
-
-    auto step = [&](auto do_qk_c, auto do_pv_c, f32x16_t& sCur, f32x16_t& sNext, u32x4_t (&pCur)[2], u32x4_t (&pPrev)[2],
+    f32x16_t sA[2], sB[2];
+    u32x4_t pA[2][2], pB[2][2];
+#pragma unroll
+    for (int qs = 0; qs < 2; ++qs)
+#pragma unroll
+      for (int h = 0; h < 2; ++h) { pA[qs][h] = u32x4_t{0u, 0u, 0u, 0u}; pB[qs][h] = u32x4_t{0u, 0u, 0u, 0u}; }
+
+    auto step = [&](auto do_qk_c, auto do_pv_c, f32x16_t (&sCur)[2], f32x16_t (&sNext)[2], u32x4_t (&pCur)[2][2], u32x4_t (&pPrev)[2][2],
                     uint32_t kOff, uint32_t vOff, auto&& hook) __attribute__((always_inline)) {
       constexpr bool DO_QK = decltype(do_qk_c)::value, DO_PV = decltype(do_pv_c)::value;
-      constexpr int NPV = DO_PV ? 2 * MT : 0, NQK = DO_QK ? KS : 0, NS = NPV + NQK;
-      constexpr int KSLOT = 2, VS0 = NPV + 1, VPS = 3;
-      const uint32_t va01 = vlane01 + vOff, va2 = __umul24(vmul, vOff) + vlane2;
+      constexpr int NPV = DO_PV ? 2 * MB : 0, NQK = DO_QK ? 2 * KS : 0, NS = NPV + NQK;
+      constexpr int KAHEAD = 5;
+      uint32_t va = vlane + vOff, ka = klane + kOff;
+      asm volatile("" : "+v"(va), "+v"(ka));
       float e[NEXP];
       auto do_cvt = [&](auto c_c) __attribute__((always_inline)) {
-        constexpr int c = decltype(c_c)::value, h = c / 4, jj = c % 4;
-        pCur[h][jj] = pack16(e[2 * c], e[2 * c + 1]);
+        constexpr int c = decltype(c_c)::value, qs = c / 8, h = (c / 4) % 2, jj = c % 4;
+        pCur[qs][h][jj] = pack16(e[2 * c], e[2 * c + 1]);
       };
       auto cdone = [](int s) constexpr { return s < 0 ? 0 : (NEXP * s / NS) / 2; };
       __builtin_amdgcn_sched_barrier(0);
       static_for<NS>([&](auto s_c) __attribute__((always_inline)) {
         constexpr int s = decltype(s_c)::value;
         if constexpr (s < NPV) {
-          pv_mfma(s_c, pPrev);
+          pv_mfma(std::integral_constant<int, 2 * s>{}, pPrev);
+          pv_mfma(std::integral_constant<int, 2 * s + 1>{}, pPrev);
         } else {
-          constexpr int ks = s - NPV;
-          if constexpr (ks == 0) sNext = mfma32(kf[0], qf[0], minit);
-          else sNext = mfma32(kf[ks], qf[ks], sNext);
+          constexpr int i = s - NPV, ks = i / 2, qs = i % 2;
+          if constexpr (ks == 0) {
+            f32x16_t z;
+#pragma unroll
+            for (int r = 0; r < 16; ++r) z[r] = 0.f;
+            sNext[qs] = mfma32(kf[0], qf[qs][0], z);
+          } else {
+            sNext[qs] = mfma32(kf[ks], qf[qs][ks], sNext[qs]);
+          }
         }
-        if constexpr (DO_QK && DO_PV && s == KSLOT) read_k(kOff);
-        if constexpr (DO_QK && s >= VS0 && VPS * (s - VS0) < 12) {
-          static_for<VPS>([&](auto i_c) __attribute__((always_inline)) {
-            constexpr int i = VPS * (s - VS0) + decltype(i_c)::value;
-            if constexpr (i < 12) read_vhalf(std::integral_constant<int, i>{}, va01, va2);
-          });
+        if constexpr (DO_QK) {
+          constexpr int tt = s - NPV + KAHEAD;
+          if constexpr (tt >= 0 && tt % 2 == 0 && tt / 2 < KS) read_k1(std::integral_constant<int, tt / 2>{}, ka);
+          if constexpr (s >= NPV) read_v1(std::integral_constant<int, s - NPV>{}, va);
         }
         hook(s_c);
         constexpr int E0 = NEXP * s / NS, E1 = NEXP * (s + 1) / NS;
         static_for<E1 - E0>([&](auto x_c) __attribute__((always_inline)) {
           constexpr int x = E0 + decltype(x_c)::value;
-          e[x] = __builtin_amdgcn_exp2f(sCur[x]);
+          e[x] = __builtin_amdgcn_exp2f(sCur[x / 16][x % 16] - off[x / 16]);
+          lsum[x / 16] += e[x];
         });
         constexpr int C0 = cdone(s - 1), C1 = cdone(s);
         static_for<C1 - C0>([&](auto c_c) __attribute__((always_inline)) { do_cvt(std::integral_constant<int, C0 + decltype(c_c)::value>{}); });
+        static_for<8>([&](auto k_c) __attribute__((always_inline)) {
+          constexpr int k = decltype(k_c)::value, need = (k / 4) * 8 + 4 + (k % 4);
+          if constexpr (need < cdone(s - 1) && !(need < cdone(s - 2))) swap_p(k_c, pCur);
+        });
         __builtin_amdgcn_sched_barrier(0);
       });
       {
         constexpr int C0 = cdone(NS - 1);
         static_for<NCVT - C0>([&](auto c_c) __attribute__((always_inline)) { do_cvt(std::integral_constant<int, C0 + decltype(c_c)::value>{}); });
+        static_for<8>([&](auto k_c) __attribute__((always_inline)) {
+          constexpr int k = decltype(k_c)::value, need = (k / 4) * 8 + 4 + (k % 4);
+          if constexpr (!(need < cdone(NS - 2))) swap_p(k_c, pCur);
+        });
       }
     };
 
-    if constexpr (!E_EARLY_DMA) prologue_issue();
     prologue_wait();
     {
-      float m_off;
-      if constexpr (E_SAMPLED) {
-        const bool wide = first_scores(sA, m_off, E_BIAS, (uint32_t)E_SAMPLE);
+      if constexpr (W_SAMPLED) {
+        const bool wide = first_scores(sA, W_BIAS, (uint32_t)W_SAMPLE);
         if (__syncthreads_count(wide ? 1 : 0) * 4 > NT) { dm_count(p, 0); return false; }
         read_k(0u);
-        sA = minit;
-#pragma unroll
-        for (int ks = 0; ks < KS; ++ks) sA = mfma32(kf[ks], qf[ks], sA);
+        qk_scores(sA);
       } else {
-        first_scores(sA, m_off, E_BIAS);
-      }
-      read_k((uint32_t)E_UNITB);
+        first_scores(sA, W_BIAS, 0u);
+      }
+      {
+        uint32_t ka = klane + (uint32_t)W_UNITB;
+        asm volatile("" : "+v"(ka));
+        static_for<3>([&](auto ks_c) __attribute__((always_inline)) { read_k1(ks_c, ka); });
+      }
     }
 
     auto iteration = [&](int t, auto first_c, auto last_c, auto dma_c_) __attribute__((always_inline)) {
       constexpr bool FIRST = decltype(first_c)::value, LAST = decltype(last_c)::value, DMA = decltype(dma_c_)::value;
+      [[maybe_unused]] uint32_t vo = 0u;
       auto even_hook = [&](auto s_c) __attribute__((always_inline)) {
-        if constexpr (DMA && decltype(s_c)::value == 1) dma_a(t + 3);
+        constexpr int s = decltype(s_c)::value;
+        if constexpr (DMA && s % 3 == 0 && s < 9 && s / 3 < NDMA) vo = tab(s / 3);
+        if constexpr (DMA && s % 3 == 1 && s < 9 && s / 3 < NDMA) dma_i(t + 2, std::integral_constant<int, s / 3>{}, vo);
       };
       auto odd_hook = [&](auto s_c) __attribute__((always_inline)) {
-        if constexpr (DMA && decltype(s_c)::value == 1) dma_b(t + 3);
-        if constexpr (DMA && decltype(s_c)::value == 4) dma_c(t + 3);
+        constexpr int s = decltype(s_c)::value;
+        if constexpr (DMA && s % 3 == 0 && s < 6 && 3 + s / 3 < NDMA) vo = tab(3 + s / 3);
+        if constexpr (DMA && s % 3 == 1 && s < 6 && 3 + s / 3 < NDMA) dma_i(t + 2, std::integral_constant<int, 3 + s / 3>{}, vo);
       };
       const uint32_t tb = tile_base(t), tn = tile_base(t + 1);
-      step(std::true_type{}, std::integral_constant<bool, !FIRST>{}, sA, sB, pA, pB, tb + E_UNITB, tb + E_KB, even_hook);
-      step(std::integral_constant<bool, !LAST>{}, std::true_type{}, sB, sA, pB, pA, tn, tb + E_KB + E_UNITB, odd_hook);
-      if constexpr (!LAST) {
-        if constexpr (DMA) asm volatile("s_waitcnt vmcnt(%0)\n\ts_barrier" :: "i"(NDMA) : "memory");
-        else asm volatile("s_waitcnt vmcnt(0)\n\ts_barrier" ::: "memory");
-      }
+      step(std::true_type{}, std::integral_constant<bool, !FIRST>{}, sA, sB, pA, pB, tb + W_UNITB, tb + W_KB, even_hook);
+      step(std::integral_constant<bool, !LAST>{}, std::true_type{}, sB, sA, pB, pA, tn, tb + W_KB + W_UNITB, odd_hook);
+      if constexpr (!LAST) asm volatile("s_waitcnt vmcnt(0)\n\ts_barrier" ::: "memory");
     };
     constexpr std::true_type Y{};
     constexpr std::false_type N{};
     iteration(0, Y, N, Y);
-    for (int t = 1; t < nt - 3; ++t) iteration(t, N, N, Y);
-    iteration(nt - 3, N, N, N);
+    for (int t = 1; t < nt - 2; ++t) iteration(t, N, N, Y);
     iteration(nt - 2, N, N, N);
     iteration(nt - 1, N, Y, N);
     {
-      read_v(tile_base(nt - 1) + E_KB + E_UNITB);
-      static_for<2 * MT>([&](auto i_c) __attribute__((always_inline)) { pv_mfma(i_c, pB); });
+      read_v(tile_base(nt - 1) + W_KB + W_UNITB);
+      static_for<4 * MB>([&](auto i_c) __attribute__((always_inline)) { pv_mfma(i_c, pB); });
     }
     return finish(true);
   };
 
   auto run_exact = [&](auto rerun_c) __attribute__((always_inline)) {
     clear_o();
-    float m_off;
-    f32x16_t sc;
-    if constexpr (decltype(rerun_c)::value || !E_EARLY_DMA) prologue_issue();
+    f32x16_t sc[2];
+    if constexpr (decltype(rerun_c)::value) prologue_issue();
     prologue_wait();
-    first_scores(sc, m_off, 0.f);
+    first_scores(sc, 0.f, 0u);
     for (int t = 0; t < nt; ++t) {
-      const bool more = t + 3 < nt;
-      if (more) { dma_a(t + 3); dma_b(t + 3); dma_c(t + 3); }
+      if (t + 2 < nt) dma_tile(t + 2);
       const uint32_t tb = tile_base(t);
 #pragma unroll
       for (int sub = 0; sub < 2; ++sub) {
         if (t > 0 || sub > 0) {
-          read_k(tb + sub * E_UNITB);
-          sc = minit;
-#pragma unroll
-          for (int ks = 0; ks < KS; ++ks) sc = mfma32(kf[ks], qf[ks], sc);
-          float mx = sc[0];
-#pragma unroll
-          for (int r = 1; r < 16; ++r) mx = fmaxf(mx, sc[r]);
-          if (__any(mx > LAZY_THR)) {
-            const float delta = fmaxf(fmaxf(mx, __shfl_xor(mx, 32)), 0.f);
-            m_off += delta;
-            const float alpha = __builtin_amdgcn_exp2f(-delta);
-#pragma unroll
-            for (int r = 0; r < 16; ++r) { sc[r] -= delta; minit[r] = -m_off; }
-#pragma unroll
-            for (int mt = 0; mt < MT; ++mt)
-#pragma unroll
-              for (int r = 0; r < 16; ++r) oacc[mt][r] *= alpha;
+          read_k(tb + sub * W_UNITB);
+          qk_scores(sc);
+#pragma unroll
+          for (int qs = 0; qs < 2; ++qs) {
+            float mx = sc[qs][0];
+#pragma unroll
+            for (int r = 1; r < 16; ++r) mx = fmaxf(mx, sc[qs][r]);
+            if (__any(mx - off[qs] > LAZY_THR)) {
+              const float delta = fmaxf(fmaxf(mx, __shfl_xor(mx, 32)) - off[qs], 0.f);
+              off[qs] += delta;
+              const float alpha = __builtin_amdgcn_exp2f(-delta);
+              lsum[qs] *= alpha;
+#pragma unroll
+              for (int a = 0; a < 2; ++a) {
+                const float alpha_o = __shfl(alpha, 16 * a + i16);
+#pragma unroll
+                for (int mb = 0; mb < MB; ++mb)
+#pragma unroll
+                  for (int r = 0; r < 4; ++r) oacc[mb][2 * qs + a][r] *= alpha_o;
+              }
+            }
           }
         }
-        u32x4_t pf[2];
-#pragma unroll
-        for (int h = 0; h < 2; ++h)
-#pragma unroll
-          for (int jj = 0; jj < 4; ++jj)
-            pf[h][jj] = pack16(__builtin_amdgcn_exp2f(sc[8 * h + 2 * jj]), __builtin_amdgcn_exp2f(sc[8 * h + 2 * jj + 1]));
-        read_v(tb + E_KB + sub * E_UNITB);
-        static_for<2 * MT>([&](auto i_c) __attribute__((always_inline)) { pv_mfma(i_c, pf); });
-      }
-      if (t + 1 < nt) {
-        if (more) asm volatile("s_waitcnt vmcnt(%0)\n\ts_barrier" :: "i"(NDMA) : "memory");
-        else asm volatile("s_waitcnt vmcnt(0)\n\ts_barrier" ::: "memory");
-      }
+        u32x4_t pf[2][2];
+#pragma unroll
+        for (int qs = 0; qs < 2; ++qs)
+#pragma unroll
+          for (int h = 0; h < 2; ++h)
+#pragma unroll
+            for (int jj = 0; jj < 4; ++jj) {
+              const float e0 = __builtin_amdgcn_exp2f(sc[qs][8 * h + 2 * jj] - off[qs]), e1 = __builtin_amdgcn_exp2f(sc[qs][8 * h + 2 * jj + 1] - off[qs]);
+              lsum[qs] += e0 + e1;
+              pf[qs][h][jj] = pack16(e0, e1);
+            }
+        static_for<8>([&](auto k_c) __attribute__((always_inline)) { swap_p(k_c, pf); });
+        read_v(tb + W_KB + sub * W_UNITB);
+        static_for<4 * MB>([&](auto i_c) __attribute__((always_inline)) { pv_mfma(i_c, pf); });
+      }
+      if (t + 1 < nt) asm volatile("s_waitcnt vmcnt(0)\n\ts_barrier" ::: "memory");
     }
     finish(false);
   };
 
-  __syncthreads();
   dm_count(p, 2);
   if constexpr (TRY_NOMAX) {
     if (!run_fast()) run_exact(std::true_type{});
@@ -400,14 +476,16 @@
   }
 }
 
-template <int FLAGS>
+template <int FLAGS, int NW>
 int launch_dm80(int groups, hipStream_t s, const AttnParams& p) {
+  constexpr int NT = 64 * NW, NDMA = (W_BLOCKS + NW - 1) / NW;
+  constexpr int SMEM = W_TAB + NDMA * NT * 4;
   static uint64_t attr_done = 0;
   if (int rc = a3d_once_per_device(attr_done, [] {
-        return (int)hipFuncSetAttribute(reinterpret_cast<const void*>(&flash_attn_dm80_kernel<FLAGS>),
-                                        hipFuncAttributeMaxDynamicSharedMemorySize, E_SMEM_BYTES); })) return rc;
-  const int q_tiles = (p.q_len + 255) / 256;
-  flash_attn_dm80_kernel<FLAGS><<<dim3((unsigned)(p.heads * q_tiles), (unsigned)groups), dim3(512), E_SMEM_BYTES, s>>>(p);
+        return (int)hipFuncSetAttribute(reinterpret_cast<const void*>(&flash_attn_dm80_kernel<FLAGS, NW>),
+                                        hipFuncAttributeMaxDynamicSharedMemorySize, SMEM); })) return rc;
+  const int q_tiles = (p.q_len + NT - 1) / NT;
+  flash_attn_dm80_kernel<FLAGS, NW><<<dim3((unsigned)(p.heads * q_tiles), (unsigned)groups), dim3(NT), SMEM, s>>>(p);
   return a3d_launch_status();
 }
 
@@ -415,8 +493,10 @@
 
 int A3D_FN(a3d_launch_flash_dm80)(int flags, int groups, hipStream_t s, const AttnParams& p) {
   switch (flags) {
-    case 0: return launch_dm80<0>(groups, s, p);
-    case 1: return launch_dm80<1>(groups, s, p);
+    case 0: return launch_dm80<0, 4>(groups, s, p);
+    case 1: return launch_dm80<1, 4>(groups, s, p);
+    case 2: return launch_dm80<0, 8>(groups, s, p);
+    case 3: return launch_dm80<1, 8>(groups, s, p);
     default: return A3D_EINVAL;
   }
 }
diff --git a/animate3d_amd/csrc/flash_attn_dm80_narrow.hip b/animate3d_amd/csrc/flash_attn_dm80_narrow.hip
--- /dev/null
+++ b/animate3d_amd/csrc/flash_attn_dm80_narrow.hip
@@ -0,0 +1,422 @@
+#include "flash_common.h"
+
+namespace {
+
+constexpr int E_ROWB = 160;
+constexpr int E_UNITB = 32 * E_ROWB;
+constexpr int E_KB = 2 * E_UNITB;
+constexpr int E_TILEB = 2 * E_KB;
+constexpr int E_RING = 5;
+constexpr int E_CV = E_RING * E_TILEB + 32;
+constexpr int E_CV_BYTES = 2752;
+constexpr int E_SAMPLE = E_CV + E_CV_BYTES;
+constexpr int E_SMEM_BYTES = E_SAMPLE + E_UNITB;
+constexpr float E_L_BAD = 1.2676506e30f;
+#ifdef A3D_STORAGE_F16
+constexpr float E_BIAS = F16_BIAS;
+constexpr bool E_SAMPLED = true;
+#else
+constexpr float E_BIAS = 40.f;
+constexpr bool E_SAMPLED = false;
+#endif
+
+#ifdef A3D_EXP_R5_PATHS
+constexpr bool E_EARLY_DMA = false;
+#else
+constexpr bool E_EARLY_DMA = true;
+#endif
+
+extern __shared__ __attribute__((aligned(16))) uint8_t e_smem[];
+A3D_DEV u32x4_t e_lds128(uint32_t off) { return *reinterpret_cast<const u32x4_t*>(e_smem + off); }
+A3D_DEV u32x2_t e_ldstr(uint32_t off) { return lds_tr16_b64(reinterpret_cast<const uint16_t*>(e_smem + off)); }
+
+template <int FLAGS>
+__global__ __launch_bounds__(512, 2) void flash_attn_dm80n_kernel(const AttnParams p) {
+  constexpr int D = 80, KS = 5, MT = 3, NT = 512, BQ = 256;
+  constexpr int NEXP = 16, NCVT = 8, NDMA = 3;
+  constexpr bool TRY_NOMAX = (FLAGS & 1) != 0;
+
+  const int tid = threadIdx.x, lane = tid & 63, wid = tid >> 6;
+  const int w = __builtin_amdgcn_readfirstlane(wid);
+  const int l31 = lane & 31, g = lane >> 5, i16 = lane & 15, q4 = lane >> 4;
+  const int head = blockIdx.x % p.heads;
+  const int qt = blockIdx.x / p.heads;
+  const int64_t grp = blockIdx.y;
+  const int64_t hoff = (int64_t)head * D;
+  const uint32_t lds0 = fa_lds_addr(e_smem);
+
+  for (int i = tid; i < E_CV_BYTES / 2; i += NT) {
+    const int vb = 2 * i;
+    reinterpret_cast<uint16_t*>(e_smem + E_CV)[i] = (vb == 0 || vb == 160 || vb == 2560 || vb == 2720) ? ONE16 : (uint16_t)0;
+  }
+
+  const int64_t ld = p.km.ld;
+  const int64_t kgbase = map_group_base(p.km, grp);
+  const uint32_t seg_len = (uint32_t)p.km.seg_len;
+  const int64_t tile_step = (int64_t)64 * ld;
+  const int64_t wrap_step = (p.km.seg_stride - p.km.seg_len) * ld;
+  auto slot_src = [&](int slot) -> uint32_t {
+    const bool isk = slot < 640;
+    const int s2 = isk ? slot : slot - 640;
+    const int prow = s2 / 10, cpos = s2 % 10;
+    const int c = isk ? (cpos ^ ((prow >> 3) & 1)) : cpos;
+    const int key = isk ? prow : ((prow & ~7) | (((prow & 7) >> 1) + 4 * (prow & 1)));
+    return (uint32_t)(((int64_t)key * ld + c * 8) * 2);
+  };
+  const uint32_t voffA = slot_src(64 * w + lane);
+  const uint32_t voffB = slot_src(512 + 64 * w + lane);
+  const uint32_t voffC = slot_src(1024 + 32 * w + l31);
+  uint32_t voffS = 0;
+  if constexpr (E_SAMPLED) {
+    const int ss = (64 * w + lane) % 320, prow = ss / 10;
+    const int64_t key = (int64_t)prow * (p.kv_len / 32);
+    voffS = (uint32_t)((map_seq(p.km, key) * ld + ((ss % 10) ^ ((prow >> 3) & 1)) * 8) * 2);
+  }
+  const uint64_t maskS = w < 5 ? ~0ull : 0ull;
+
+  const int krow = kperm(l31);
+  const uint32_t klane = (uint32_t)(krow * E_ROWB + 16 * (g ^ ((krow >> 3) & 1)));
+  const int c4 = i16 & 3;
+  const uint32_t vrow = (uint32_t)((8 * (q4 >> 1) + 2 * (i16 >> 2)) * E_ROWB);
+  const uint32_t vlane01 = vrow + (uint32_t)(2 * (16 * (q4 & 1) + 4 * c4));
+  const bool v2_data = (q4 & 1) == 0;
+  const uint32_t vlane2 = v2_data ? vrow + (uint32_t)(2 * (64 + 4 * c4)) : (c4 == 0 ? (uint32_t)E_CV : (uint32_t)(E_CV + 8));
+  uint32_t vmul = v2_data ? 1u : 0u;
+  asm volatile("" : "+v"(vmul));
+
+  const uint16_t* gA = nullptr;
+  const uint16_t* gB = nullptr;
+  const uint16_t* gC = nullptr;
+  uint32_t seg_off = 0;
+  auto dma_reset = [&]() __attribute__((always_inline)) {
+    gA = dm_scalar(p.K + hoff + kgbase * ld);
+    gB = dm_scalar((w < 2 ? p.K : p.V) + hoff + kgbase * ld);
+    gC = dm_scalar(p.V + hoff + kgbase * ld);
+    seg_off = 0;
+  };
+  auto tile_base = [&](int tile) __attribute__((always_inline)) -> uint32_t { return (uint32_t)((tile % E_RING) * E_TILEB); };
+  auto dma_a = [&](int tile) __attribute__((always_inline)) { dm_glds16(voffA, gA, lds0 + tile_base(tile) + 1024 * w); };
+  auto dma_b = [&](int tile) __attribute__((always_inline)) { dm_glds16(voffB, gB, lds0 + tile_base(tile) + 8192 + 1024 * w); };
+  auto dma_c = [&](int tile) __attribute__((always_inline)) {
+    dm_glds16_m(voffC, gC, lds0 + tile_base(tile) + 16384 + 512 * w, 0xffffffffull);
+    seg_off += 64;
+    int64_t stp = tile_step;
+    if (seg_off >= seg_len) { stp += wrap_step; seg_off = 0; }
+    gA += stp; gB += stp; gC += stp;
+  };
+  auto prologue_issue = [&]() __attribute__((always_inline)) {
+    dma_reset();
+    if constexpr (E_SAMPLED && TRY_NOMAX)
+      dm_glds16_m(voffS, dm_scalar(p.K + hoff + kgbase * ld), lds0 + (uint32_t)(E_SAMPLE + 1024 * (w < 5 ? w : 0)), maskS);
+    dma_a(0); dma_b(0); dma_c(0);
+    dma_a(1); dma_b(1); dma_c(1);
+    dma_a(2); dma_b(2); dma_c(2);
+  };
+  auto prologue_wait = [&]() __attribute__((always_inline)) { asm volatile("s_waitcnt vmcnt(%0)\n\ts_barrier" :: "i"(NDMA) : "memory"); };
+  if constexpr (E_EARLY_DMA) prologue_issue();
+
+  const int q_idx = qt * BQ + wid * 32 + l31;
+  u32x4_t qf[KS];
+  {
+    const int64_t q_row = map_row(p.qm, grp, q_idx < p.q_len ? q_idx : p.q_len - 1);
+#pragma unroll
+    for (int ks = 0; ks < KS; ++ks) {
+      u32x4_t wq = *reinterpret_cast<const u32x4_t*>(p.Q + q_row * p.qm.ld + hoff + 16 * ks + 8 * g);
+#pragma unroll
+      for (int j = 0; j < 4; ++j) wq[j] = pack16(lo16(wq[j]) * p.scale_log2, hi16(wq[j]) * p.scale_log2);
+      qf[ks] = wq;
+    }
+  }
+
+
+  f32x16_t oacc[MT];
+  f32x16_t minit;
+  u32x4_t kf[KS];
+  u32x4_t vf[MT][2];
+  auto read_k = [&](uint32_t koff) __attribute__((always_inline)) {
+    const uint32_t a = klane + koff;
+#pragma unroll
+    for (int ks = 0; ks < KS; ++ks) kf[ks] = e_lds128(a + 32 * ks);
+  };
+  auto read_vhalf = [&](auto i_c, uint32_t a01, uint32_t a2) __attribute__((always_inline)) {
+    constexpr int i = decltype(i_c)::value, h = i / 6, mt = (i / 2) % 3, rr = i % 2;
+    const u32x2_t t = e_ldstr((mt == 2 ? a2 : a01 + 64 * mt) + (16 * h + rr) * E_ROWB);
+    vf[mt][h][2 * rr] = t[0];
+    vf[mt][h][2 * rr + 1] = t[1];
+  };
+  auto read_v = [&](uint32_t voff) __attribute__((always_inline)) {
+    const uint32_t a01 = vlane01 + voff, a2 = __umul24(vmul, voff) + vlane2;
+    static_for<12>([&](auto i_c) __attribute__((always_inline)) { read_vhalf(i_c, a01, a2); });
+  };
+  auto pv_mfma = [&](auto i_c, u32x4_t (&P)[2]) __attribute__((always_inline)) {
+    constexpr int i = decltype(i_c)::value, h = i / 3, mt = i % 3;
+    oacc[mt] = mfma32(vf[mt][h], P[h], oacc[mt]);
+  };
+  auto clear_o = [&]() __attribute__((always_inline)) {
+#pragma unroll
+    for (int mt = 0; mt < MT; ++mt)
+#pragma unroll
+      for (int r = 0; r < 16; ++r) oacc[mt][r] = 0.f;
+#pragma unroll
+    for (int r = 0; r < 16; ++r) minit[r] = 0.f;
+  };
+  const int nt = p.kv_len / 64;
+  auto first_scores = [&](f32x16_t& s, float& m_off, float bias, uint32_t koff = 0u) __attribute__((always_inline)) -> bool {
+    read_k(koff);
+#pragma unroll
+    for (int r = 0; r < 16; ++r) s[r] = 0.f;
+#pragma unroll
+    for (int ks = 0; ks < KS; ++ks) s = mfma32(kf[ks], qf[ks], s);
+    float mx = s[0];
+#pragma unroll
+    for (int r = 1; r < 16; ++r) mx = fmaxf(mx, s[r]);
+    mx = fmaxf(mx, __shfl_xor(mx, 32));
+    bool wide = false;
+    if constexpr (E_SAMPLED) {
+      if (bias != 0.f) {
+        float sm = 0.f, sq = 0.f;
+#pragma unroll
+        for (int r = 0; r < 16; ++r) { sm += s[r]; sq = fmaf(s[r], s[r], sq); }
+        sm += __shfl_xor(sm, 32); sq += __shfl_xor(sq, 32);
+        const float mean = sm * (1.f / 32.f);
+        bias = f16_sampled_bias(mx, mean, sq * (1.f / 32.f) - mean * mean, f16_expected_max_sds(p.kv_len), wide);
+      }
+    }
+    m_off = mx + bias;
+#pragma unroll
+    for (int r = 0; r < 16; ++r) { s[r] -= m_off; minit[r] = -m_off; }
+    return wide;
+  };
+  auto finish = [&](bool check) __attribute__((always_inline)) -> bool {
+    const float l_tot = __shfl(oacc[2][8], l31);
+    const bool bad = !(l_tot < E_L_BAD) || !(l_tot > 0.f);
+    if (check) {
+      if (__syncthreads_or(bad ? 1 : 0)) { dm_count(p, 1); return false; }
+    }
+    const float inv = p.out_scale / l_tot;
+    if (p.lse != nullptr && q_idx < p.q_len && g == 0)
+      p.lse[((int64_t)grp * p.heads + head) * p.q_len + q_idx] = __builtin_amdgcn_logf(l_tot) - minit[0];
+    if (q_idx < p.q_len) {
+      uint16_t* orow = p.O + map_row(p.om, grp, q_idx) * p.om.ld + hoff;
+      const bool wide_rows = E_EARLY_DMA && !p.accumulate && ((reinterpret_cast<uintptr_t>(p.O) | (uintptr_t)(p.om.ld * 2)) & 15u) == 0;
+      if (wide_rows) {
+#pragma unroll
+        for (int mt = 0; mt < MT; ++mt)
+#pragma unroll
+          for (int pr = 0; pr < 2; ++pr) {
+            if (32 * mt + 16 * pr >= D) continue;
+            u32x4_t v;
+#pragma unroll
+            for (int c = 0; c < 2; ++c) {
+              const uint32_t w0 = pack16(oacc[mt][8 * pr + 2 * c] * inv, oacc[mt][8 * pr + 2 * c + 1] * inv);
+              const uint32_t w1 = pack16(oacc[mt][8 * pr + 4 + 2 * c] * inv, oacc[mt][8 * pr + 4 + 2 * c + 1] * inv);
+              const auto r = __builtin_amdgcn_permlane32_swap(w0, w1, false, false);
+              v[c] = r[0];
+              v[2 + c] = r[1];
+            }
+            *reinterpret_cast<u32x4_t*>(orow + 32 * mt + 16 * pr + 8 * g) = v;
+          }
+      } else {
+#pragma unroll
+        for (int mt = 0; mt < MT; ++mt)
+#pragma unroll
+          for (int qd = 0; qd < 4; ++qd) {
+            const int d = 32 * mt + 8 * qd + 4 * g;
+            if (d < D) {
+              float v[4];
+#pragma unroll
+              for (int j = 0; j < 4; ++j) v[j] = oacc[mt][4 * qd + j] * inv;
+              if (p.accumulate) {
+                const u32x2_t prev = *reinterpret_cast<const u32x2_t*>(orow + d);
+                v[0] += lo16(prev[0]); v[1] += hi16(prev[0]); v[2] += lo16(prev[1]); v[3] += hi16(prev[1]);
+              }
+              u32x2_t o;
+              o[0] = pack16(v[0], v[1]);
+              o[1] = pack16(v[2], v[3]);
+              *reinterpret_cast<u32x2_t*>(orow + d) = o;
+            }
+          }
+      }
+    }
+    return true;
+  };
+
+  auto run_fast = [&]() __attribute__((always_inline)) -> bool {
+    clear_o();
+    f32x16_t sA, sB;
+    u32x4_t pA[2], pB[2];
+#pragma unroll
+    for (int h = 0; h < 2; ++h) { pA[h] = u32x4_t{0u, 0u, 0u, 0u}; pB[h] = u32x4_t{0u, 0u, 0u, 0u}; }
+
+    auto step = [&](auto do_qk_c, auto do_pv_c, f32x16_t& sCur, f32x16_t& sNext, u32x4_t (&pCur)[2], u32x4_t (&pPrev)[2],
+                    uint32_t kOff, uint32_t vOff, auto&& hook) __attribute__((always_inline)) {
+      constexpr bool DO_QK = decltype(do_qk_c)::value, DO_PV = decltype(do_pv_c)::value;
+      constexpr int NPV = DO_PV ? 2 * MT : 0, NQK = DO_QK ? KS : 0, NS = NPV + NQK;
+      constexpr int KSLOT = 2, VS0 = NPV + 1, VPS = 3;
+      const uint32_t va01 = vlane01 + vOff, va2 = __umul24(vmul, vOff) + vlane2;
+      float e[NEXP];
+      auto do_cvt = [&](auto c_c) __attribute__((always_inline)) {
+        constexpr int c = decltype(c_c)::value, h = c / 4, jj = c % 4;
+        pCur[h][jj] = pack16(e[2 * c], e[2 * c + 1]);
+      };
+      auto cdone = [](int s) constexpr { return s < 0 ? 0 : (NEXP * s / NS) / 2; };
+      __builtin_amdgcn_sched_barrier(0);
+      static_for<NS>([&](auto s_c) __attribute__((always_inline)) {
+        constexpr int s = decltype(s_c)::value;
+        if constexpr (s < NPV) {
+          pv_mfma(s_c, pPrev);
+        } else {
+          constexpr int ks = s - NPV;
+          if constexpr (ks == 0) sNext = mfma32(kf[0], qf[0], minit);
+          else sNext = mfma32(kf[ks], qf[ks], sNext);
+        }
+        if constexpr (DO_QK && DO_PV && s == KSLOT) read_k(kOff);
+        if constexpr (DO_QK && s >= VS0 && VPS * (s - VS0) < 12) {
+          static_for<VPS>([&](auto i_c) __attribute__((always_inline)) {
+            constexpr int i = VPS * (s - VS0) + decltype(i_c)::value;
+            if constexpr (i < 12) read_vhalf(std::integral_constant<int, i>{}, va01, va2);
+          });
+        }
+        hook(s_c);
+        constexpr int E0 = NEXP * s / NS, E1 = NEXP * (s + 1) / NS;
+        static_for<E1 - E0>([&](auto x_c) __attribute__((always_inline)) {
+          constexpr int x = E0 + decltype(x_c)::value;
+          e[x] = __builtin_amdgcn_exp2f(sCur[x]);
+        });
+        constexpr int C0 = cdone(s - 1), C1 = cdone(s);
+        static_for<C1 - C0>([&](auto c_c) __attribute__((always_inline)) { do_cvt(std::integral_constant<int, C0 + decltype(c_c)::value>{}); });
+        __builtin_amdgcn_sched_barrier(0);
+      });
+      {
+        constexpr int C0 = cdone(NS - 1);
+        static_for<NCVT - C0>([&](auto c_c) __attribute__((always_inline)) { do_cvt(std::integral_constant<int, C0 + decltype(c_c)::value>{}); });
+      }
+    };
+
+    if constexpr (!E_EARLY_DMA) prologue_issue();
+    prologue_wait();
+    {
+      float m_off;
+      if constexpr (E_SAMPLED) {
+        const bool wide = first_scores(sA, m_off, E_BIAS, (uint32_t)E_SAMPLE);
+        if (__syncthreads_count(wide ? 1 : 0) * 4 > NT) { dm_count(p, 0); return false; }
+        read_k(0u);
+        sA = minit;
+#pragma unroll
+        for (int ks = 0; ks < KS; ++ks) sA = mfma32(kf[ks], qf[ks], sA);
+      } else {
+        first_scores(sA, m_off, E_BIAS);
+      }
+      read_k((uint32_t)E_UNITB);
+    }
+
+    auto iteration = [&](int t, auto first_c, auto last_c, auto dma_c_) __attribute__((always_inline)) {
+      constexpr bool FIRST = decltype(first_c)::value, LAST = decltype(last_c)::value, DMA = decltype(dma_c_)::value;
+      auto even_hook = [&](auto s_c) __attribute__((always_inline)) {
+        if constexpr (DMA && decltype(s_c)::value == 1) dma_a(t + 3);
+      };
+      auto odd_hook = [&](auto s_c) __attribute__((always_inline)) {
+        if constexpr (DMA && decltype(s_c)::value == 1) dma_b(t + 3);
+        if constexpr (DMA && decltype(s_c)::value == 4) dma_c(t + 3);
+      };
+      const uint32_t tb = tile_base(t), tn = tile_base(t + 1);
+      step(std::true_type{}, std::integral_constant<bool, !FIRST>{}, sA, sB, pA, pB, tb + E_UNITB, tb + E_KB, even_hook);
+      step(std::integral_constant<bool, !LAST>{}, std::true_type{}, sB, sA, pB, pA, tn, tb + E_KB + E_UNITB, odd_hook);
+      if constexpr (!LAST) {
+        if constexpr (DMA) asm volatile("s_waitcnt vmcnt(%0)\n\ts_barrier" :: "i"(NDMA) : "memory");
+        else asm volatile("s_waitcnt vmcnt(0)\n\ts_barrier" ::: "memory");
+      }
+    };
+    constexpr std::true_type Y{};
+    constexpr std::false_type N{};
+    iteration(0, Y, N, Y);
+    for (int t = 1; t < nt - 3; ++t) iteration(t, N, N, Y);
+    iteration(nt - 3, N, N, N);
+    iteration(nt - 2, N, N, N);
+    iteration(nt - 1, N, Y, N);
+    {
+      read_v(tile_base(nt - 1) + E_KB + E_UNITB);
+      static_for<2 * MT>([&](auto i_c) __attribute__((always_inline)) { pv_mfma(i_c, pB); });
+    }
+    return finish(true);
+  };
+
+  auto run_exact = [&](auto rerun_c) __attribute__((always_inline)) {
+    clear_o();
+    float m_off;
+    f32x16_t sc;
+    if constexpr (decltype(rerun_c)::value || !E_EARLY_DMA) prologue_issue();
+    prologue_wait();
+    first_scores(sc, m_off, 0.f);
+    for (int t = 0; t < nt; ++t) {
+      const bool more = t + 3 < nt;
+      if (more) { dma_a(t + 3); dma_b(t + 3); dma_c(t + 3); }
+      const uint32_t tb = tile_base(t);
+#pragma unroll
+      for (int sub = 0; sub < 2; ++sub) {
+        if (t > 0 || sub > 0) {
+          read_k(tb + sub * E_UNITB);
+          sc = minit;
+#pragma unroll
+          for (int ks = 0; ks < KS; ++ks) sc = mfma32(kf[ks], qf[ks], sc);
+          float mx = sc[0];
+#pragma unroll
+          for (int r = 1; r < 16; ++r) mx = fmaxf(mx, sc[r]);
+          if (__any(mx > LAZY_THR)) {
+            const float delta = fmaxf(fmaxf(mx, __shfl_xor(mx, 32)), 0.f);
+            m_off += delta;
+            const float alpha = __builtin_amdgcn_exp2f(-delta);
+#pragma unroll
+            for (int r = 0; r < 16; ++r) { sc[r] -= delta; minit[r] = -m_off; }
+#pragma unroll
+            for (int mt = 0; mt < MT; ++mt)
+#pragma unroll
+              for (int r = 0; r < 16; ++r) oacc[mt][r] *= alpha;
+          }
+        }
+        u32x4_t pf[2];
+#pragma unroll
+        for (int h = 0; h < 2; ++h)
+#pragma unroll
+          for (int jj = 0; jj < 4; ++jj)
+            pf[h][jj] = pack16(__builtin_amdgcn_exp2f(sc[8 * h + 2 * jj]), __builtin_amdgcn_exp2f(sc[8 * h + 2 * jj + 1]));
+        read_v(tb + E_KB + sub * E_UNITB);
+        static_for<2 * MT>([&](auto i_c) __attribute__((always_inline)) { pv_mfma(i_c, pf); });
+      }
+      if (t + 1 < nt) {
+        if (more) asm volatile("s_waitcnt vmcnt(%0)\n\ts_barrier" :: "i"(NDMA) : "memory");
+        else asm volatile("s_waitcnt vmcnt(0)\n\ts_barrier" ::: "memory");
+      }
+    }
+    finish(false);
+  };
+
+  __syncthreads();
+  dm_count(p, 2);
+  if constexpr (TRY_NOMAX) {
+    if (!run_fast()) run_exact(std::true_type{});
+  } else {
+    run_exact(std::false_type{});
+  }
+}
+
+template <int FLAGS>
+int launch_dm80n(int groups, hipStream_t s, const AttnParams& p) {
+  static uint64_t attr_done = 0;
+  if (int rc = a3d_once_per_device(attr_done, [] {
+        return (int)hipFuncSetAttribute(reinterpret_cast<const void*>(&flash_attn_dm80n_kernel<FLAGS>),
+                                        hipFuncAttributeMaxDynamicSharedMemorySize, E_SMEM_BYTES); })) return rc;
+  const int q_tiles = (p.q_len + 255) / 256;
+  flash_attn_dm80n_kernel<FLAGS><<<dim3((unsigned)(p.heads * q_tiles), (unsigned)groups), dim3(512), E_SMEM_BYTES, s>>>(p);
+  return a3d_launch_status();
+}
+
+}
+
+int A3D_FN(a3d_launch_flash_dm80_narrow)(int flags, int groups, hipStream_t s, const AttnParams& p) {
+  switch (flags) {
+    case 0: return launch_dm80n<0>(groups, s, p);
+    case 1: return launch_dm80n<1>(groups, s, p);
+    default: return A3D_EINVAL;
+  }
+}
diff --git a/animate3d_amd/csrc/flash_common.h b/animate3d_amd/csrc/flash_common.h
--- a/animate3d_amd/csrc/flash_common.h
+++ b/animate3d_amd/csrc/flash_common.h
@@ -91,5 +91,6 @@
 
 __attribute__((visibility("hidden"))) int A3D_FN(a3d_launch_flash_dm)(int flags, int groups, hipStream_t s, const AttnParams& p);
 __attribute__((visibility("hidden"))) int A3D_FN(a3d_launch_flash_dm80)(int flags, int groups, hipStream_t s, const AttnParams& p);
+__attribute__((visibility("hidden"))) int A3D_FN(a3d_launch_flash_dm80_narrow)(int flags, int groups, hipStream_t s, const AttnParams& p);
 __attribute__((visibility("hidden"))) int A3D_FN(a3d_launch_flash_dm160)(int flags, int groups, hipStream_t s, const AttnParams& p);
 __attribute__((visibility("hidden"))) int A3D_FN(a3d_launch_cross_attn40)(int groups, hipStream_t s, const AttnParams& p);
diff --git a/animate3d_amd/hip_ops.py b/animate3d_amd/hip_ops.py
--- a/animate3d_amd/hip_ops.py
+++ b/animate3d_amd/hip_ops.py
@@ -342,14 +342,14 @@
 
     def flash_attn(self, q, k, v, qmap: RowMap, kmap: RowMap, groups: int, heads: int, q_len: int, kv_len: int, *,
                    out=None, out_scale: float = 1.0, accumulate: bool = False, causal: bool = False, with_lse: bool = False,
-                   accumulation_target: bool = False, exact: bool = False, plain: bool = False):
+                   accumulation_target: bool = False, exact: bool = False, plain: bool = False, dm80_narrow: bool = False, dm80_wg512: bool = False):
         q, k, v = self._act(q, "attn.q"), self._act(k, "attn.k"), self._act(v, "attn.v")
         C = q.shape[1]
         D = C // heads
         assert k.stride(0) == v.stride(0)
         o = out if out is not None else self.empty(q.shape[0], C)
         qm, km, om = qmap.c(q.stride(0)), kmap.c(k.stride(0)), qmap.c(o.stride(0))
-        flags = (1 if accumulate else 0) | (2 if causal else 0) | (4 if exact else 0) | (8 if plain else 0)
+        flags = (1 if accumulate else 0) | (2 if causal else 0) | (4 if exact else 0) | (8 if plain else 0) | (16 if dm80_narrow else 0) | (32 if dm80_wg512 else 0)
         if with_lse:
             lse = torch.empty((groups, heads, q_len), dtype=torch.float32, device=self.device)
             rc = self.lib.a3d_flash_attn_lse_bf16(self._stream(), _p(q), _p(k), _p(v), _p(o), ctypes.byref(qm), ctypes.byref(km), ctypes.byref(om),
diff --git a/include/animate3d_hip.h b/include/animate3d_hip.h
--- a/include/animate3d_hip.h
+++ b/include/animate3d_hip.h
@@ -61,6 +61,8 @@
 #define A3D_ATTN_CAUSAL 2
 #define A3D_ATTN_EXACT 4
 #define A3D_ATTN_PLAIN 8
+#define A3D_ATTN_DM80_NARROW 16
+#define A3D_ATTN_DM80_WG512 32
 int a3d_flash_attn_bf16(a3d_stream_t stream, const void* Q, const void* K, const void* V, void* O,
                         const a3d_rowmap* qmap, const a3d_rowmap* kmap, const a3d_rowmap* omap,
                         int groups, int heads, int head_dim, int64_t q_len, int64_t kv_len,
```

Result: no change. 2.385 denoise-steps/s, median of 6 (+0.3%).
